# tj12323/GeoPurify

Hardware: AMD Instinct MI355X
Metric: scenes/sec (ScanNet-val shape) + pooled-feature GB/s vs HBM peak (higher is better)
Workload: dtype f32 (student convolutions and pooling: f16 hi/lo split operands, 3 MFMAs per product, fp32 accumulate)

## Files before the change

geopurify_amd/_lib.py:

```python
import ctypes
import os
from ctypes import POINTER, c_char_p, c_double, c_float, c_int32, c_int64, c_size_t, c_uint32, c_void_p

_HERE = os.path.dirname(os.path.abspath(__file__))
LIB_PATH = os.environ.get("GP_LIB") or os.path.join(_HERE, "libgeopurify_hip.so")

_P = c_void_p
GP_KNN_MAX_K = 127

SIGNATURES = {
    "gp_version": (c_int32, []),
    "gp_last_error": (c_char_p, []),
    "gp_debug_set": (c_int32, [c_int32, c_int32]),
    "gp_debug_ptr": (c_int32, [c_int32, _P, c_size_t]),
    "gp_voxelize_workspace_bytes": (c_size_t, [c_int64]),
    "gp_voxelize_f64": (c_int32, [_P, c_int64, POINTER(c_double), _P, _P, _P, _P, _P, _P, _P, c_size_t, _P]),
    "gp_fnv_hash_f64": (c_int32, [_P, c_int64, _P, _P]),
    "gp_project_points_f64": (c_int32, [_P, c_int64, POINTER(c_double), c_double, c_double, c_double,
                                        c_double, _P, c_int32, c_int32, c_int32, c_double, _P, _P, _P]),
    "gp_render_depth_f64": (c_int32, [_P, c_int64, POINTER(c_double), c_double, c_double, c_double, c_double,
                                      c_int32, c_int32, c_int32, _P, _P]),
    "gp_minmax_i32": (c_int32, [_P, c_int64, _P, _P]),
    "gp_morton_order_workspace_bytes": (c_size_t, [c_int64]),
    "gp_morton_order": (c_int32, [_P, c_int64, _P, _P, _P, c_size_t, _P]),
    "gp_grid_bytes": (c_size_t, [c_int64, POINTER(c_int32)]),
    "gp_grid_build": (c_int32, [_P, c_int64, POINTER(c_int32), POINTER(c_int32), _P, c_size_t, _P]),
    "gp_scatter_mean_csr": (c_int32, [_P, c_int64, c_int32, _P, _P, c_int64, _P, _P, c_int64, c_int32, _P]),
    "gp_gather_rows": (c_int32, [_P, c_int64, c_int32, _P, c_int64, _P, _P, c_int64, _P]),
    "gp_kernel_map_build": (c_int32, [_P, _P, c_int64, _P, _P]),
    "gp_coords_order_batched_workspace_bytes": (c_size_t, [c_int64]),
    "gp_coords_order_batched": (c_int32, [_P, c_int64, _P, _P, _P, _P, _P, c_size_t, _P]),
    "gp_kernel_map_sorted": (c_int32, [_P, c_int64, _P, _P]),
    "gp_quantize_batched_workspace_bytes": (c_size_t, [c_int64]),
    "gp_quantize_batched": (c_int32, [_P, c_int64, _P, _P, _P, _P, _P, _P, _P, c_size_t, _P]),
    "gp_segment_labels": (c_int32, [_P, c_int64, _P, _P, _P, c_int64, c_int64, c_int32, _P, _P]),
    "gp_sparse_conv": (c_int32, [_P, c_int64, _P, c_int64, _P, c_int32, c_int32, c_int32, _P, _P, _P,
                                 c_int64, c_int32, _P, c_int64, _P]),
    "gp_conv_pairs_workspace_bytes": (c_size_t, [c_int64, c_int32]),
    "gp_conv_pairs_build": (c_int32, [_P, c_int64, c_int32, c_int32, _P, _P, _P, _P, _P, _P, _P, c_size_t, _P]),
    "gp_conv_chunk_plan_workspace_bytes": (c_size_t, [c_int64, c_int32]),
    "gp_conv_chunk_plan": (c_int32, [_P, c_int64, c_int32, c_int32, c_int32, c_int32, c_int32, _P, _P, _P, c_size_t, _P]),
    "gp_conv_weights_split": (c_int32, [_P, c_int32, c_int32, c_int32, c_float, _P, _P, _P]),
    "gp_split_f16": (c_int32, [_P, c_int64, c_int32, c_int64, _P, _P, c_int64, _P]),
    "gp_sparse_conv_f16x3": (c_int32, [_P, c_int64, _P, _P, c_int64, _P, _P, _P, _P, _P, c_int32, c_int64, c_int64, c_int32, _P, _P,
                                       c_int32, c_int32, _P, _P, _P, _P, c_int64, c_int32, _P, c_int64, _P, _P,
                                       c_int64, c_int32, POINTER(c_int32), POINTER(c_int32), POINTER(c_int32), _P, _P,
                                       _P, _P, c_int64, _P, c_int32, c_int32, _P]),
    "gp_conv_weights_split_blocked": (c_int32, [_P, c_int32, c_int32, c_int32, c_float, _P, _P, c_int32, _P]),
    "gp_pow2_scale": (c_int32, [_P, c_int64, c_int32, c_int64, _P, _P, c_size_t, _P]),
    "gp_voxel_rows_operands": (c_int32, [_P, c_int64, c_int32, _P, c_int64, c_int32, _P, _P, c_int64, _P, _P, c_int64, c_int32, _P, c_int64,
                                         _P, _P, _P, c_size_t, _P]),
    "gp_split_f16_scaled": (c_int32, [_P, c_int64, c_int32, c_int64, _P, _P, c_int64, _P, _P, _P, _P]),
    "gp_rcb_order": (c_int32, [_P, c_int64, c_int32, c_int32, _P, _P, _P]),
    "gp_rows_renumber_i32": (c_int32, [_P, c_int64, c_int32, _P, _P, _P, _P]),
    "gp_l2norm_rows": (c_int32, [_P, c_int64, c_int32, c_int64, _P]),
    "gp_embed_head_f16x3": (c_int32, [_P, _P, c_int64, _P, _P, _P, c_int64, c_int32, c_int32, c_float, c_int32, _P, c_int64, _P, _P, c_float, _P, _P]),
    "gp_knn_workspace_bytes": (c_size_t, [c_int64]),
    "gp_knn_lattice": (c_int32, [_P, _P, _P, c_int64, c_int32, _P, _P, c_size_t, _P]),
    "gp_knn_lattice_two_pass": (c_int32, [_P, _P, _P, c_int64, c_int32, _P, _P, c_size_t, _P]),
    "gp_knn_batched_workspace_bytes": (c_size_t, [c_int64]),
    "gp_knn_batched": (c_int32, [_P, _P, c_int64, c_int32, _P, _P, _P, c_size_t, _P]),
    "gp_affinity_softmax": (c_int32, [_P, c_int64, c_int32, _P, c_int32, c_int64, c_float, _P, _P]),
    "gp_affinity_softmax_scatter": (c_int32, [_P, c_int64, c_int32, _P, c_int32, c_int64, c_float, _P, _P, _P, _P, _P]),
    "gp_pool_ell": (c_int32, [_P, c_int64, _P, _P, c_int32, c_int64, c_int32, _P, c_int64, _P]),
    "gp_pool_transpose_workspace_bytes": (c_size_t, [c_int64, c_int32]),
    "gp_pool_transpose_build": (c_int32, [_P, c_int64, c_int32, _P, _P, _P, c_size_t, _P]),
    "gp_pool_ell_transpose": (c_int32, [_P, c_int64, _P, _P, _P, c_int32, c_int64, c_int32, _P, c_int64, _P]),
    "gp_pool_ell_wgrad": (c_int32, [_P, c_int64, _P, c_int64, _P, c_int32, c_int64, c_int32, _P, c_int32, _P]),
    "gp_affinity_softmax_backward_workspace_bytes": (c_size_t, [c_int64, c_int32]),
    "gp_affinity_softmax_backward": (c_int32, [_P, c_int64, c_int32, _P, _P, _P, c_int32, c_int64, c_float, _P, _P, _P, c_int64, _P,
                                               c_size_t, _P]),
    "gp_l2norm_rows_backward": (c_int32, [_P, c_int64, _P, c_int64, c_int32, c_int64, _P, c_int64, _P]),
    "gp_pool_tiles_workspace_bytes": (c_size_t, [c_int64, c_int32]),
    "gp_pool_tiles_count": (c_int32, [_P, c_int64, c_int32, c_int32, _P, _P, c_size_t, _P]),
    "gp_pool_tiles_fill": (c_int32, [_P, _P, c_int64, c_int32, c_int32, _P, _P, _P, _P]),
    "gp_pool_tiles_apply": (c_int32, [_P, c_int64, _P, _P, _P, c_int32, c_int64, c_int32, _P, c_int64, _P]),
    "gp_pool_mfma_workspace_bytes": (c_size_t, [c_int64, c_int32]),
    "gp_pool_mfma_count": (c_int32, [_P, c_int64, c_int32, c_int32, c_int32, _P, _P, _P, c_size_t, _P]),
    "gp_pool_mfma_fill": (c_int32, [_P, _P, c_int64, c_int32, c_int32, _P, _P, c_int64, _P, _P, _P, _P]),
    "gp_pool_mfma_apply": (c_int32, [_P, _P, c_int64, _P, _P, _P, _P, c_int64, c_int32, c_int32, _P, _P, c_int64, _P, c_int64, _P, _P]),
    "gp_pool_mfma_apply_persistent": (c_int32, [_P, _P, c_int64, _P, _P, _P, _P, c_int64, c_int32, c_int32, c_int32, _P, _P, c_int64,
                                                _P, c_int64, c_int64, _P, _P, _P]),
    "gp_pool_cs_workspace_bytes": (c_size_t, [c_int64, c_int32]),
    "gp_pool_cs_count": (c_int32, [_P, c_int64, c_int32, c_int32, _P, _P, _P, _P, c_size_t, _P]),
    "gp_pool_cs_fill": (c_int32, [_P, _P, c_int64, c_int32, c_int32, _P, c_int64, c_int32, _P, _P, _P, _P, _P]),
    "gp_pool_cs_structure": (c_int32, [_P, c_int64, c_int32, c_int32, _P, c_int64, c_int32, _P, _P, _P, _P, _P, _P]),
    "gp_pool_cs_structure_valid": (c_int32, [_P, c_int64, c_int32, c_int32, _P, c_int64, c_int32, _P, _P, _P, _P]),
    "gp_affinity_cs_fragments": (c_int32, [_P, _P, c_int64, c_int32, c_int32, c_float, _P, _P, _P, _P, c_int32, _P, _P, _P]),
    "gp_pool_cs_apply": (c_int32, [_P, _P, c_int64, _P, _P, _P, _P, _P, c_int64, c_int32, c_int32, _P, _P, c_int64, _P, c_int64, _P, _P]),
    "gp_pool_cs_deps": (c_int32, [_P, _P, c_int64, c_int32, _P, _P, _P]),
    "gp_pool_cs_chain_flag_words": (c_size_t, [c_int64, c_int32]),
    "gp_pool_cs_chain_flag_words_d": (c_size_t, [c_int64, c_int32, c_int32]),
    "gp_pool_cs_apply_chain": (c_int32, [_P, _P, _P, _P, c_int64, _P, _P, _P, _P, _P, c_int64, c_int32, c_int32, c_int32, _P, c_int64, _P, _P, _P,
                                         c_uint32, _P]),
    "gp_lift_dense_accum": (c_int32, [_P, c_int32, c_int32, c_int32, _P, _P, _P, c_int64, _P, c_int64, _P, _P]),
    "gp_lift_dense_bilinear_accum": (c_int32, [_P, c_int32, c_int32, c_int32, c_int32, c_int32, _P, _P, _P, c_int64, _P,
                                               c_int64, _P, _P]),
    "gp_lift_dense_finish": (c_int32, [_P, c_int64, c_int32, _P, c_int64, _P, _P]),
    "gp_lift_masks_workspace_bytes": (c_size_t, [c_int32, c_int32, c_int32]),
    "gp_lift_masks_view": (c_int32, [_P, c_int32, c_int32, c_int32, _P, _P, _P, _P, _P, c_int32, c_int32,
                                     _P, _P, c_int64, _P, _P, _P, c_size_t, _P]),
    "gp_pv_count": (c_int32, [_P, c_int64, _P, _P]),
    "gp_scan_workspace_bytes": (c_size_t, [c_int64]),
    "gp_exclusive_scan_i64": (c_int32, [_P, c_int64, _P, _P, c_size_t, _P]),
    "gp_pv_fill": (c_int32, [_P, _P, c_int64, c_int32, _P, _P, _P, _P, _P]),
    "gp_segment_tables": (c_int32, [_P, c_int32, c_int32, _P, c_int32, c_float, _P, _P, _P]),
    "gp_fuse_views_top3": (c_int32, [_P, _P, _P, c_int64, _P, _P, c_int32, c_int32, c_int32, _P, c_int64, _P, _P]),
    "gp_seen_masks": (c_int32, [_P, c_int64, _P, _P, _P]),
    "gp_fuse_views_top3_fill": (c_int32, [_P, _P, _P, c_int64, _P, _P, c_int32, c_int32, c_int32, _P, _P, c_int64, _P]),
    "gp_nn1_workspace_bytes": (c_size_t, [c_int64, c_int64]),
    "gp_nn1_f64": (c_int32, [_P, c_int64, _P, c_int64, _P, _P, c_size_t, _P]),
    "gp_nn1_masked_workspace_bytes": (c_size_t, [c_int64]),
    "gp_nn1_masked_f64": (c_int32, [_P, c_int64, _P, _P, _P, _P, c_size_t, _P]),
    "gp_visible_lists_workspace_bytes": (c_size_t, [c_int64]),
    "gp_visible_lists": (c_int32, [_P, c_int64, _P, _P, _P, _P, _P, c_size_t, _P]),
    "gp_views_visible_lists_workspace_bytes": (c_size_t, [c_int64, c_int32]),
    "gp_views_visible_lists": (c_int32, [_P, c_int64, _P, _P, c_int32, c_int32, c_int32, c_int32, c_double, c_int64, c_int64,
                                         _P, _P, _P, _P, _P, _P, _P, c_size_t, _P]),
    "gp_lift_masks_views_workspace_bytes": (c_size_t, [c_int32, c_int32, c_int32, c_int32, c_int64, c_int64, c_int64]),
    "gp_lift_masks_views": (c_int32, [_P, c_int32, c_int32, c_int32, c_int32, _P, _P, _P, _P, _P, c_int32, c_int32, _P, c_int64,
                                      _P, _P, _P, _P, _P, _P, c_int32, c_int64, c_int64, _P, _P, _P, _P, _P, c_size_t, _P]),
    "gp_classify_argmax": (c_int32, [_P, c_int64, c_int32, c_int64, _P, c_int32, c_float, _P, _P, _P]),
    "gp_gather_rows_classify": (c_int32, [_P, c_int64, c_int32, _P, c_int64, _P, _P, c_int64, _P, c_int32, c_float, _P, _P, _P]),
    "gp_rows_argmax": (c_int32, [_P, c_int64, c_int32, c_int64, _P, c_int64, c_int32, _P, _P, _P]),
    "gp_col_stats_workspace_bytes": (c_size_t, [c_int64, c_int32]),
    "gp_col_stats": (c_int32, [_P, c_int64, c_int64, c_int32, _P, _P, _P, c_size_t, _P]),
    "gp_bn_train_apply": (c_int32, [_P, c_int64, c_int64, c_int32, _P, _P, _P, _P, c_float, _P, c_int64, c_int32, _P, c_int64,
                                    _P, _P, c_int64, c_float, _P, _P, _P]),
    "gp_bn_train_backward_workspace_bytes": (c_size_t, [c_int64, c_int32]),
    "gp_bn_train_backward": (c_int32, [_P, c_int64, _P, c_int64, _P, c_int64, _P, _P, c_float, _P, _P, c_int64, c_int32, _P, c_int64,
                                       _P, c_int64, _P, _P, _P, _P, _P, c_int64, _P, c_size_t, _P]),
    "gp_col_sums_f64": (c_int32, [_P, c_int64, c_int64, c_int32, _P, _P, _P, c_size_t, _P]),
    "gp_bn_bwd_sums_f64": (c_int32, [_P, c_int64, _P, c_int64, _P, c_int64, _P, _P, c_float, _P, _P, c_int64, c_int32, _P, _P, c_size_t, _P]),
    "gp_bn_bwd_apply": (c_int32, [_P, c_int64, _P, c_int64, _P, c_int64, _P, _P, c_float, _P, _P, _P, c_int64, c_int64, c_int32, _P, c_int64,
                                  _P, c_int64, _P, _P]),
    "gp_infonce_workspace_bytes": (c_size_t, [c_int64, c_int32]),
    "gp_infonce_fwd_bwd": (c_int32, [_P, c_int64, c_int64, c_int32, _P, c_int64, _P, c_int64, c_int32, c_float, _P, _P, c_int64,
                                     _P, c_size_t, _P]),
    "gp_infonce_weighted_fwd_bwd": (c_int32, [_P, c_int64, c_int64, c_int32, _P, c_int64, _P, c_int64, c_int32, c_float, _P, _P, _P, _P, c_int64,
                                              _P, c_size_t, _P]),
    "gp_conv_wgrad_workspace_bytes": (c_size_t, [c_int64, c_int32, c_int32]),
    "gp_conv_wgrad_f16x3": (c_int32, [_P, _P, c_int64, _P, _P, c_int64, _P, _P, _P, c_int64, _P, c_int32, c_int32, c_int32, c_int32,
                                      _P, _P, _P, c_size_t, _P]),
    "gp_adamw_step": (c_int32, [_P, _P, _P, _P, c_int64, c_float, c_float, c_float, c_float, c_float, c_int64, _P]),
    "gp_knn_points_f32": (c_int32, [_P, c_int64, _P, c_int64, c_int32, _P, _P, _P]),
    "gp_sampler_select": (c_int32, [_P, c_int64, c_int64, c_int64, _P, c_int32, _P, _P, _P]),
    "gp_sim_segments_f16x3": (c_int32, [_P, _P, c_int64, c_int32, _P, _P, _P, _P, c_int64, c_int64, _P, _P]),
    "gp_sampler_select_segments": (c_int32, [_P, _P, _P, _P, c_int64, c_int64, _P, c_int32, _P, _P, _P]),
    "gp_sampler_micro_segments": (c_int32, [_P, _P, _P, _P, _P, c_int64, c_int32, _P, c_int64, c_int32, _P, _P]),
    "gp_normalize_split_f16": (c_int32, [_P, c_int64, c_int32, c_int64, c_int64, c_float, _P, _P, c_int64, _P]),
    "gp_iou_hist_i64": (c_int32, [_P, _P, c_int64, c_int32, POINTER(c_int64), c_int32, _P, _P]),
    "gp_nn1_batched_workspace_bytes": (c_size_t, [c_int64]),
    "gp_nn1_batched": (c_int32, [_P, _P, _P, _P, c_int64, c_int32, _P, _P, _P, c_size_t, _P]),
    "gp_iou_hist_batched_i64": (c_int32, [_P, _P, c_int64, _P, _P, c_int64, c_int32, c_int32, POINTER(c_int64), c_int32, _P, _P]),
    "gp_sparse_conv_tiles": (c_int32, [POINTER(c_int32)]),
    "gp_segment_loss_col_step": (c_int32, []),
    "gp_segment_loss_unit_rows": (c_int32, [_P, c_int64, c_int32, c_int64, _P, c_int64, c_int32, _P, _P]),
    "gp_segment_loss_items_workspace_bytes": (c_size_t, [c_int64, c_int64]),
    "gp_segment_loss_items": (c_int32, [_P, _P, c_int64, _P, _P, c_int64, c_int32, POINTER(c_int64), c_int32, c_int32, _P, _P, _P, _P, _P, _P,
                                        _P, c_size_t, _P]),
    "gp_segment_loss_rows": (c_int32, [_P, c_int64, c_int64, c_int32, c_int32, _P, _P, _P, _P, _P, _P, _P, c_int64, _P, _P, _P]),
    "gp_segment_loss_reduce_workspace_bytes": (c_size_t, [c_int64, c_int32]),
    "gp_segment_loss_reduce": (c_int32, [_P, _P, c_int64, _P, c_int32, c_int32, _P, _P, _P, c_size_t, _P]),
    "gp_fused_decode_workspace_bytes": (c_size_t, [c_int64, c_int64]),
    "gp_fused_decode": (c_int32, [_P, c_int64, _P, _P, c_int64, c_int64, _P, c_int64, c_int32, _P, _P, _P, _P, c_size_t, _P]),
    "gp_lift_batched_col_chunk": (c_int32, []),
    "gp_lift_batched_transpose": (c_int32, [_P, c_int32, c_int32, c_int64, _P, _P]),
    "gp_lift_batched_workspace_bytes": (c_size_t, [c_int64, c_int32]),
    "gp_lift_batched": (c_int32, [_P, c_int64, _P, c_int32, c_int32, c_int32, _P, _P, _P, _P, c_int32, c_int32, c_int32, c_int32, c_int32,
                                  c_double, c_int64, c_int64, c_int32, _P, c_int64, _P, _P, _P, _P, _P, _P, _P, c_size_t, _P]),
    "gp_lift_stream_state_bytes": (c_size_t, [c_int64]),
    "gp_lift_stream_begin_workspace_bytes": (c_size_t, [c_int64]),
    "gp_lift_stream_begin": (c_int32, [_P, c_int64, c_int32, _P, c_size_t, _P, c_int64, _P, _P, _P, c_size_t, _P]),
    "gp_lift_stream_add_workspace_bytes": (c_size_t, [c_int32]),
    "gp_lift_stream_add": (c_int32, [_P, c_int64, _P, c_size_t, _P, c_int32, c_int32, c_int32, _P, _P, _P, _P, c_int32, c_int32, c_int32,
                                     c_int32, c_int32, c_double, c_int64, c_int64, _P, c_int64, _P, _P, _P, _P, _P, c_size_t, _P]),
    "gp_lift_stream_finish_workspace_bytes": (c_size_t, [c_int64]),
    "gp_lift_stream_finish": (c_int32, [_P, c_int64, _P, c_size_t, _P, c_int32, c_int64, _P, _P, c_int32, _P, c_int64, _P, _P, _P, _P,
                                        c_size_t, _P]),
    "gp_lift_masks_batched_lists_workspace_bytes": (c_size_t, [c_int64, c_int32]),
    "gp_lift_masks_batched_lists": (c_int32, [_P, c_int64, _P, _P, _P, _P, c_int32, c_int32, c_int32, c_int32, c_double, c_int64, c_int64,
                                              c_int64, _P, _P, _P, _P, _P, _P, _P, _P, _P, c_size_t, _P]),
    "gp_lift_masks_batched_workspace_bytes": (c_size_t, [c_int64, c_int32, c_int32, c_int32, c_int32, c_int32, c_int32, c_int64, c_int32,
                                                         c_int64]),
    "gp_lift_masks_batched": (c_int32, [_P, c_int64, _P, c_int32, _P, c_int32, c_int32, c_int32, _P, _P, _P, _P, _P, c_int32, c_int32,
                                        _P, _P, _P, _P, _P, _P, c_int64, c_int32, c_int64, _P, _P, c_int32, c_int32, c_int32,
                                        _P, c_int64, _P, _P, _P, _P, _P, _P, c_size_t, _P]),
}

_lib = None


# ... 39 lines not shown
```

geopurify_amd/csrc/order_grid.hip:

```cpp
#include <cstring>
#include <rocprim/device/device_radix_sort.hpp>

#include "gp_grid.h"

namespace {

__global__ void minmax_kernel(const int32_t *__restrict__ c, int64_t nv, int32_t *__restrict__ mm) {
    int lo[3] = {INT32_MAX, INT32_MAX, INT32_MAX}, hi[3] = {INT32_MIN, INT32_MIN, INT32_MIN};
    for (int64_t i = blockIdx.x * (int64_t)blockDim.x + threadIdx.x; i < nv; i += (int64_t)gridDim.x * blockDim.x) {
#pragma unroll
        for (int a = 0; a < 3; ++a) {
            int v = c[i * 3 + a];
            lo[a] = min(lo[a], v);
            hi[a] = max(hi[a], v);
        }
    }
    __shared__ int s_lo[4][3], s_hi[4][3];
#pragma unroll
    for (int a = 0; a < 3; ++a) {
        for (int o = 32; o > 0; o >>= 1) {
            lo[a] = min(lo[a], __shfl_xor(lo[a], o, 64));
            hi[a] = max(hi[a], __shfl_xor(hi[a], o, 64));
        }
        if (gp_lane() == 0) { s_lo[threadIdx.x >> 6][a] = lo[a]; s_hi[threadIdx.x >> 6][a] = hi[a]; }
    }
    __syncthreads();
    if (threadIdx.x < 3) {
        const int a = threadIdx.x;
        atomicMin(&mm[a], min(min(s_lo[0][a], s_lo[1][a]), min(s_lo[2][a], s_lo[3][a])));
        atomicMax(&mm[3 + a], max(max(s_hi[0][a], s_hi[1][a]), max(s_hi[2][a], s_hi[3][a])));
    }
}

__global__ void init_minmax_kernel(int32_t *mm) {
    if (threadIdx.x < 3) mm[threadIdx.x] = INT32_MAX;
    else if (threadIdx.x < 6) mm[threadIdx.x] = INT32_MIN;
}

__global__ void morton_keys_kernel(const int32_t *__restrict__ c, int64_t nv, const int32_t *__restrict__ mm,
                                   uint64_t *__restrict__ keys, int32_t *__restrict__ vals) {
    int64_t i = blockIdx.x * (int64_t)blockDim.x + threadIdx.x;
    if (i >= nv) return;
    uint32_t x = (uint32_t)(c[i * 3 + 0] - mm[0]);
    uint32_t y = (uint32_t)(c[i * 3 + 1] - mm[1]);
    uint32_t z = (uint32_t)(c[i * 3 + 2] - mm[2]);
    keys[i] = gp_morton3(x, y, z);
    vals[i] = (int32_t)i;
}

__global__ void invert_perm_kernel(const int32_t *__restrict__ perm, int64_t nv, int32_t *__restrict__ rank) {
    int64_t i = blockIdx.x * (int64_t)blockDim.x + threadIdx.x;
    if (i < nv) rank[perm[i]] = (int32_t)i;
}

__global__ void grid_init_kernel(void *grid, int3 origin, int3 extent, int3 cdim, int64_t nv, int32_t max_cells,
                                 int64_t cell_index_off, int64_t records_off) {
    GpGridHeader *h = reinterpret_cast<GpGridHeader *>(grid);
    if (blockIdx.x == 0 && threadIdx.x == 0) {
        h->origin[0] = origin.x; h->origin[1] = origin.y; h->origin[2] = origin.z;
        h->extent[0] = extent.x; h->extent[1] = extent.y; h->extent[2] = extent.z;
        h->cdim[0] = cdim.x; h->cdim[1] = cdim.y; h->cdim[2] = cdim.z;
        h->status = 0; h->ncells = 0; h->max_cells = max_cells; h->nv = nv;
        h->cell_index_off = cell_index_off; h->records_off = records_off;
    }
    int32_t *ci = reinterpret_cast<int32_t *>(reinterpret_cast<char *>(grid) + cell_index_off);
    int64_t ncell = (int64_t)cdim.x * cdim.y * cdim.z;
    for (int64_t i = blockIdx.x * (int64_t)blockDim.x + threadIdx.x; i < ncell; i += (int64_t)gridDim.x * blockDim.x)
        ci[i] = -1;
}

__device__ __forceinline__ int64_t cell_raster(const GpGridHeader *h, int rx, int ry, int rz) {
    return ((int64_t)(rz >> 3) * h->cdim[1] + (ry >> 3)) * h->cdim[0] + (rx >> 3);
}

__global__ void grid_heads_kernel(void *grid, const int32_t *__restrict__ c, int64_t nv) {
    GpGridHeader *h = reinterpret_cast<GpGridHeader *>(grid);
    int32_t *ci = reinterpret_cast<int32_t *>(reinterpret_cast<char *>(grid) + h->cell_index_off);
    GpCellRec *recs = reinterpret_cast<GpCellRec *>(reinterpret_cast<char *>(grid) + h->records_off);
    int64_t i = blockIdx.x * (int64_t)blockDim.x + threadIdx.x;
    if (i >= nv) return;
    int rx = c[i * 3] - h->origin[0], ry = c[i * 3 + 1] - h->origin[1], rz = c[i * 3 + 2] - h->origin[2];
    bool bad = (unsigned)rx >= (unsigned)h->extent[0] || (unsigned)ry >= (unsigned)h->extent[1] ||
               (unsigned)rz >= (unsigned)h->extent[2];
    uint64_t key = gp_morton3(rx, ry, rz);
    bool head = true;
    if (i > 0) {
        int px = c[i * 3 - 3] - h->origin[0], py = c[i * 3 - 2] - h->origin[1], pz = c[i * 3 - 1] - h->origin[2];
        uint64_t pk = gp_morton3(px, py, pz);
        if (pk >= key) bad = true;
        head = (pk >> 9) != (key >> 9);
    }
    if (bad) { atomicOr(&h->status, 1); return; }
    if (head) {
        int slot = atomicAdd(&h->ncells, 1);
        GpCellRec &r = recs[slot];
        r.start = (int32_t)i;
        r.count = 0;
#pragma unroll
        for (int j = 0; j < 16; ++j) r.bits[j] = 0u;
        ci[cell_raster(h, rx, ry, rz)] = slot;
    }
}

__global__ void grid_fill_kernel(void *grid, const int32_t *__restrict__ c, int64_t nv) {
    GpGridHeader *h = reinterpret_cast<GpGridHeader *>(grid);
    if (h->status) return;
    int32_t *ci = reinterpret_cast<int32_t *>(reinterpret_cast<char *>(grid) + h->cell_index_off);
    GpCellRec *recs = reinterpret_cast<GpCellRec *>(reinterpret_cast<char *>(grid) + h->records_off);
    int64_t i = blockIdx.x * (int64_t)blockDim.x + threadIdx.x;
    if (i >= nv) return;
    int rx = c[i * 3] - h->origin[0], ry = c[i * 3 + 1] - h->origin[1], rz = c[i * 3 + 2] - h->origin[2];
    int slot = ci[cell_raster(h, rx, ry, rz)];
    uint32_t l = gp_local9(rx, ry, rz);
    atomicOr(&recs[slot].bits[l >> 5], 1u << (l & 31));
    atomicAdd(&recs[slot].count, 1);
}

__global__ void kernel_map_kernel(const void *grid, const int32_t *__restrict__ c, int64_t nv,
                                  int32_t *__restrict__ nbr_map) {
    GpGridView g(grid);
    int64_t i = blockIdx.x * (int64_t)blockDim.x + threadIdx.x;
    if (i >= nv) return;
    int rx = c[i * 3] - g.h->origin[0], ry = c[i * 3 + 1] - g.h->origin[1], rz = c[i * 3 + 2] - g.h->origin[2];
    int k = 0;
    for (int dz = -1; dz <= 1; ++dz)
        for (int dy = -1; dy <= 1; ++dy)
            for (int dx = -1; dx <= 1; ++dx, ++k)
                nbr_map[(int64_t)k * nv + i] = (k == 13) ? (int32_t)i : g.lookup_rel(rx + dx, ry + dy, rz + dz);
}

}

extern "C" int gp_minmax_i32(const int32_t *coords, int64_t nv, int32_t *mm, void *stream_) {
    GP_CHECK_ARG(coords && mm && nv > 0, "gp_minmax_i32: null/empty argument");
    hipStream_t s = gp_stream(stream_);
    int blocks = (int)((nv + 255) / 256);
    init_minmax_kernel<<<1, 64, 0, s>>>(mm);
    minmax_kernel<<<min(blocks, 64), 256, 0, s>>>(coords, nv, mm);
    GP_CHECK_LAUNCH();
    return GP_OK;
}

extern "C" size_t gp_morton_order_workspace_bytes(int64_t nv) {
    size_t tmp = 0;
    (void)rocprim::radix_sort_pairs(nullptr, tmp, (uint64_t *)nullptr, (uint64_t *)nullptr, (int32_t *)nullptr,
                              (int32_t *)nullptr, (size_t)nv, 0, 64, 0);
    GpCarver cv(nullptr, 0);
    cv.take<int32_t>(8);
    cv.take<uint64_t>(nv);
    cv.take<uint64_t>(nv);
    cv.take<int32_t>(nv);
    cv.take<char>(tmp);
    return cv.off;
}

extern "C" int gp_morton_order(const int32_t *coords, int64_t nv, int32_t *perm, int32_t *rank, void *workspace,
                               size_t workspace_bytes, void *stream_) {
    GP_CHECK_ARG(nv > 0 && nv < (1ll << 31), "gp_morton_order: nv=%lld out of range", (long long)nv);
    hipStream_t s = gp_stream(stream_);
    size_t tmp = 0;
    (void)rocprim::radix_sort_pairs(nullptr, tmp, (uint64_t *)nullptr, (uint64_t *)nullptr, (int32_t *)nullptr,
                              (int32_t *)nullptr, (size_t)nv, 0, 64, 0);
    GpCarver cv(workspace, workspace_bytes);
    int32_t *mm = cv.take<int32_t>(8);
    uint64_t *k0 = cv.take<uint64_t>(nv);
    uint64_t *k1 = cv.take<uint64_t>(nv);
    int32_t *v0 = cv.take<int32_t>(nv);
    char *t = cv.take<char>(tmp);
    if (!cv.ok()) { gp_set_error("gp_morton_order: workspace too small (%zu < %zu)", workspace_bytes, cv.off); return GP_ENOMEM; }
    int blocks = (int)((nv + 255) / 256);
    init_minmax_kernel<<<1, 64, 0, s>>>(mm);
    minmax_kernel<<<min(blocks, 64), 256, 0, s>>>(coords, nv, mm);
    morton_keys_kernel<<<blocks, 256, 0, s>>>(coords, nv, mm, k0, v0);
    GP_CHECK_LAUNCH();
    GP_CHECK_HIP(rocprim::radix_sort_pairs(t, tmp, k0, k1, v0, perm, (size_t)nv, 0, 64, s));
    invert_perm_kernel<<<blocks, 256, 0, s>>>(perm, nv, rank);
    GP_CHECK_LAUNCH();
    return GP_OK;
}

static void grid_layout(int64_t nv, const int32_t *extent, int3 &cdim, int32_t &max_cells, int64_t &ci_off,
                        int64_t &rec_off, size_t &total) {
    cdim = make_int3(((extent[0] - 1) >> 3) + 1, ((extent[1] - 1) >> 3) + 1, ((extent[2] - 1) >> 3) + 1);
    int64_t ncell = (int64_t)cdim.x * cdim.y * cdim.z;
    max_cells = (int32_t)(nv < ncell ? nv : ncell);
    ci_off = 256;
    rec_off = ci_off + (int64_t)gp_align_up((size_t)ncell * 4, 256);
    total = (size_t)rec_off + gp_align_up((size_t)max_cells * sizeof(GpCellRec), 256);
}

extern "C" size_t gp_grid_bytes(int64_t nv, const int32_t *extent_host) {
    if (!extent_host || nv <= 0 || extent_host[0] <= 0 || extent_host[1] <= 0 || extent_host[2] <= 0) return 0;
    int3 cdim; int32_t mc; int64_t a, b; size_t total;
    grid_layout(nv, extent_host, cdim, mc, a, b, total);
    return total;
}

extern "C" int gp_grid_build(const int32_t *coords, int64_t nv, const int32_t *origin_host, const int32_t *extent_host,
                             void *grid, size_t grid_bytes, void *stream_) {
    GP_CHECK_ARG(coords && grid && origin_host && extent_host && nv > 0, "gp_grid_build: null/empty argument");
    for (int a = 0; a < 3; ++a)
        if (extent_host[a] <= 0 || extent_host[a] > (1 << 15)) { gp_set_error("gp_grid_build: extent[%d]=%d not in 1..32768", a, extent_host[a]); return GP_ERANGE; }
    int3 cdim; int32_t mc; int64_t ci_off, rec_off; size_t total;
    grid_layout(nv, extent_host, cdim, mc, ci_off, rec_off, total);
    if (grid_bytes < total) { gp_set_error("gp_grid_build: grid buffer too small (%zu < %zu)", grid_bytes, total); return GP_ENOMEM; }
    hipStream_t s = gp_stream(stream_);
    int blocks = (int)((nv + 255) / 256);
    grid_init_kernel<<<1024, 256, 0, s>>>(grid, make_int3(origin_host[0], origin_host[1], origin_host[2]),
                                         make_int3(extent_host[0], extent_host[1], extent_host[2]), cdim, nv, mc, ci_off, rec_off);
    grid_heads_kernel<<<blocks, 256, 0, s>>>(grid, coords, nv);
    grid_fill_kernel<<<blocks, 256, 0, s>>>(grid, coords, nv);
    GP_CHECK_LAUNCH();
    return GP_OK;
}

extern "C" int gp_kernel_map_build(const void *grid, const int32_t *coords, int64_t nv, int32_t *nbr_map, void *stream_) {
    GP_CHECK_ARG(grid && coords && nbr_map && nv > 0, "gp_kernel_map_build: null/empty argument");
    kernel_map_kernel<<<(int)((nv + 255) / 256), 256, 0, gp_stream(stream_)>>>(grid, coords, nv, nbr_map);
    GP_CHECK_LAUNCH();
    return GP_OK;
}
```

geopurify_amd/csrc/rcb.hip:

```cpp
#include "gp_common.h"

namespace {

constexpr int RCB_MAX_SEG = 32;

template <int CH, int NT>
__global__ void __launch_bounds__(NT)
rcb_chunk_kernel(const int32_t *__restrict__ coords , int64_t nv, int leaf, int32_t *__restrict__ sigma, int32_t *__restrict__ rho) {
    __shared__ int s_c[3][CH];
    __shared__ unsigned s_key[CH];
    __shared__ unsigned short s_perm[2][CH];
    __shared__ unsigned char s_seg[CH];
    __shared__ int s_start[RCB_MAX_SEG + 1], s_len[RCB_MAX_SEG], s_axis[RCB_MAX_SEG], s_lo[RCB_MAX_SEG][3], s_hi[RCB_MAX_SEG][3];
    __shared__ int s_nseg, s_more;
    const int tid = threadIdx.x;
    const int64_t base = (int64_t)blockIdx.x * CH;
    const int n = (int)((nv - base) < CH ? (nv - base) : CH);
    for (int i = tid; i < CH; i += NT) {
        const int64_t r = base + (i < n ? i : n - 1);
        s_c[0][i] = coords[r * 3];
        s_c[1][i] = coords[r * 3 + 1];
        s_c[2][i] = coords[r * 3 + 2];
        s_perm[0][i] = (unsigned short)i;
    }
    if (tid == 0) { s_nseg = 1; s_start[0] = 0; s_len[0] = n; s_more = n > leaf; }
    __syncthreads();
    int cur = 0, level = 0;
    while (s_more) {
        const int nseg = s_nseg;
        for (int i = tid; i < nseg * 3; i += NT) { s_lo[i / 3][i % 3] = 0x7fffffff; s_hi[i / 3][i % 3] = -0x7fffffff; }
        for (int i = tid; i < CH; i += NT) {
            int sg = 0;
            if (i < n) {
                int lo = 0, hi = nseg - 1;
                while (lo < hi) { const int mid = (lo + hi + 1) >> 1; if (s_start[mid] <= i) lo = mid; else hi = mid - 1; }
                sg = lo;
            }
            s_seg[i] = (unsigned char)sg;
        }
        __syncthreads();
        for (int i = tid; i < n; i += NT) {
            const int sg = s_seg[i];
            if (s_len[sg] > leaf) {
                const int r = s_perm[cur][i];
#pragma unroll
                for (int a = 0; a < 3; ++a) { atomicMin(&s_lo[sg][a], s_c[a][r]); atomicMax(&s_hi[sg][a], s_c[a][r]); }
            }
        }
        __syncthreads();
        if (tid < nseg) {
            int ax = 0, best = -1;
            if (s_len[tid] > leaf) {
#pragma unroll
                for (int a = 0; a < 3; ++a) { const int e = s_hi[tid][a] - s_lo[tid][a]; if (e > best) { best = e; ax = a; } }
            } else {
                ax = -1;
            }
            s_axis[tid] = ax;
        }
        __syncthreads();
        for (int i = tid; i < CH; i += NT) {
            unsigned k = 0xffffffffu;
            if (i < n) {
                const int sg = s_seg[i], ax = s_axis[sg];
                unsigned c = 0;
                if (ax >= 0) c = (unsigned)(s_c[ax][s_perm[cur][i]] - s_lo[sg][ax]) & 0x7fffu;
                k = ((unsigned)sg << 27) | (c << 12) | (unsigned)i;
            }
            s_key[i] = k;
        }
        __syncthreads();
        const int limit = (n == CH) ? (CH >> level) : CH;
        for (int kk = 2; kk <= limit; kk <<= 1)
            for (int j = kk >> 1; j > 0; j >>= 1) {
                for (int i = tid; i < CH; i += NT) {
                    const int ixj = i ^ j;
                    if (ixj > i) {
                        const unsigned x = s_key[i], y = s_key[ixj];
                        const bool up = (kk == limit) || ((i & kk) == 0);
                        if ((x > y) == up) { s_key[i] = y; s_key[ixj] = x; }
                    }
                }
                __syncthreads();
            }
        ++level;
        for (int i = tid; i < n; i += NT) s_perm[cur ^ 1][i] = s_perm[cur][s_key[i] & 0xfffu];
        cur ^= 1;
        if (tid == 0) {
            int ns = 0, more = 0;
            int st[RCB_MAX_SEG], ln[RCB_MAX_SEG];
            for (int sg = 0; sg < nseg; ++sg) {
                const int len = s_len[sg], start = s_start[sg];
                if (len > leaf && ns + 2 <= RCB_MAX_SEG) {
                    int half = ((len / 2 + leaf - 1) / leaf) * leaf;
                    if (half >= len) half = len / 2;
                    st[ns] = start; ln[ns] = half; ++ns;
                    st[ns] = start + half; ln[ns] = len - half; ++ns;
                    more |= (half > leaf) | (len - half > leaf);
                } else {
                    st[ns] = start; ln[ns] = len; ++ns;
                }
            }
            for (int sg = 0; sg < ns; ++sg) { s_start[sg] = st[sg]; s_len[sg] = ln[sg]; }
            s_nseg = ns;
            s_more = more && ns < RCB_MAX_SEG;
        }
        __syncthreads();
    }
    for (int i = tid; i < n; i += NT) {
        const int r = s_perm[cur][i];
        sigma[base + i] = (int32_t)(base + r);
        rho[base + r] = (int32_t)(base + i);
    }
}

__global__ void rows_renumber_kernel(const int32_t *__restrict__ nbr, int64_t nv, int k, const int32_t *__restrict__ sigma,
                                     const int32_t *__restrict__ rho, int32_t *__restrict__ out) {
    const int64_t total = nv * k;
    for (int64_t i = blockIdx.x * (int64_t)blockDim.x + threadIdx.x; i < total; i += (int64_t)gridDim.x * blockDim.x) {
        const int64_t p = i / k;
        const int j = (int)(i - p * k);
        out[i] = rho[nbr[(int64_t)sigma[p] * k + j]];
    }
}

}

extern "C" int gp_rcb_order(const int32_t *coords, int64_t nv, int32_t chunk_rows, int32_t leaf_rows, int32_t *sigma, int32_t *rho,
                            void *stream_) {
    GP_CHECK_ARG(coords && sigma && rho && nv > 0, "gp_rcb_order: null/empty argument");
    GP_CHECK_ARG(chunk_rows == 1024 || chunk_rows == 2048, "gp_rcb_order: chunk_rows=%d (1024 or 2048: a chunk lives in one workgroup's LDS)", chunk_rows);
    GP_CHECK_ARG(leaf_rows >= 16 && chunk_rows % leaf_rows == 0 && chunk_rows / leaf_rows <= RCB_MAX_SEG,
                 "gp_rcb_order: leaf_rows=%d must divide the chunk into at most %d leaves", leaf_rows, RCB_MAX_SEG);
    GP_CHECK_ARG(nv < ((int64_t)1 << 31), "gp_rcb_order: row ids are 32-bit");
    hipStream_t s = gp_stream(stream_);
    const unsigned blocks = (unsigned)((nv + chunk_rows - 1) / chunk_rows);
    if (chunk_rows == 1024) rcb_chunk_kernel<1024, 256><<<blocks, 256, 0, s>>>(coords, nv, leaf_rows, sigma, rho);
    else rcb_chunk_kernel<2048, 512><<<blocks, 512, 0, s>>>(coords, nv, leaf_rows, sigma, rho);
    GP_CHECK_LAUNCH();
    return GP_OK;
}

extern "C" int gp_rows_renumber_i32(const int32_t *nbr, int64_t nv, int32_t k, const int32_t *sigma, const int32_t *rho, int32_t *out,
                                    void *stream_) {
    GP_CHECK_ARG(nbr && sigma && rho && out && nv > 0 && k > 0 && out != nbr, "gp_rows_renumber_i32: null/empty argument (out must not alias nbr)");
    rows_renumber_kernel<<<2048, 256, 0, gp_stream(stream_)>>>(nbr, nv, k, sigma, rho, out);
    GP_CHECK_LAUNCH();
    return GP_OK;
}
```

geopurify_amd/csrc/sparse_conv_v2.hip:

```cpp
#include <cstring>
#include <type_traits>
#include <rocprim/device/device_scan.hpp>

#include <hip/hip_fp16.h>

#include <stdlib.h>

#include "gp_common.h"
#include "gp_gfx950.h"

namespace {

constexpr int TM = 256, TN = 256, TK = 32;
constexpr int NT2 = 512;
constexpr int APITCH = 32;
__device__ __forceinline__ int sw_slot(int row, int slot) {
    const int h = (0x78 >> (((row >> 2) & 3) * 2)) & 3;
    return slot ^ h;
}

__device__ __forceinline__ void pair_decode(int64_t i, int kv, const int32_t *__restrict__ R, int nchunks, int &c, int &k, int64_t &u) {
    const int row_q = (int)(i / kv);
    int lo = 0, hi = nchunks - 1;
    while (lo < hi) {
        const int mid = (lo + hi + 1) >> 1;
        if (R[mid] <= row_q) lo = mid; else hi = mid - 1;
    }
    c = lo;
    const int64_t r0 = R[c], rows_raw = R[c + 1] - r0, rows_c = rows_raw > 0 ? rows_raw : 1;
    const int64_t rem = i - (int64_t)kv * r0;
    int64_t kk = rem / rows_c;
    kk = kk < 0 ? 0 : (kk >= kv ? kv - 1 : kk);
    k = (int)kk;
    u = r0 + (rem - kk * rows_c);
}
__global__ void pair_flags_kernel(const int32_t *__restrict__ nm, int64_t nv, int kv, const int32_t *__restrict__ R, int nchunks,
                                  int32_t *__restrict__ f) {
    int64_t total = (int64_t)kv * nv;
    int64_t i = blockIdx.x * (int64_t)blockDim.x + threadIdx.x;
    if (i >= total) return;
    int c, k; int64_t u;
    pair_decode(i, kv, R, nchunks, c, k, u);
    u = u < 0 ? 0 : (u >= nv ? nv - 1 : u);
    f[i] = nm[(int64_t)k * nv + u] >= 0 ? 1 : 0;
}
__global__ void pair_emit_kernel(const int32_t *__restrict__ nm, const int32_t *__restrict__ sc, int64_t nv, int kv,
                                 const int32_t *__restrict__ R, int nchunks, int32_t *__restrict__ pair_in, int32_t *__restrict__ pair_pos,
                                 int32_t *__restrict__ seg_off ) {
    int64_t total = (int64_t)kv * nv;
    int64_t i = blockIdx.x * (int64_t)blockDim.x + threadIdx.x;
    if (i >= total) return;
    int c, k; int64_t u;
    pair_decode(i, kv, R, nchunks, c, k, u);
    u = u < 0 ? 0 : (u >= nv ? nv - 1 : u);
    int in = nm[(int64_t)k * nv + u];
    int s = sc[i];
    pair_pos[(int64_t)k * nv + u] = in >= 0 ? s : -1;
    if (in >= 0) pair_in[s] = in;
    if (u == (int64_t)R[c]) seg_off[c * kv + k] = s;
    if (i == total - 1) seg_off[(c + 1) * kv] = s + (in >= 0 ? 1 : 0);
}
__global__ void chunk_count_kernel(const int32_t *__restrict__ nm, int64_t nv, int kv, int granule, int32_t *__restrict__ cnt ) {
    const int g = blockIdx.x, k = blockIdx.y;
    const int64_t r0 = (int64_t)g * granule, r1 = r0 + granule < nv ? r0 + granule : nv;
    int c = 0;
    for (int64_t u = r0 + threadIdx.x; u < r1; u += blockDim.x) c += nm[(int64_t)k * nv + u] >= 0;
    c = gp_wave_sum(c);
    __shared__ int s_c[4];
    if (gp_lane() == 0) s_c[threadIdx.x >> 6] = c;
    __syncthreads();
    if (threadIdx.x == 0) cnt[g * 32 + k] = s_c[0] + s_c[1] + s_c[2] + s_c[3];
}
constexpr int CP_WIN = 512;
__device__ __forceinline__ int cp_sum32(int v) {
    v += __builtin_amdgcn_update_dpp(0, v, 0xB1, 0xF, 0xF, true);
    v += __builtin_amdgcn_update_dpp(0, v, 0x4E, 0xF, 0xF, true);
    v += __builtin_amdgcn_update_dpp(0, v, 0x141, 0xF, 0xF, true);
    v += __builtin_amdgcn_update_dpp(0, v, 0x140, 0xF, 0xF, true);
    return __builtin_amdgcn_readlane(v, 0) + __builtin_amdgcn_readlane(v, 16);
}
__global__ void __launch_bounds__(256)
chunk_plan_kernel(const int32_t *__restrict__ cnt, int ngran, int kv, int granule, int64_t nv, int col_tiles, int target,
                  int max_chunks, int32_t *__restrict__ R, int32_t *__restrict__ n_chunks) {
    __shared__ unsigned short s_cnt[CP_WIN * 32];
    const int tid = threadIdx.x, lane = tid & 63;
    int sum = 0, nc = 0, start_g = 0;
    if (tid == 0) R[0] = 0;
    for (int g0 = 0; g0 < ngran; g0 += CP_WIN) {
        const int n = ngran - g0 < CP_WIN ? ngran - g0 : CP_WIN;
        __syncthreads();
        {
            const int4 *c4 = reinterpret_cast<const int4 *>(cnt + (int64_t)g0 * 32);
            const int n4 = n * 8;
            for (int i0 = tid; i0 < n4; i0 += 1024) {
                int4 v[4];
#pragma unroll
                for (int q = 0; q < 4; ++q) v[q] = (i0 + q * 256 < n4) ? c4[i0 + q * 256] : make_int4(0, 0, 0, 0);
#pragma unroll
                for (int q = 0; q < 4; ++q) {
                    const int i = i0 + q * 256;
                    if (i < n4) {
                        const int k0 = (i * 4) & 31;
                        s_cnt[i * 4 + 0] = (unsigned short)(k0 + 0 < kv ? v[q].x : 0);
                        s_cnt[i * 4 + 1] = (unsigned short)(k0 + 1 < kv ? v[q].y : 0);
                        s_cnt[i * 4 + 2] = (unsigned short)(k0 + 2 < kv ? v[q].z : 0);
                        s_cnt[i * 4 + 3] = (unsigned short)(k0 + 3 < kv ? v[q].w : 0);
                    }
                }
            }
        }
        __syncthreads();
        if (tid < 64) {
            auto step = [&](int g, int add, int tiles_with) {
                if (tiles_with > target && g != start_g && nc + 1 < max_chunks) {
                    ++nc;
                    if (lane == 0) R[nc] = g * granule;
                    sum = add;
                    start_g = g;
                    return true;
                }
                sum += add;
                return false;
            };
            for (int gl = 0; gl < n; gl += 4) {
                int a[4], run[4], t[4];
#pragma unroll
                for (int j = 0; j < 4; ++j) a[j] = (lane < 32 && gl + j < n) ? s_cnt[(gl + j) * 32 + lane] : 0;
                run[0] = sum + a[0];
#pragma unroll
                for (int j = 1; j < 4; ++j) run[j] = run[j - 1] + a[j];
#pragma unroll
                for (int j = 0; j < 4; ++j) t[j] = cp_sum32(lane < 32 ? (run[j] + TM - 1) / TM : 0) * col_tiles;
                bool redo = false;
#pragma unroll
                for (int j = 0; j < 4; ++j) {
                    if (gl + j >= n) break;
                    const int tiles_with = redo ? cp_sum32(lane < 32 ? (sum + a[j] + TM - 1) / TM : 0) * col_tiles : t[j];
                    redo = step(g0 + gl + j, a[j], tiles_with) || redo;
                }
            }
        }
    }
    if (tid == 0) { R[nc + 1] = (int32_t)nv; n_chunks[0] = nc + 1; }
}
__global__ void tile_desc_kernel(const int32_t *__restrict__ seg_off, const int32_t *__restrict__ tile_start, int nseg, int kv,
                                 int4 *__restrict__ desc) {
    int sgi = blockIdx.x * blockDim.x + threadIdx.x;
    if (sgi >= nseg) return;
    int t0 = tile_start[sgi], t1 = tile_start[sgi + 1];
    int p0 = seg_off[sgi], p1 = seg_off[sgi + 1];
    for (int t = t0; t < t1; ++t) {
        int base = p0 + (t - t0) * TM;
        desc[t] = make_int4(sgi % kv, base, min(TM, p1 - base), 0);
    }
}

__global__ void tile_start_kernel(const int32_t *__restrict__ seg_off, int nseg, int32_t *__restrict__ tile_start) {
    if (blockIdx.x != 0 || threadIdx.x != 0) return;
    int acc = 0;
    for (int s = 0; s < nseg; ++s) {
        tile_start[s] = acc;
        acc += (seg_off[s + 1] - seg_off[s] + TM - 1) / TM;
    }
    tile_start[nseg] = acc;
}

struct V2Smem {
    _Float16 a_hi[2][TM][APITCH];
    _Float16 a_lo[2][TM][APITCH];
    _Float16 b_hi[2][TN][APITCH];
    _Float16 b_lo[2][TN][APITCH];
};

template <int NRT>
__device__ __forceinline__ void mma_step_f16x3(const V2Smem &sm, int buf, int wm, int wn, int fl, int fsw,
                                               f32x4 (&acc)[4][8]) {
    f16x8 ah[NRT > 0 ? NRT : 1], al[NRT > 0 ? NRT : 1];
#pragma unroll
    for (int i = 0; i < NRT; ++i) {
        ah[i] = *reinterpret_cast<const f16x8 *>(&sm.a_hi[buf][wm * 64 + i * 16 + fl][fsw]);
        al[i] = *reinterpret_cast<const f16x8 *>(&sm.a_lo[buf][wm * 64 + i * 16 + fl][fsw]);
    }
#pragma unroll
    for (int j = 0; j < 8; ++j) {
        f16x8 bh = *reinterpret_cast<const f16x8 *>(&sm.b_hi[buf][wn * 128 + j * 16 + fl][fsw]);
        f16x8 bl = *reinterpret_cast<const f16x8 *>(&sm.b_lo[buf][wn * 128 + j * 16 + fl][fsw]);
#pragma unroll
        for (int i = 0; i < NRT; ++i) acc[i][j] = __builtin_amdgcn_mfma_f32_16x16x32_f16(ah[i], bh, acc[i][j], 0, 0, 0);
#pragma unroll
        for (int i = 0; i < NRT; ++i) acc[i][j] = __builtin_amdgcn_mfma_f32_16x16x32_f16(ah[i], bl, acc[i][j], 0, 0, 0);
#pragma unroll
        for (int i = 0; i < NRT; ++i) acc[i][j] = __builtin_amdgcn_mfma_f32_16x16x32_f16(al[i], bh, acc[i][j], 0, 0, 0);
    }
}
template <int NRT>
__device__ __forceinline__ void mma_step_f16x3_off(const unsigned char *smem, const uint32_t (&fa_hi)[4], const uint32_t (&fa_lo)[4],
                                                   uint32_t a_off, const V2Smem &sm, int buf, int wn, int fl, int fsw, f32x4 (&acc)[4][8]) {
    f16x8 ah[NRT > 0 ? NRT : 1], al[NRT > 0 ? NRT : 1];
#pragma unroll
    for (int i = 0; i < NRT; ++i) {
        ah[i] = *reinterpret_cast<const f16x8 *>(smem + fa_hi[i] + a_off);
        al[i] = *reinterpret_cast<const f16x8 *>(smem + fa_lo[i] + a_off);
    }
#pragma unroll
    for (int j = 0; j < 8; ++j) {
        f16x8 bh = *reinterpret_cast<const f16x8 *>(&sm.b_hi[buf][wn * 128 + j * 16 + fl][fsw]);
        f16x8 bl = *reinterpret_cast<const f16x8 *>(&sm.b_lo[buf][wn * 128 + j * 16 + fl][fsw]);
#pragma unroll
        for (int i = 0; i < NRT; ++i) acc[i][j] = __builtin_amdgcn_mfma_f32_16x16x32_f16(ah[i], bh, acc[i][j], 0, 0, 0);
#pragma unroll
        for (int i = 0; i < NRT; ++i) acc[i][j] = __builtin_amdgcn_mfma_f32_16x16x32_f16(ah[i], bl, acc[i][j], 0, 0, 0);
#pragma unroll
        for (int i = 0; i < NRT; ++i) acc[i][j] = __builtin_amdgcn_mfma_f32_16x16x32_f16(al[i], bh, acc[i][j], 0, 0, 0);
    }
}
template <bool TUNE>
__global__ void __launch_bounds__(NT2)
conv_phase1_kernel(const float *__restrict__ x, int64_t ld_x, const int32_t *__restrict__ pair_in,
                   const int32_t *__restrict__ off, const int32_t *__restrict__ tile_start, const int4 *__restrict__ tile_desc,
                   int nseg, int kv, const _Float16 *__restrict__ w_hi, const _Float16 *__restrict__ w_lo, int cin, int cout,
                   float *__restrict__ P, int n_tiles, int ablate_, int tile_begin, int tile_count, int pair_base, int w_blocked) {
    extern __shared__ __align__(16) unsigned char smem_raw[];
    const int ablate = TUNE ? ablate_ : 0;
    V2Smem &sm = *reinterpret_cast<V2Smem *>(smem_raw);
// ... 798 lines not shown
            }
        }
    }
}

__global__ void split_rows_scaled_kernel(const float *__restrict__ x, int64_t ld_x, int d, int64_t n, _Float16 *__restrict__ hi,
                                         _Float16 *__restrict__ lo, int64_t ld_h, const float *__restrict__ scale,
                                         float *__restrict__ row_inv, const int32_t *__restrict__ dst_row) {
    const int lane = gp_lane();
    for (int64_t r = (blockIdx.x * (int64_t)blockDim.x + threadIdx.x) >> 6; r < n; r += ((int64_t)gridDim.x * blockDim.x) >> 6) {
        float s = scale ? scale[0] : 1.f;
        const int64_t ro = dst_row ? (int64_t)dst_row[r] : r;
        if (row_inv) {
            float amax = 0.f;
            for (int c = lane * 4; c < d; c += 256) {
                float4 a = *reinterpret_cast<const float4 *>(x + r * ld_x + c);
                amax = fmaxf(amax, fmaxf(fmaxf(fabsf(a.x), fabsf(a.y)), fmaxf(fabsf(a.z), fabsf(a.w))));
            }
            s = gp_pow2_for(gp_wave_max(amax));
            if (lane == 0) row_inv[ro] = 1.f / s;
        }
        for (int c = lane * 4; c < d; c += 256) {
            float4 a = *reinterpret_cast<const float4 *>(x + r * ld_x + c);
            float v[4] = {a.x * s, a.y * s, a.z * s, a.w * s};
            f16x4 h, l;
            gp_split_f16<4>(v, h, l);
            if (lo) {
                *reinterpret_cast<f16x4 *>(hi + ro * ld_h + c) = h;
                *reinterpret_cast<f16x4 *>(lo + ro * ld_h + c) = l;
            } else {
                _Float16 *ph = hi + ro * ld_h + ((c >> 5) << 6) + (c & 31);
                *reinterpret_cast<f16x4 *>(ph) = h;
                *reinterpret_cast<f16x4 *>(ph + 32) = l;
            }
        }
    }
}

__global__ void amax_kernel(const float *__restrict__ x, int64_t ld_x, int d, int64_t n, unsigned *__restrict__ out) {
    float m = 0.f;
    const int64_t total = n * (d / 4);
    for (int64_t i = blockIdx.x * (int64_t)blockDim.x + threadIdx.x; i < total; i += (int64_t)gridDim.x * blockDim.x) {
        int64_t r = i / (d / 4);
        int c = (int)(i - r * (d / 4)) * 4;
        float4 a = *reinterpret_cast<const float4 *>(x + r * ld_x + c);
        m = fmaxf(m, fmaxf(fmaxf(fabsf(a.x), fabsf(a.y)), fmaxf(fabsf(a.z), fabsf(a.w))));
    }
    __shared__ float s_m[4];
    m = gp_wave_max(m);
    if (gp_lane() == 0) s_m[threadIdx.x >> 6] = m;
    __syncthreads();
    if (threadIdx.x == 0) atomicMax(out, __float_as_uint(fmaxf(fmaxf(s_m[0], s_m[1]), fmaxf(s_m[2], s_m[3]))));
}
__global__ void pow2_scale_kernel(const unsigned *__restrict__ amax_bits, float *__restrict__ out2) {
    const float s = gp_pow2_for(__uint_as_float(amax_bits[0]));
    out2[0] = s;
    out2[1] = 1.f / s;
}

__global__ void split_rows_kernel(const float *__restrict__ x, int64_t ld_x, int d, int64_t n, _Float16 *__restrict__ hi,
                                  _Float16 *__restrict__ lo, int64_t ld_h) {
    int64_t total = n * (d / 4);
    for (int64_t i = blockIdx.x * (int64_t)blockDim.x + threadIdx.x; i < total; i += (int64_t)gridDim.x * blockDim.x) {
        int64_t r = i / (d / 4);
        int c = (int)(i - r * (d / 4)) * 4;
        float4 a = *reinterpret_cast<const float4 *>(x + r * ld_x + c);
        float v[4] = {a.x, a.y, a.z, a.w};
        f16x4 h, l;
        gp_split_f16<4>(v, h, l);
        *reinterpret_cast<f16x4 *>(hi + r * ld_h + c) = h;
        *reinterpret_cast<f16x4 *>(lo + r * ld_h + c) = l;
    }
}

__global__ void weight_split_kernel(const float *__restrict__ w, int kv, int cin, int cout, float s,
                                    _Float16 *__restrict__ hi, _Float16 *__restrict__ lo) {
    int64_t total = (int64_t)kv * cin * cout;
    for (int64_t i = blockIdx.x * (int64_t)blockDim.x + threadIdx.x; i < total; i += (int64_t)gridDim.x * blockDim.x) {
        int64_t k = i / ((int64_t)cin * cout);
        int64_t rem = i - k * (int64_t)cin * cout;
        int n = (int)(rem / cin), c = (int)(rem % cin);
        const float v = w[(k * cin + c) * cout + n] * s;
        gp_split_f16(v, hi[i], lo[i]);
    }
}

__global__ void __launch_bounds__(256)
weight_split_blocked_kernel(const float *__restrict__ w, int kv, int cin, int cout, float s,
                            _Float16 *__restrict__ hi, _Float16 *__restrict__ lo, int transpose_flip) {
    const int steps = cin / TK, nt = cout / TN;
    const int st = blockIdx.x % steps, t = (blockIdx.x / steps) % nt, k = blockIdx.x / (steps * nt);
    const int c = threadIdx.x;
    const int rho = (c & 128) | ((c >> 3) & 15) | ((c & 7) << 4);
    float v[TK];
    if (transpose_flip) {
        const float *src = w + ((int64_t)(kv - 1 - k) * cout + t * TN + c) * cin + st * TK;
#pragma unroll
        for (int q = 0; q < TK / 4; ++q) *reinterpret_cast<float4 *>(v + 4 * q) = *reinterpret_cast<const float4 *>(src + 4 * q);
    } else {
        const float *src = w + ((int64_t)k * cin + st * TK) * cout + t * TN + c;
#pragma unroll
        for (int kk = 0; kk < TK; ++kk) v[kk] = src[(int64_t)kk * cout];
    }
    const int64_t o = ((((int64_t)k * nt + t) * steps + st) * TN + rho) * TK;
#pragma unroll
    for (int q = 0; q < TK / 8; ++q) {
        f16x8 h, l;
#pragma unroll
        for (int j = 0; j < 8; ++j) gp_split_f16(v[q * 8 + j] * s, h, l, j);
        *reinterpret_cast<f16x8 *>(hi + o + q * 8) = h;
        *reinterpret_cast<f16x8 *>(lo + o + q * 8) = l;
    }
}

size_t scan_tmp32(int64_t n) {
    size_t t = 0;
    (void)rocprim::exclusive_scan(nullptr, t, (int32_t *)nullptr, (int32_t *)nullptr, (int32_t)0, (size_t)n, rocprim::plus<int32_t>(), 0);
    return t;
}

}

#define g_conv_ablate g_gp_knobs[3]


extern "C" size_t gp_conv_pairs_workspace_bytes(int64_t nv, int32_t kv) {
    if (nv <= 0 || kv <= 0) return 0;
    GpCarver cv(nullptr, 0);
    cv.take<int32_t>((size_t)kv * nv);
    cv.take<int32_t>((size_t)kv * nv);
    cv.take<char>(scan_tmp32((int64_t)kv * nv));
    return cv.off;
}

extern "C" int gp_conv_pairs_build(const int32_t *nbr_map, int64_t nv, int32_t kv, int32_t num_chunks, const int32_t *chunk_row_off,
                                   int32_t *pair_in, int32_t *pair_pos, int32_t *seg_off, int32_t *tile_start, int32_t *tile_desc,
                                   void *workspace, size_t workspace_bytes, void *stream_) {
    GP_CHECK_ARG(nbr_map && pair_in && pair_pos && seg_off && tile_start && tile_desc && workspace && nv > 0 && kv > 0, "gp_conv_pairs_build: null/empty argument");
    GP_CHECK_ARG((int64_t)kv * nv < (1ll << 31), "gp_conv_pairs_build: kernel map too large");
    GP_CHECK_ARG(num_chunks >= 1 && chunk_row_off, "gp_conv_pairs_build: num_chunks=%d needs the chunk row offsets (device, [num_chunks + 1], 0 .. nv ascending)", num_chunks);
    int64_t total = (int64_t)kv * nv;
    GpCarver cv(workspace, workspace_bytes);
    int32_t *f = cv.take<int32_t>(total), *sc = cv.take<int32_t>(total);
    size_t tb = scan_tmp32(total);
    char *tmp = cv.take<char>(tb);
    if (!cv.ok()) { gp_set_error("gp_conv_pairs_build: workspace too small (%zu < %zu)", workspace_bytes, cv.off); return GP_ENOMEM; }
    hipStream_t s = gp_stream(stream_);
    int blocks = (int)((total + 255) / 256);
    int nseg = num_chunks * kv;
    pair_flags_kernel<<<blocks, 256, 0, s>>>(nbr_map, nv, kv, chunk_row_off, num_chunks, f);
    GP_CHECK_HIP(rocprim::exclusive_scan(tmp, tb, f, sc, (int32_t)0, (size_t)total, rocprim::plus<int32_t>(), s));
    pair_emit_kernel<<<blocks, 256, 0, s>>>(nbr_map, sc, nv, kv, chunk_row_off, num_chunks, pair_in, pair_pos, seg_off);
    tile_start_kernel<<<1, 64, 0, s>>>(seg_off, nseg, tile_start);
    tile_desc_kernel<<<(nseg + 255) / 256, 256, 0, s>>>(seg_off, tile_start, nseg, kv, reinterpret_cast<int4 *>(tile_desc));
    GP_CHECK_LAUNCH();
    return GP_OK;
}

extern "C" size_t gp_conv_chunk_plan_workspace_bytes(int64_t nv, int32_t granule_rows) {
    if (nv <= 0 || granule_rows <= 0) return 0;
    return (size_t)((nv + granule_rows - 1) / granule_rows) * 32 * sizeof(int32_t);
}
extern "C" int gp_conv_chunk_plan(const int32_t *nbr_map, int64_t nv, int32_t kv, int32_t granule_rows, int32_t col_tiles,
                                  int32_t target_tiles, int32_t max_chunks, int32_t *chunk_row_off, int32_t *n_chunks, void *workspace,
                                  size_t workspace_bytes, void *stream_) {
    GP_CHECK_ARG(nbr_map && chunk_row_off && n_chunks && workspace && nv > 0 && kv > 0 && kv <= 32, "gp_conv_chunk_plan: null/empty argument");
    GP_CHECK_ARG(granule_rows >= 64 && granule_rows <= 65535 && col_tiles >= 1 && target_tiles >= col_tiles && max_chunks >= 1, "gp_conv_chunk_plan: bad sizes");
    const int64_t ngran = (nv + granule_rows - 1) / granule_rows;
    GP_CHECK_ARG(workspace_bytes >= gp_conv_chunk_plan_workspace_bytes(nv, granule_rows), "gp_conv_chunk_plan: workspace too small");
    hipStream_t s = gp_stream(stream_);
    int32_t *cnt = static_cast<int32_t *>(workspace);
    chunk_count_kernel<<<dim3((unsigned)ngran, (unsigned)kv), 256, 0, s>>>(nbr_map, nv, kv, granule_rows, cnt);
    chunk_plan_kernel<<<1, 256, 0, s>>>(cnt, (int)ngran, kv, granule_rows, nv, col_tiles, target_tiles, max_chunks, chunk_row_off, n_chunks);
    GP_CHECK_LAUNCH();
    return GP_OK;
}

extern "C" int gp_conv_weights_split(const float *w, int32_t kv, int32_t cin, int32_t cout, float scale_pow2,
                                     void *w_hi, void *w_lo, void *stream_) {
    GP_CHECK_ARG(w && w_hi && w_lo && kv > 0 && cin > 0 && cout > 0, "gp_conv_weights_split: null/empty argument");
    weight_split_kernel<<<2048, 256, 0, gp_stream(stream_)>>>(w, kv, cin, cout, scale_pow2, static_cast<_Float16 *>(w_hi),
                                                              static_cast<_Float16 *>(w_lo));
    GP_CHECK_LAUNCH();
    return GP_OK;
}

extern "C" int gp_conv_weights_split_blocked(const float *w, int32_t kv, int32_t cin, int32_t cout, float scale_pow2, void *w_hi,
                                             void *w_lo, int32_t transpose_flip, void *stream_) {
    GP_CHECK_ARG(w && w_hi && w_lo && kv > 0 && cin > 0 && cout > 0, "gp_conv_weights_split_blocked: null/empty argument");
    GP_CHECK_ARG(cin % TK == 0 && cout % TN == 0, "gp_conv_weights_split_blocked: cin=%d must be a multiple of %d and cout=%d of %d", cin, TK, cout, TN);
    GP_CHECK_ARG(!transpose_flip || ((reinterpret_cast<uintptr_t>(w) & 15) == 0), "gp_conv_weights_split_blocked: w must be 16-byte aligned");
    weight_split_blocked_kernel<<<(unsigned)((int64_t)kv * (cout / TN) * (cin / TK)), 256, 0, gp_stream(stream_)>>>(
        w, kv, cin, cout, scale_pow2, static_cast<_Float16 *>(w_hi), static_cast<_Float16 *>(w_lo), transpose_flip);
    GP_CHECK_LAUNCH();
    return GP_OK;
}

extern "C" int gp_split_f16(const float *x, int64_t ld_x, int32_t d, int64_t n, void *hi, void *lo, int64_t ld_h,
                            void *stream_) {
    GP_CHECK_ARG(x && hi && lo && n > 0 && d > 0 && d % 4 == 0 && ld_x % 4 == 0 && ld_h % 4 == 0, "gp_split_f16: bad argument");
    split_rows_kernel<<<2048, 256, 0, gp_stream(stream_)>>>(x, ld_x, d, n, static_cast<_Float16 *>(hi), static_cast<_Float16 *>(lo), ld_h);
    GP_CHECK_LAUNCH();
    return GP_OK;
}

extern "C" int gp_pow2_scale(const float *x, int64_t ld_x, int32_t d, int64_t n, float *scale2, void *workspace,
                             size_t workspace_bytes, void *stream_) {
    GP_CHECK_ARG(x && scale2 && workspace && workspace_bytes >= 4 && n > 0 && d > 0 && d % 4 == 0 && ld_x % 4 == 0,
                 "gp_pow2_scale: bad argument");
    hipStream_t s = gp_stream(stream_);
    GP_CHECK_HIP(hipMemsetAsync(workspace, 0, 4, s));
    amax_kernel<<<1024, 256, 0, s>>>(x, ld_x, d, n, static_cast<unsigned *>(workspace));
    pow2_scale_kernel<<<1, 1, 0, s>>>(static_cast<const unsigned *>(workspace), scale2);
    GP_CHECK_LAUNCH();
    return GP_OK;
}

extern "C" int gp_split_f16_scaled(const float *x, int64_t ld_x, int32_t d, int64_t n, void *hi, void *lo, int64_t ld_h,
                                   const float *scale, float *row_inv_scale, const int32_t *dst_row, void *stream_) {
    GP_CHECK_ARG(x && hi && n > 0 && d > 0 && d % 4 == 0 && ld_x % 4 == 0 && ld_h % 4 == 0, "gp_split_f16_scaled: bad argument");
    GP_CHECK_ARG(lo || (d % 32 == 0 && ld_h >= 2 * (int64_t)d), "gp_split_f16_scaled: lo = NULL asks for interleaved rows in hi: d %% 32 == 0 and ld_h >= 2 d");
    GP_CHECK_ARG(!(scale && row_inv_scale), "gp_split_f16_scaled: one global scale OR per-row scales");
    int64_t waves = n < 16384 ? n : 16384;
    split_rows_scaled_kernel<<<(unsigned)((waves * 64 + 255) / 256), 256, 0, gp_stream(stream_)>>>(
        x, ld_x, d, n, static_cast<_Float16 *>(hi), static_cast<_Float16 *>(lo), ld_h, scale, row_inv_scale, dst_row);
    GP_CHECK_LAUNCH();
    return GP_OK;
}

extern "C" int gp_sparse_conv_f16x3(const float *x, int64_t ld_x, const void *x_hi, const void *x_lo, int64_t ld_xh,
                                    const int32_t *pair_in, const int32_t *pair_pos,
                                    const int32_t *pair_off, const int32_t *tile_start, const int32_t *tile_desc,
                                    int32_t nseg, int64_t num_pairs, int64_t nv, int32_t kv,
                                    const void *w_hi, const void *w_lo, int32_t cin, int32_t cout, float *partial,
                                    const float *scale, const float *shift, const float *residual, int64_t ld_res,
                                    int32_t relu, float *y, int64_t ld_y, void *y_hi, void *y_lo, int64_t ld_yh,
                                    int32_t num_chunks, const int32_t *chunk_row_off_host, const int32_t *chunk_tile_off_host,
                                    const int32_t *chunk_pair_off_host, const float *x_row_inv_scale, float *y_row_inv_scale,
                                    const void *res_hi, const void *res_lo, int64_t ld_rh, const float *res_row_inv_scale, int32_t w_blocked,
                                    int32_t plane_flags, void *stream_) {
    GP_CHECK_ARG(plane_flags >= 0 && plane_flags < 64, "gp_sparse_conv_f16x3: plane_flags is a mask of 1 (x interleaved), 2 (y interleaved), 4 (residual interleaved), 8 (fp32 partial rows), 16 (one dense offset: phase 1 writes y), 32 (phase 2 walks one row at a time)");
    const bool direct = (plane_flags & 16) != 0;
    GP_CHECK_ARG(!direct || (kv == 1 && num_pairs == nv && x_hi && y && ld_y == cout && !scale && !shift && !residual && !res_hi && !relu && !y_hi &&
                             !y_row_inv_scale && !(g_gp_knobs[3] & 16)),
                 "gp_sparse_conv_f16x3: plane_flags bit 4 is for kv = 1 with a pair for every row, pre-split x, contiguous fp32 y and no epilogue");
    GP_CHECK_ARG(!(plane_flags & 1) || (x_hi && ld_xh % 64 == 0 && cin % 32 == 0), "gp_sparse_conv_f16x3: interleaved x rows come as ONE tensor (x_hi) of 2 x cin halfs per row");
    GP_CHECK_ARG(!(plane_flags & 2) || (y_hi && ld_yh % 64 == 0 && (uintptr_t)y_hi % 16 == 0), "gp_sparse_conv_f16x3: interleaved y rows go to ONE tensor (y_hi) of 2 x cout halfs per row");
    GP_CHECK_ARG(!(plane_flags & 4) || (res_hi && ld_rh % 64 == 0), "gp_sparse_conv_f16x3: interleaved residual rows come as ONE tensor (res_hi)");
    GP_CHECK_ARG(w_blocked == 0 || w_blocked == 1, "gp_sparse_conv_f16x3: w_blocked is 0 (row-major weights) or 1 (gp_conv_weights_split_blocked)");
    GP_CHECK_ARG(!res_hi || ((res_lo || (plane_flags & 4)) && !residual && ld_rh % 8 == 0 && (uintptr_t)res_hi % 16 == 0 && (uintptr_t)res_lo % 16 == 0),
                 "gp_sparse_conv_f16x3: the residual comes as fp32 rows OR as 16-byte aligned split planes (res_hi + res_lo), not both");
    GP_CHECK_ARG(res_hi || (!res_lo && !res_row_inv_scale), "gp_sparse_conv_f16x3: res_lo / res_row_inv_scale belong to res_hi");
    GP_CHECK_ARG((x || (x_hi && (x_lo || (plane_flags & 1)))) && pair_in && pair_pos && pair_off && tile_start && tile_desc && nseg > 0 && w_hi && w_lo && partial && (y || y_hi), "gp_sparse_conv_f16x3: null argument");
    GP_CHECK_ARG(!x_hi || (ld_xh % 8 == 0 && (uintptr_t)x_hi % 16 == 0 && (uintptr_t)x_lo % 16 == 0), "gp_sparse_conv_f16x3: pre-split rows must be 16-byte aligned");
    GP_CHECK_ARG(!(plane_flags & 1) || !(g_gp_knobs[3] & 16), "gp_sparse_conv_f16x3: interleaved x rows need the LDS-DMA path");
    GP_CHECK_ARG(!y_hi || ((y_lo || (plane_flags & 2)) && ld_yh % 4 == 0), "gp_sparse_conv_f16x3: y_hi/y_lo come as a pair");
    GP_CHECK_ARG(!x_row_inv_scale || x_hi, "gp_sparse_conv_f16x3: x_row_inv_scale belongs to pre-split operands (x_hi/x_lo)");
    GP_CHECK_ARG(!y_row_inv_scale || (y_hi && cout <= 1024), "gp_sparse_conv_f16x3: y_row_inv_scale needs y_hi/y_lo and cout <= 1024");
    GP_CHECK_ARG(nv > 0 && num_pairs > 0 && (kv == 27 || kv == 1), "gp_sparse_conv_f16x3: bad sizes");
    GP_CHECK_ARG(cin % TK == 0, "gp_sparse_conv_f16x3: cin=%d must be a multiple of %d", cin, TK);
    GP_CHECK_ARG(x_hi || (ld_x % 4 == 0 && (uintptr_t)x % 16 == 0), "gp_sparse_conv_f16x3: x rows must be 16-byte aligned");
    GP_SMEM_ATTR(conv_phase1_kernel<false>, sizeof(V2Smem));
    GP_SMEM_ATTR(conv_phase1_kernel<true>, sizeof(V2Smem));
    constexpr size_t P1_DMA_SMEM = sizeof(V2Smem) + TM * sizeof(float);
    GP_SMEM_ATTR(conv_phase1_dma_kernel, P1_DMA_SMEM);
    GP_SMEM_ATTR(conv_phase1_tuning_kernel, P1_DMA_SMEM);
    GP_SMEM_ATTR(conv_phase1_stamp_kernel, P1_DMA_SMEM);

    uint64_t *stamp = static_cast<uint64_t *>(g_gp_debug_ptr[1]);
    GP_CHECK_ARG(cout % TN == 0, "gp_sparse_conv_f16x3: cout=%d must be a multiple of %d on this path", cout, TN);
    hipStream_t s = gp_stream(stream_);
    int n_tiles = cout / TN;
    GP_CHECK_ARG((num_chunks >= 1) == (chunk_tile_off_host != nullptr) && (num_chunks >= 1) == (chunk_pair_off_host != nullptr) &&
                     (num_chunks >= 1) == (chunk_row_off_host != nullptr),
                 "gp_sparse_conv_f16x3: num_chunks=%d needs ALL THREE host chunk tables (row, tile and pair offsets), num_chunks=0 needs none",
                 num_chunks);
    if (num_chunks >= 1) {
        bool rows_ok = chunk_row_off_host[0] == 0 && chunk_row_off_host[num_chunks] == nv;
        for (int c = 0; c < num_chunks && rows_ok; ++c) rows_ok = chunk_row_off_host[c + 1] > chunk_row_off_host[c];
        GP_CHECK_ARG(rows_ok, "gp_sparse_conv_f16x3: the %d chunk row offsets do not cover rows 0 .. %lld in ascending order", num_chunks, (long long)nv);
    }
    const bool chunked = num_chunks >= 1;
    const int nchunk = chunked ? num_chunks : 1;
    constexpr int p2_wg_per_cu = 6;
    bool q24_fits = !(plane_flags & 8);
    for (int c = 0; c < nchunk; ++c) {
        const int64_t cp = chunked ? (int64_t)chunk_pair_off_host[c + 1] - chunk_pair_off_host[c] : num_pairs;
        if (cp * cout * 3 + 32 >= ((int64_t)1 << 32)) q24_fits = false;
    }
    for (int c = 0; c < nchunk; ++c) {
        int tile_begin = chunked ? chunk_tile_off_host[c] : 0;
        int tile_count = chunked ? chunk_tile_off_host[c + 1] - tile_begin : (int)(num_pairs / TM + nseg);
        int pair_base = chunked ? chunk_pair_off_host[c] : 0;
        int64_t row_begin = chunked ? chunk_row_off_host[c] : 0;
        int64_t row_count = chunked ? chunk_row_off_host[c + 1] - row_begin : nv;
        const int64_t chunk_pairs = chunked ? (int64_t)chunk_pair_off_host[c + 1] - pair_base : num_pairs;
        const int64_t q_e_off = (chunk_pairs * cout * 3 + 15) & ~(int64_t)15;
        const bool dma_path = x_hi && !(g_conv_ablate & 16);
        const bool q24 = dma_path && !(g_conv_ablate & 32) && q24_fits;
        if (tile_count > 0) {
            int64_t nblocks = (((int64_t)tile_count * n_tiles + 7) / 8) * 8;
            const int tune = (g_conv_ablate & ~16) | ((dma_path && (!q24_fits || direct)) ? 32 : 0);
#define P1_ARGS static_cast<const _Float16 *>(x_hi), static_cast<const _Float16 *>(x_lo), ld_xh, pair_in, pair_off, tile_start,              \
                reinterpret_cast<const int4 *>(tile_desc), nseg, kv, static_cast<const _Float16 *>(w_hi), static_cast<const _Float16 *>(w_lo), \
                cin, cout, direct ? y + (int64_t)pair_base * cout : partial, n_tiles, tune, tile_begin, tile_count, pair_base, x_row_inv_scale, stamp, \
                q_e_off, w_blocked, plane_flags & 1
// ... 44 lines not shown
```

geopurify_amd/csrc/voxelize.hip:

```cpp
#include <cstring>
#include <rocprim/device/device_radix_sort.hpp>
#include <rocprim/device/device_scan.hpp>

#include "gp_common.h"
#include "gp_project.h"

namespace {

struct Mat34 { double m[3][4]; };
struct Mat44 { double m[4][4]; };

__global__ void vox_affine_kernel(const double *__restrict__ c, int64_t n, Mat34 R, double *__restrict__ out,
                                  long long *__restrict__ mn) {
    long long lo[3] = {LLONG_MAX, LLONG_MAX, LLONG_MAX};
    for (int64_t i = blockIdx.x * (int64_t)blockDim.x + threadIdx.x; i < n; i += (int64_t)gridDim.x * blockDim.x) {
        double x = c[i * 3], y = c[i * 3 + 1], z = c[i * 3 + 2];
#pragma unroll
        for (int a = 0; a < 3; ++a) {
            double v = floor(dot4_blas(R.m[a], x, y, z));
            out[i * 3 + a] = v;
            long long iv = (long long)v;
            lo[a] = iv < lo[a] ? iv : lo[a];
        }
    }
    __shared__ long long s_lo[4][3];
#pragma unroll
    for (int a = 0; a < 3; ++a) {
        for (int o = 32; o > 0; o >>= 1) {
            long long t = __shfl_xor(lo[a], o, 64);
            lo[a] = t < lo[a] ? t : lo[a];
        }
        if (gp_lane() == 0) s_lo[threadIdx.x >> 6][a] = lo[a];
    }
    __syncthreads();
    if (threadIdx.x < 3) {
        const int a = threadIdx.x;
        long long v = s_lo[0][a];
#pragma unroll
        for (int w = 1; w < 4; ++w) v = s_lo[w][a] < v ? s_lo[w][a] : v;
        atomicMin(&mn[a], v);
    }
}

__global__ void init_min_kernel(long long *mn) {
    if (threadIdx.x < 3) mn[threadIdx.x] = LLONG_MAX;
}

__device__ __forceinline__ uint64_t fnv3(double a, double b, double c) {
    uint64_t h = 14695981039346656037ull;
    h *= 1099511628211ull; h ^= (uint64_t)a;
    h *= 1099511628211ull; h ^= (uint64_t)b;
    h *= 1099511628211ull; h ^= (uint64_t)c;
    return h;
}

__global__ void vox_hash_kernel(double *__restrict__ c, int64_t n, const long long *__restrict__ mn,
                                uint64_t *__restrict__ keys, int64_t *__restrict__ vals) {
    int64_t i = blockIdx.x * (int64_t)blockDim.x + threadIdx.x;
    if (i >= n) return;
    double v[3];
#pragma unroll
    for (int a = 0; a < 3; ++a) {
        v[a] = floor(c[i * 3 + a] - (double)mn[a]);
        c[i * 3 + a] = v[a];
    }
    keys[i] = fnv3(v[0], v[1], v[2]);
    vals[i] = i;
}

__global__ void fnv_kernel(const double *__restrict__ c, int64_t n, uint64_t *__restrict__ h) {
    int64_t i = blockIdx.x * (int64_t)blockDim.x + threadIdx.x;
    if (i < n) h[i] = fnv3(c[i * 3], c[i * 3 + 1], c[i * 3 + 2]);
}

__global__ void head_flags_kernel(const uint64_t *__restrict__ ks, int64_t n, int32_t *__restrict__ flag) {
    int64_t i = blockIdx.x * (int64_t)blockDim.x + threadIdx.x;
    if (i < n) flag[i] = (i == 0 || ks[i] != ks[i - 1]) ? 1 : 0;
}

__global__ void vox_emit_kernel(const double *__restrict__ c, const int64_t *__restrict__ order,
                                const int32_t *__restrict__ flag, const int32_t *__restrict__ scan, int64_t n,
                                double *__restrict__ coords_aug, int64_t *__restrict__ inds,
                                int64_t *__restrict__ inv, int64_t *__restrict__ nv_dev,
                                int64_t *__restrict__ order_out, int64_t *__restrict__ seg_start) {
    int64_t i = blockIdx.x * (int64_t)blockDim.x + threadIdx.x;
    if (i >= n) return;
    int64_t p = order[i];
    int64_t v = (int64_t)scan[i] - 1;
    inv[p] = v;
    if (order_out) order_out[i] = p;
    if (flag[i]) {
        inds[v] = p;
        coords_aug[v * 3] = c[p * 3];
        coords_aug[v * 3 + 1] = c[p * 3 + 1];
        coords_aug[v * 3 + 2] = c[p * 3 + 2];
        if (seg_start) seg_start[v] = i;
    }
    if (i == n - 1) {
        *nv_dev = v + 1;
        if (seg_start) seg_start[v + 1] = n;
    }
}

__global__ void views_flags_kernel(const double *__restrict__ c, int64_t n, const double *__restrict__ params,
                                   const double *__restrict__ depth, int W, int H, int cut, double tau, int32_t *__restrict__ flags) {
    const int64_t i = blockIdx.x * (int64_t)blockDim.x + threadIdx.x;
    const int v = blockIdx.y;
    if (i >= n) return;
    const double *P = params + v * 20;
    long long ui, vi;
    flags[(int64_t)v * n + i] = project_point(c[i * 3], c[i * 3 + 1], c[i * 3 + 2], P, P + 4, P + 8, P[16], P[17], P[18], P[19],
                                              depth ? depth + (int64_t)v * W * H : nullptr, W, H, cut, tau, ui, vi) ? 1 : 0;
}
__global__ void views_compact_kernel(const double *__restrict__ c, int64_t n, int nviews, const double *__restrict__ params,
                                     const double *__restrict__ depth, int W, int H, int cut, double tau,
                                     const int32_t *__restrict__ sc , int64_t *__restrict__ ent_pt,
                                     int64_t *__restrict__ ent_x, int64_t *__restrict__ ent_y, int32_t *__restrict__ ent_view,
                                     int64_t *__restrict__ view_off) {
    const int64_t i = blockIdx.x * (int64_t)blockDim.x + threadIdx.x;
    const int v = blockIdx.y;
    if (i >= n) return;
    const double *P = params + v * 20;
    long long ui, vi;
    const bool inside = project_point(c[i * 3], c[i * 3 + 1], c[i * 3 + 2], P, P + 4, P + 8, P[16], P[17], P[18], P[19],
                                      depth ? depth + (int64_t)v * W * H : nullptr, W, H, cut, tau, ui, vi);
    const int32_t pos = sc[(int64_t)v * n + i];
    if (inside) { ent_pt[pos] = i; ent_x[pos] = vi; ent_y[pos] = ui; ent_view[pos] = v; }
    if (i == 0) view_off[v] = pos;
    if (v == nviews - 1 && i == n - 1) view_off[nviews] = pos + (inside ? 1 : 0);
}
__global__ void views_keep_kernel(const int64_t *__restrict__ view_off, int nviews, int64_t min_visible, int64_t val_keep,
                                  uint8_t *__restrict__ keep) {
    const int v = blockIdx.x * blockDim.x + threadIdx.x;
    if (v >= nviews) return;
    const int64_t nv = view_off[v + 1] - view_off[v];
    keep[v] = (nv != 0 && nv >= min_visible && nv <= val_keep) ? 1 : 0;
}

__global__ void project_kernel(const double *__restrict__ c, int64_t n, Mat44 M, double fx, double fy, double cx,
                               double cy, const double *__restrict__ depth, int W, int H, int cut, double tau,
                               int64_t *__restrict__ mapping, double *__restrict__ weight) {
    int64_t i = blockIdx.x * (int64_t)blockDim.x + threadIdx.x;
    if (i >= n) return;
    long long ui, vi;
    const bool inside = project_point(c[i * 3], c[i * 3 + 1], c[i * 3 + 2], M.m[0], M.m[1], M.m[2], fx, fy, cx, cy, depth, W, H,
                                      cut, tau, ui, vi);
    mapping[i * 3] = inside ? vi : 0;
    mapping[i * 3 + 1] = inside ? ui : 0;
    mapping[i * 3 + 2] = inside ? 1 : 0;
    if (weight) {
        double a = (double)ui - (double)W / 2, b = (double)vi - (double)H / 2;
        weight[i] = exp(-sqrt(a * a + b * b) / 10.0);
    }
}

__global__ void depth_fill_kernel(double *__restrict__ depth, int64_t n) {
    int64_t i = blockIdx.x * (int64_t)blockDim.x + threadIdx.x;
    if (i < n) depth[i] = 999999.0;
}
__global__ void render_depth_kernel(const double *__restrict__ c, int64_t n, Mat44 M, double fx, double fy, double cx,
                                    double cy, int W, int H, int cut, double *__restrict__ depth) {
    int64_t i = blockIdx.x * (int64_t)blockDim.x + threadIdx.x;
    if (i >= n) return;
    double x = c[i * 3], y = c[i * 3 + 1], z = c[i * 3 + 2];
    double p0 = dot4_blas(M.m[0], x, y, z), p1 = dot4_blas(M.m[1], x, y, z), p2 = dot4_blas(M.m[2], x, y, z);
    double u = (p0 * fx) / p2 + cx;
    double v = (p1 * fy) / p2 + cy;
    double ur = rint(u), vr = rint(v);
    bool finite = (fabs(ur) < 9.0e15) && (fabs(vr) < 9.0e15);
    long long ui = finite ? (long long)ur : -1, vi = finite ? (long long)vr : -1;
    bool inside = finite && ui >= cut && vi >= cut && ui < (long long)W - cut && vi < (long long)H - cut;
    if (inside && p2 > 0.2)
        atomicMin(reinterpret_cast<unsigned long long *>(depth + vi * W + ui), (unsigned long long)__double_as_longlong(p2));
}

size_t sort_tmp_bytes(int64_t n) {
    size_t t = 0;
    (void)rocprim::radix_sort_pairs(nullptr, t, (uint64_t *)nullptr, (uint64_t *)nullptr, (int64_t *)nullptr,
                                    (int64_t *)nullptr, (size_t)n, 0, 64, 0);
    size_t t2 = 0;
    (void)rocprim::inclusive_scan(nullptr, t2, (int32_t *)nullptr, (int32_t *)nullptr, (size_t)n, rocprim::plus<int32_t>(), 0);
    return t > t2 ? t : t2;
}

struct VoxWs {
    long long *mn; double *ctmp; uint64_t *k0, *k1; int64_t *v0, *v1; int32_t *flag, *scan; char *tmp; size_t tmp_bytes;
};
VoxWs carve_vox(GpCarver &cv, int64_t n) {
    VoxWs w;
    w.tmp_bytes = sort_tmp_bytes(n);
    w.mn = cv.take<long long>(4);
    w.ctmp = cv.take<double>(3 * n);
    w.k0 = cv.take<uint64_t>(n);
    w.k1 = cv.take<uint64_t>(n);
    w.v0 = cv.take<int64_t>(n);
    w.v1 = cv.take<int64_t>(n);
    w.flag = cv.take<int32_t>(n);
    w.scan = cv.take<int32_t>(n);
    w.tmp = cv.take<char>(w.tmp_bytes);
    return w;
}

}

extern "C" size_t gp_voxelize_workspace_bytes(int64_t n) {
    if (n <= 0) return 0;
    GpCarver cv(nullptr, 0);
    carve_vox(cv, n);
    return cv.off;
}

extern "C" int gp_voxelize_f64(const double *coords, int64_t n, const double *rigid_host, double *coords_aug,
                               int64_t *inds, int64_t *inds_reconstruct, int64_t *nv_dev, int64_t *order,
                               int64_t *seg_start, void *workspace, size_t workspace_bytes, void *stream_) {
    GP_CHECK_ARG(coords && rigid_host && coords_aug && inds && inds_reconstruct && nv_dev && workspace,
                 "gp_voxelize_f64: null argument");
    GP_CHECK_ARG(n > 0 && n < (1ll << 31), "gp_voxelize_f64: n=%lld out of range (empty clouds are rejected like the reference's assert)", (long long)n);
    GpCarver cv(workspace, workspace_bytes);
    VoxWs w = carve_vox(cv, n);
    if (!cv.ok()) { gp_set_error("gp_voxelize_f64: workspace too small (%zu < %zu)", workspace_bytes, cv.off); return GP_ENOMEM; }
    hipStream_t s = gp_stream(stream_);
    Mat34 R;
    for (int a = 0; a < 3; ++a)
        for (int k = 0; k < 4; ++k) R.m[a][k] = rigid_host[a * 4 + k];
    int blocks = (int)((n + 255) / 256);
    init_min_kernel<<<1, 64, 0, s>>>(w.mn);
    vox_affine_kernel<<<blocks < 256 ? blocks : 256, 256, 0, s>>>(coords, n, R, w.ctmp, w.mn);
    vox_hash_kernel<<<blocks, 256, 0, s>>>(w.ctmp, n, w.mn, w.k0, w.v0);
    GP_CHECK_LAUNCH();
    size_t tb = w.tmp_bytes;
    GP_CHECK_HIP(rocprim::radix_sort_pairs(w.tmp, tb, w.k0, w.k1, w.v0, w.v1, (size_t)n, 0, 64, s));
    head_flags_kernel<<<blocks, 256, 0, s>>>(w.k1, n, w.flag);
    tb = w.tmp_bytes;
    GP_CHECK_HIP(rocprim::inclusive_scan(w.tmp, tb, w.flag, w.scan, (size_t)n, rocprim::plus<int32_t>(), s));
    vox_emit_kernel<<<blocks, 256, 0, s>>>(w.ctmp, w.v1, w.flag, w.scan, n, coords_aug, inds, inds_reconstruct, nv_dev,
                                           order, seg_start);
    GP_CHECK_LAUNCH();
    return GP_OK;
}

extern "C" int gp_fnv_hash_f64(const double *coords, int64_t n, uint64_t *hash, void *stream_) {
    GP_CHECK_ARG(coords && hash && n > 0, "gp_fnv_hash_f64: null/empty argument");
    fnv_kernel<<<(int)((n + 255) / 256), 256, 0, gp_stream(stream_)>>>(coords, n, hash);
    GP_CHECK_LAUNCH();
    return GP_OK;
}

extern "C" int gp_project_points_f64(const double *coords, int64_t n, const double *w2c_host, double fx, double fy,
                                     double cx, double cy, const double *depth, int32_t width, int32_t height,
                                     int32_t cut_bound, double vis_thres, int64_t *mapping, double *weight,
                                     void *stream_) {
    GP_CHECK_ARG(coords && w2c_host && mapping && n > 0, "gp_project_points_f64: null/empty argument");
    GP_CHECK_ARG(width > 0 && height > 0, "gp_project_points_f64: bad image size %dx%d", width, height);
    Mat44 M;
    for (int a = 0; a < 4; ++a)
        for (int k = 0; k < 4; ++k) M.m[a][k] = w2c_host[a * 4 + k];
    project_kernel<<<(int)((n + 255) / 256), 256, 0, gp_stream(stream_)>>>(coords, n, M, fx, fy, cx, cy, depth, width,
                                                                          height, cut_bound, vis_thres, mapping, weight);
    GP_CHECK_LAUNCH();
    return GP_OK;
}

static size_t views_scan_tmp(int64_t n) {
    size_t t = 0;
    (void)rocprim::exclusive_scan(nullptr, t, (int32_t *)nullptr, (int32_t *)nullptr, (int32_t)0, (size_t)n, rocprim::plus<int32_t>(), 0);
    return t;
}
extern "C" size_t gp_views_visible_lists_workspace_bytes(int64_t n, int32_t nviews) {
    if (n <= 0 || nviews <= 0) return 0;
    GpCarver cv(nullptr, 0);
    cv.take<int32_t>(n * nviews); cv.take<int32_t>(n * nviews); cv.take<char>(views_scan_tmp(n * nviews));
    return cv.off;
}
extern "C" int gp_views_visible_lists(const double *coords, int64_t n, const double *params, const double *depth, int32_t nviews,
                                      int32_t width, int32_t height, int32_t cut_bound, double vis_thres, int64_t min_visible,
                                      int64_t val_keep, int64_t *ent_pt, int64_t *ent_x, int64_t *ent_y, int32_t *ent_view,
                                      int64_t *view_off, uint8_t *keep, void *workspace, size_t workspace_bytes, void *stream_) {
    GP_CHECK_ARG(coords && params && ent_pt && ent_x && ent_y && ent_view && view_off && keep && workspace && n > 0,
                 "gp_views_visible_lists: null/empty argument");
    GP_CHECK_ARG(nviews > 0 && nviews <= 65535 && width > 0 && height > 0, "gp_views_visible_lists: bad view count / image size");
    GP_CHECK_ARG(n * (int64_t)nviews < (int64_t)INT32_MAX, "gp_views_visible_lists: n * views must stay below 2^31");
    GpCarver cv(workspace, workspace_bytes);
    int32_t *flags = cv.take<int32_t>(n * nviews), *sc = cv.take<int32_t>(n * nviews);
    size_t tb = views_scan_tmp(n * nviews);
    char *tmp = cv.take<char>(tb);
    if (!cv.ok()) { gp_set_error("gp_views_visible_lists: workspace too small"); return GP_ENOMEM; }
    hipStream_t s = gp_stream(stream_);
    dim3 grid((unsigned)((n + 255) / 256), (unsigned)nviews);
    views_flags_kernel<<<grid, 256, 0, s>>>(coords, n, params, depth, width, height, cut_bound, vis_thres, flags);
    GP_CHECK_HIP(rocprim::exclusive_scan(tmp, tb, flags, sc, (int32_t)0, (size_t)(n * nviews), rocprim::plus<int32_t>(), s));
    views_compact_kernel<<<grid, 256, 0, s>>>(coords, n, nviews, params, depth, width, height, cut_bound, vis_thres, sc, ent_pt, ent_x,
                                              ent_y, ent_view, view_off);
    views_keep_kernel<<<(nviews + 255) / 256, 256, 0, s>>>(view_off, nviews, min_visible, val_keep, keep);
    GP_CHECK_LAUNCH();
    return GP_OK;
}

extern "C" int gp_render_depth_f64(const double *coords, int64_t n, const double *w2c_host, double fx, double fy, double cx,
                                   double cy, int32_t width, int32_t height, int32_t cut_bound, double *depth,
                                   void *stream_) {
    GP_CHECK_ARG(coords && w2c_host && depth && n > 0, "gp_render_depth_f64: null/empty argument");
    GP_CHECK_ARG(width > 0 && height > 0, "gp_render_depth_f64: bad image size %dx%d", width, height);
    Mat44 M;
    for (int a = 0; a < 4; ++a)
        for (int k = 0; k < 4; ++k) M.m[a][k] = w2c_host[a * 4 + k];
    hipStream_t s = gp_stream(stream_);
    int64_t px = (int64_t)width * height;
    depth_fill_kernel<<<(int)((px + 255) / 256), 256, 0, s>>>(depth, px);
    render_depth_kernel<<<(int)((n + 255) / 256), 256, 0, s>>>(coords, n, M, fx, fy, cx, cy, width, height, cut_bound, depth);
    GP_CHECK_LAUNCH();
    return GP_OK;
}
```

geopurify_amd/ops.py:

```python
import ctypes

import numpy as np
import torch

from . import _lib
from ._lib import check


def _ptr(t):
    return ctypes.c_void_p(t.data_ptr()) if t is not None else None


def _stream():
    return ctypes.c_void_p(torch.cuda.current_stream().cuda_stream)


def _ws(nbytes, device):
    return torch.empty(max(int(nbytes), 256), dtype=torch.uint8, device=device)


def _chk(t, dtype, name):
    if t.dtype != dtype or not t.is_cuda or not t.is_contiguous():
        raise ValueError(f"{name}: expected contiguous CUDA {dtype}, got {t.dtype} cuda={t.is_cuda} contig={t.is_contiguous()}")
    return t


READBACK = {"seconds": 0.0, "calls": 0}


def readback(t):
    import time
    t0 = time.perf_counter()
    v = t.tolist()
    READBACK["seconds"] += time.perf_counter() - t0
    READBACK["calls"] += 1
    return v


def _dbl16(m):
    a = np.ascontiguousarray(np.asarray(m, dtype=np.float64).reshape(16))
    return (ctypes.c_double * 16)(*a.tolist())


def voxelize(coords, rigid):
    lib = _lib.load()
    _chk(coords, torch.float64, "coords")
    n = coords.shape[0]
    dev = coords.device
    ws = _ws(lib.gp_voxelize_workspace_bytes(n), dev)
    ca = torch.empty((n, 3), dtype=torch.float64, device=dev)
    inds = torch.empty(n, dtype=torch.int64, device=dev)
    inv = torch.empty(n, dtype=torch.int64, device=dev)
    order = torch.empty(n, dtype=torch.int64, device=dev)
    seg = torch.empty(n + 1, dtype=torch.int64, device=dev)
    nvd = torch.zeros(1, dtype=torch.int64, device=dev)
    check(lib.gp_voxelize_f64(_ptr(coords), n, _dbl16(rigid), _ptr(ca), _ptr(inds), _ptr(inv), _ptr(nvd),
                              _ptr(order), _ptr(seg), _ptr(ws), ws.numel(), _stream()), "gp_voxelize_f64")
    nv = int(readback(nvd)[0])
    return {"coords_aug": ca[:nv], "inds": inds[:nv], "inds_reconstruct": inv, "order": order,
            "seg_start": seg[:nv + 1], "nv": nv}


def fnv_hash(coords):
    lib = _lib.load()
    _chk(coords, torch.float64, "coords")
    out = torch.empty(coords.shape[0], dtype=torch.int64, device=coords.device)
    check(lib.gp_fnv_hash_f64(_ptr(coords), coords.shape[0], _ptr(out), _stream()), "gp_fnv_hash_f64")
    return out


def project_points(coords, w2c, fx, fy, cx, cy, depth, width, height, cut_bound, vis_thres, want_weight=False):
    lib = _lib.load()
    _chk(coords, torch.float64, "coords")
    n = coords.shape[0]
    if depth is not None:
        _chk(depth, torch.float64, "depth")
        assert depth.shape == (height, width)
    mapping = torch.empty((n, 3), dtype=torch.int64, device=coords.device)
    weight = torch.empty(n, dtype=torch.float64, device=coords.device) if want_weight else None
    check(lib.gp_project_points_f64(_ptr(coords), n, _dbl16(w2c), float(fx), float(fy), float(cx), float(cy),
                                    _ptr(depth), int(width), int(height), int(cut_bound), float(vis_thres),
                                    _ptr(mapping), _ptr(weight), _stream()), "gp_project_points_f64")
    return (mapping, weight) if want_weight else mapping


def render_depth(coords, w2c, fx, fy, cx, cy, width, height, cut_bound):
    lib = _lib.load()
    _chk(coords, torch.float64, "coords")
    depth = torch.empty((height, width), dtype=torch.float64, device=coords.device)
    check(lib.gp_render_depth_f64(_ptr(coords), coords.shape[0], _dbl16(w2c), float(fx), float(fy), float(cx), float(cy),
                                  int(width), int(height), int(cut_bound), _ptr(depth), _stream()), "gp_render_depth_f64")
    return depth


def minmax_i32(coords):
    lib = _lib.load()
    _chk(coords, torch.int32, "coords")
    mm = torch.empty(6, dtype=torch.int32, device=coords.device)
    check(lib.gp_minmax_i32(_ptr(coords), coords.shape[0], _ptr(mm), _stream()), "gp_minmax_i32")
    return mm


def morton_order(coords_i32):
    lib = _lib.load()
    _chk(coords_i32, torch.int32, "coords")
    nv = coords_i32.shape[0]
    dev = coords_i32.device
    ws = _ws(lib.gp_morton_order_workspace_bytes(nv), dev)
    perm = torch.empty(nv, dtype=torch.int32, device=dev)
    rank = torch.empty(nv, dtype=torch.int32, device=dev)
    check(lib.gp_morton_order(_ptr(coords_i32), nv, _ptr(perm), _ptr(rank), _ptr(ws), ws.numel(), _stream()),
          "gp_morton_order")
    return perm, rank


class Grid:

    def __init__(self, buf, origin, extent, nv):
        self.buf, self.origin, self.extent, self.nv = buf, origin, extent, nv

    def status(self):
        return int(self.buf[36:40].view(torch.int32).item())


def grid_build(coords_sorted, origin=None, extent=None):
    lib = _lib.load()
    _chk(coords_sorted, torch.int32, "coords")
    nv = coords_sorted.shape[0]
    if origin is None or extent is None:
        lo = coords_sorted.amin(0)
        hi = coords_sorted.amax(0)
        lohi = torch.stack([lo, hi]).cpu().tolist()
        origin = lohi[0]
        extent = [lohi[1][a] - lohi[0][a] + 1 for a in range(3)]
    o = (ctypes.c_int32 * 3)(*[int(v) for v in origin])
    e = (ctypes.c_int32 * 3)(*[int(v) for v in extent])
    nbytes = lib.gp_grid_bytes(nv, e)
    if nbytes == 0:
        raise _lib.GeoPurifyHipError("gp_grid_bytes: invalid extent")
    buf = _ws(nbytes, coords_sorted.device)
    check(lib.gp_grid_build(_ptr(coords_sorted), nv, o, e, _ptr(buf), buf.numel(), _stream()), "gp_grid_build")
    return Grid(buf, list(origin), list(extent), nv)


def kernel_map_build(grid, coords_sorted):
    lib = _lib.load()
    nv = coords_sorted.shape[0]
    nm = torch.empty((27, nv), dtype=torch.int32, device=coords_sorted.device)
    check(lib.gp_kernel_map_build(_ptr(grid.buf), _ptr(coords_sorted), nv, _ptr(nm), _stream()), "gp_kernel_map_build")
    return nm


def coords_order_batched(coords_b):
    lib = _lib.load()
    _chk(coords_b, torch.int32, "coords")
    if coords_b.dim() != 2 or coords_b.shape[1] != 4:
        raise ValueError(f"coords_order_batched: expected [nv, 4], got {list(coords_b.shape)}")
    nv = coords_b.shape[0]
    dev = coords_b.device
    ws = _ws(lib.gp_coords_order_batched_workspace_bytes(nv), dev)
    perm = torch.empty(nv, dtype=torch.int32, device=dev)
    rank = torch.empty(nv, dtype=torch.int32, device=dev)
    keys = torch.empty(nv, dtype=torch.int64, device=dev)
    status = torch.empty(3, dtype=torch.int32, device=dev)
    check(lib.gp_coords_order_batched(_ptr(coords_b), nv, _ptr(perm), _ptr(rank), _ptr(keys), _ptr(status), _ptr(ws), ws.numel(),
                                      _stream()), "gp_coords_order_batched")
    return perm, rank, keys, status


def kernel_map_sorted(keys_sorted):
    lib = _lib.load()
    _chk(keys_sorted, torch.int64, "keys")
    nv = keys_sorted.shape[0]
    nm = torch.empty((27, nv), dtype=torch.int32, device=keys_sorted.device)
    check(lib.gp_kernel_map_sorted(_ptr(keys_sorted), nv, _ptr(nm), _stream()), "gp_kernel_map_sorted")
    return nm


class QuantizedIndex:

    def __init__(self, n, nv, coordinates, unique_index, inverse, order, seg_start, bad_batch, bad_axes):
        self.n, self.nv, self.coordinates, self.unique_index, self.inverse = n, nv, coordinates, unique_index, inverse
        self.order, self.seg_start, self.bad_batch, self.bad_axes = order, seg_start, bad_batch, bad_axes
        self.counts = seg_start[1:] - seg_start[:-1]


QUANTIZE_OUTPUTS = {"vox_coords": (torch.int32, lambda n: (n, 4)), "unique_index": (torch.int64, lambda n: (n,)),
                    "inverse": (torch.int64, lambda n: (n,)), "order": (torch.int64, lambda n: (n,)),
                    "seg_start": (torch.int64, lambda n: (n + 1,)), "status": (torch.int32, lambda n: (3,))}


def quantize_batched(coords_b, buffers=None):
    lib = _lib.load()
    _chk(coords_b, torch.int32, "coords")
    if coords_b.dim() != 2 or coords_b.shape[1] != 4:
        raise ValueError(f"quantize_batched: expected [n, 4], got {list(coords_b.shape)}")
    n = coords_b.shape[0]
    if not 0 < n < 2 ** 31:
        raise ValueError(f"quantize_batched: n={n} out of range (1 .. 2^31 - 1)")
    dev = coords_b.device
    b = {}
    for name, (dtype, shape) in QUANTIZE_OUTPUTS.items():
        t = (buffers or {}).get(name)
        if t is None:
            t = torch.empty(shape(n), dtype=dtype, device=dev)
        elif _chk(t, dtype, name).shape != shape(n) or t.device != dev:
            raise ValueError(f"quantize_batched: buffer {name} must be {list(shape(n))} on {dev}, got {list(t.shape)} on {t.device}")
        b[name] = t
    ws = _ws(lib.gp_quantize_batched_workspace_bytes(n), dev)
    check(lib.gp_quantize_batched(_ptr(coords_b), n, _ptr(b["vox_coords"]), _ptr(b["unique_index"]), _ptr(b["inverse"]),
                                  _ptr(b["order"]), _ptr(b["seg_start"]), _ptr(b["status"]), _ptr(ws), ws.numel(), _stream()),
          "gp_quantize_batched")
    nv, bad_batch, bad_axes = readback(b["status"])
    return QuantizedIndex(n, nv, b["vox_coords"][:nv], b["unique_index"][:nv], b["inverse"], b["order"], b["seg_start"][:nv + 1],
                     bad_batch, bad_axes)


SEGMENT_LABEL_RULES = {"first": 0, "differ": 1, "count": 2}


def segment_labels(labels, q, ignore_label, rule, out=None):
    lib = _lib.load()
    if rule not in SEGMENT_LABEL_RULES:
        raise ValueError(f"segment_labels: rule={rule!r}, expected one of {sorted(SEGMENT_LABEL_RULES)}")
    _chk(labels, torch.int64, "labels")
    if labels.dim() != 1 or labels.shape[0] != q.n:
        raise ValueError(f"segment_labels: expected labels [{q.n}], got {list(labels.shape)}")
    if labels.device != q.order.device:
        raise ValueError(f"segment_labels: labels on {labels.device}, the quantisation on {q.order.device}")
    if out is None:
        out = torch.empty(q.nv, dtype=torch.int64, device=labels.device)
    elif _chk(out, torch.int64, "out").shape != (q.nv,) or out.device != labels.device:
        raise ValueError(f"segment_labels: expected out [{q.nv}], got {list(out.shape)}")
    check(lib.gp_segment_labels(_ptr(labels), q.n, _ptr(q.order), _ptr(q.seg_start), _ptr(q.unique_index), q.nv, int(ignore_label),
                                SEGMENT_LABEL_RULES[rule], _ptr(out), _stream()), "gp_segment_labels")
    return out


def scatter_mean_csr(src, d, order, seg_start, nv, out, col0=0, row_map=None):
    lib = _lib.load()
    _chk(src, torch.float32, "src")
    check(lib.gp_scatter_mean_csr(_ptr(src), src.stride(0), int(d), _ptr(order), _ptr(seg_start), int(nv),
                                  _ptr(row_map), _ptr(out), out.stride(0), int(col0), _stream()),
          "gp_scatter_mean_csr")
    return out


def voxel_rows_operands(f, d, geo, dg, order, seg_start, nv, cin_pad, row_map=None, want_scale=True):
    lib = _lib.load()
    _chk(f, torch.float32, "f")
    _chk(geo, torch.float32, "geo")
    dev = f.device
    X = torch.empty((nv, cin_pad), dtype=torch.float32, device=dev)
    rows = torch.empty((nv, 2 * cin_pad), dtype=torch.float16, device=dev)
    rinv = torch.empty(nv, dtype=torch.float32, device=dev)
    sc = torch.empty(2, dtype=torch.float32, device=dev) if want_scale else None
    ws = _ws(256, dev) if want_scale else None
    check(lib.gp_voxel_rows_operands(_ptr(f), f.stride(0), int(d), _ptr(geo), geo.stride(0), int(dg), _ptr(order), _ptr(seg_start), int(nv),
                                     _ptr(row_map), _ptr(X), X.stride(0), int(cin_pad), _ptr(rows), rows.stride(0), _ptr(rinv), _ptr(sc),
                                     _ptr(ws), ws.numel() if ws is not None else 0, _stream()), "gp_voxel_rows_operands")
    return X, (rows, None, rinv), sc


def gather_rows(src, d, index, out=None, row_map=None):
    lib = _lib.load()
    n = index.shape[0]
    if out is None:
        out = torch.empty((n, d), dtype=torch.float32, device=src.device)
    check(lib.gp_gather_rows(_ptr(src), src.stride(0), int(d), _ptr(index), n, _ptr(row_map), _ptr(out),
                             out.stride(0), _stream()), "gp_gather_rows")
    return out


def gather_rows_classify(src, d, index, text_norm, logit_scale, row_map=None):
    lib = _lib.load()
    n = index.shape[0]
    out = torch.empty((n, d), dtype=torch.float32, device=src.device)
    pred = torch.empty(n, dtype=torch.int64, device=src.device)
    zero = torch.empty(n, dtype=torch.uint8, device=src.device)
    check(lib.gp_gather_rows_classify(_ptr(src), src.stride(0), int(d), _ptr(index), n, _ptr(row_map), _ptr(out), out.stride(0),
                                      _ptr(text_norm), int(text_norm.shape[0]), float(logit_scale), _ptr(pred), _ptr(zero), _stream()),
          "gp_gather_rows_classify")
    return out, pred, zero


def can_gather_rows_classify(d, num_classes):
    return d % 64 == 0 and d <= 1024 and num_classes * d * 4 <= 64 * 1024


def pool_cs_width_ok(d):
    return d % 256 == 0 and 256 <= d <= 1024


def sparse_conv(x, nbr_map, w, scale=None, shift=None, residual=None, relu=False, out=None):
    lib = _lib.load()
    nv = x.shape[0]
    if w.dim() == 3:
        kv, cin, cout = w.shape
    else:
        kv, (cin, cout) = 1, w.shape
    _chk(w, torch.float32, "w")
    if out is None:
        out = torch.empty((nv, cout), dtype=torch.float32, device=x.device)
    check(lib.gp_sparse_conv(_ptr(x), x.stride(0), _ptr(nbr_map) if kv > 1 else None, nv, _ptr(w), int(kv),
                             int(cin), int(cout), _ptr(scale), _ptr(shift), _ptr(residual),
                             residual.stride(0) if residual is not None else 0, int(bool(relu)), _ptr(out),
                             out.stride(0), _stream()), "gp_sparse_conv")
    return out


class ConvPairs:

    def __init__(self, pair_in, pair_pos, seg_off, tile_start, nseg, num_pairs, nv):
        self.pair_in, self.pair_pos, self.pair_off, self.tile_start = pair_in, pair_pos, seg_off, tile_start
        self.nseg, self.num_pairs, self.nv = nseg, num_pairs, nv
        self.partial = None
        self.num_chunks, self.chunk_row_off, self.chunk_tile_off, self.chunk_pair_off = 0, None, None, None

    def _set_chunks(self, rows, tiles, pairs):
        n = len(rows) - 1
        self.num_chunks = n
        self.chunk_row_off = (ctypes.c_int32 * (n + 1))(*rows)
        self.chunk_tile_off = (ctypes.c_int32 * (n + 1))(*tiles)
        self.chunk_pair_off = (ctypes.c_int32 * (n + 1))(*pairs)
        self.max_chunk_pairs = max(pairs[i + 1] - pairs[i] for i in range(n))

    def regroup(self, g):
        g = max(1, min(int(g), max(self.num_chunks, 1)))
        cp = ConvPairs(self.pair_in, self.pair_pos, self.pair_off, self.tile_start, self.nseg, self.num_pairs, self.nv)
        cp.tile_desc = self.tile_desc
        n = self.num_chunks
        idx = list(range(0, n, g)) + [n]
        ro, po, to = list(self.chunk_row_off), list(self.chunk_pair_off), list(self.chunk_tile_off)
        cp._set_chunks([ro[i] for i in idx], [to[i] for i in idx], [po[i] for i in idx])
        return cp


CONV_TARGET_TILES = None


def conv_pairs_build(nbr_map, chunk_rows="balanced", col_tiles=2):
    lib = _lib.load()
    kv, nv = nbr_map.shape
    dev = nbr_map.device
    if isinstance(chunk_rows, str):
        if chunk_rows != "balanced":
            raise ValueError(f"conv_pairs_build: chunk_rows={chunk_rows!r}")
    if isinstance(chunk_rows, str):
        granule = 256
        max_chunks = (nv + granule - 1) // granule
        plan = torch.empty(max_chunks + 2, dtype=torch.int32, device=dev)
        ws = _ws(lib.gp_conv_chunk_plan_workspace_bytes(nv, granule), dev)
        target = CONV_TARGET_TILES or 3 * torch.cuda.get_device_properties(dev).multi_processor_count - 16
        check(lib.gp_conv_chunk_plan(_ptr(nbr_map), nv, kv, granule, int(col_tiles), int(target), max_chunks, _ptr(plan),
                                     _ptr(plan[max_chunks + 1:]), _ptr(ws), ws.numel(), _stream()), "gp_conv_chunk_plan")
        host = readback(plan)
        nchunks = host[max_chunks + 1]
        rows = host[:nchunks + 1]
        row_off = plan[:nchunks + 1]
    else:
        ch = nv if chunk_rows is None else max(int(chunk_rows), 256)
        rows = list(range(0, nv, ch)) + [nv]
        nchunks = len(rows) - 1
        row_off = torch.tensor(rows, dtype=torch.int32, device=dev)
    nseg = nchunks * kv
    ws = _ws(lib.gp_conv_pairs_workspace_bytes(nv, kv), dev)
    pair_in = torch.empty(kv * nv, dtype=torch.int32, device=dev)
    pair_pos = torch.empty((kv, nv), dtype=torch.int32, device=dev)
    seg_off = torch.empty(nseg + 1, dtype=torch.int32, device=dev)
    tile_start = torch.empty(nseg + 1, dtype=torch.int32, device=dev)
    tile_desc = torch.empty(((kv * nv) // 256 + nseg + 1, 4), dtype=torch.int32, device=dev)
    check(lib.gp_conv_pairs_build(_ptr(nbr_map), nv, kv, nchunks, _ptr(row_off), _ptr(pair_in), _ptr(pair_pos), _ptr(seg_off),
                                  _ptr(tile_start), _ptr(tile_desc), _ptr(ws), ws.numel(), _stream()), "gp_conv_pairs_build")
    bounds = readback(torch.stack([seg_off[::kv], tile_start[::kv]]))
    num_pairs = bounds[0][-1]
    cp = ConvPairs(pair_in, pair_pos, seg_off, tile_start, nseg, num_pairs, nv)
    cp.tile_desc = tile_desc
    cp._set_chunks(rows, bounds[1], bounds[0])
    return cp


def conv_weights_split(w, scale_pow2, blocked=None, transpose_flip=False):
    lib = _lib.load()
    kv, cin, cout = w.shape
    if transpose_flip:
        if cout % 32 == 0 and cin % 256 == 0 and blocked is not False:
            hi = torch.empty((kv, cin // 256, cout // 32, 256, 32), dtype=torch.float16, device=w.device)
            lo = torch.empty_like(hi)
            check(lib.gp_conv_weights_split_blocked(_ptr(w), kv, cout, cin, float(scale_pow2), _ptr(hi), _ptr(lo), 1, _stream()),
                  "gp_conv_weights_split_blocked")
            return hi, lo
        return conv_weights_split(w.flip(0).transpose(1, 2).contiguous(), scale_pow2, blocked)
    if blocked is None:
        blocked = cin % 32 == 0 and cout % 256 == 0
    if blocked:
        hi = torch.empty((kv, cout // 256, cin // 32, 256, 32), dtype=torch.float16, device=w.device)
        lo = torch.empty_like(hi)
        check(lib.gp_conv_weights_split_blocked(_ptr(w), kv, cin, cout, float(scale_pow2), _ptr(hi), _ptr(lo), 0, _stream()),
              "gp_conv_weights_split_blocked")
        return hi, lo
    hi = torch.empty((kv, cout, cin), dtype=torch.float16, device=w.device)
    lo = torch.empty((kv, cout, cin), dtype=torch.float16, device=w.device)
    check(lib.gp_conv_weights_split(_ptr(w), kv, cin, cout, float(scale_pow2), _ptr(hi), _ptr(lo), _stream()),
          "gp_conv_weights_split")
    return hi, lo


def conv_weights_shape(w_hi):
    if w_hi.dim() == 5:
        return int(w_hi.shape[0]), int(w_hi.shape[1]) * 256, int(w_hi.shape[2]) * 32
    return tuple(int(v) for v in w_hi.shape)


def split_f16(x, d=None, scale=None, per_row=False, interleaved=False, dst_row=None, extra_zero_rows=0):
    lib = _lib.load()
    d = x.shape[1] if d is None else d
    if interleaved:
        assert per_row and d % 32 == 0, "interleaved rows are the row-scaled operand of the convolution"
        rows = torch.empty((x.shape[0], 2 * d), dtype=torch.float16, device=x.device)
        rinv = torch.empty(x.shape[0], dtype=torch.float32, device=x.device)
        check(lib.gp_split_f16_scaled(_ptr(x), x.stride(0), int(d), x.shape[0], _ptr(rows), None, rows.stride(0), None, _ptr(rinv),
                                      _ptr(dst_row), _stream()), "gp_split_f16_scaled")
        return rows, None, rinv
    hi = torch.empty((x.shape[0] + extra_zero_rows, d), dtype=torch.float16, device=x.device)
    lo = torch.empty((x.shape[0] + extra_zero_rows, d), dtype=torch.float16, device=x.device)
    if extra_zero_rows:
        hi[x.shape[0]:].zero_()
        lo[x.shape[0]:].zero_()
    if scale is None and not per_row:
        if dst_row is not None:
            raise ValueError("split_f16: dst_row needs a scaled form (scale= or per_row=True)")
        check(lib.gp_split_f16(_ptr(x), x.stride(0), int(d), x.shape[0], _ptr(hi), _ptr(lo), hi.stride(0), _stream()),
              "gp_split_f16")
        return hi, lo
    rinv = torch.empty(x.shape[0], dtype=torch.float32, device=x.device) if per_row else None
    check(lib.gp_split_f16_scaled(_ptr(x), x.stride(0), int(d), x.shape[0], _ptr(hi), _ptr(lo), hi.stride(0), _ptr(scale),
                                  _ptr(rinv), _ptr(dst_row), _stream()), "gp_split_f16_scaled")
    return (hi, lo, rinv) if per_row else (hi, lo)


def rcb_order(coords_sorted, chunk_rows=1024, leaf_rows=128):
    lib = _lib.load()
    _chk(coords_sorted, torch.int32, "coords")
    nv = coords_sorted.shape[0]
    sigma = torch.empty(nv, dtype=torch.int32, device=coords_sorted.device)
    rho = torch.empty(nv, dtype=torch.int32, device=coords_sorted.device)
    check(lib.gp_rcb_order(_ptr(coords_sorted), nv, int(chunk_rows), int(leaf_rows), _ptr(sigma), _ptr(rho), _stream()), "gp_rcb_order")
    return sigma, rho


def rows_renumber(nbr, sigma, rho):
    lib = _lib.load()
    nv, k = nbr.shape
    out = torch.empty_like(nbr)
    check(lib.gp_rows_renumber_i32(_ptr(nbr), nv, int(k), _ptr(sigma), _ptr(rho), _ptr(out), _stream()), "gp_rows_renumber_i32")
    return out


def pow2_scale(x, d=None):
    lib = _lib.load()
    d = x.shape[1] if d is None else d
    out = torch.empty(2, dtype=torch.float32, device=x.device)
    ws = _ws(256, x.device)
    check(lib.gp_pow2_scale(_ptr(x), x.stride(0), int(d), x.shape[0], _ptr(out), _ptr(ws), ws.numel(), _stream()), "gp_pow2_scale")
    return out


def sparse_conv_f16x3(x, pairs, w_hi, w_lo, scale=None, shift=None, residual=None, relu=False, out=None,
                      x_split=None, out_split=None, x_row_inv=None, out_row_inv=None, want_f32=True, fp32_partials=False, dense_single_offset=False,
                      reference_walk=False):
    lib = _lib.load()
    res_planes = residual if isinstance(residual, (tuple, list)) else None
    if res_planes is not None:
        residual = None
    rh, rl, ri = (tuple(res_planes) + (None,))[:3] if res_planes is not None else (None, None, None)
    kv, cout, cin = conv_weights_shape(w_hi)
    w_blocked = int(w_hi.dim() == 5)
    nv = pairs.nv
    dev = w_hi.device
    if dense_single_offset:
        partial = torch.empty(64, dtype=torch.float32, device=dev)
    else:
        if pairs.partial is None or pairs.partial.shape[1] < cout or pairs.partial.shape[0] < max(pairs.max_chunk_pairs, 1):
            pairs.partial = torch.empty((max(pairs.max_chunk_pairs, 1), cout), dtype=torch.float32, device=dev)
        partial = pairs.partial
    if out is None and (want_f32 or out_split is None):
        out = torch.empty((nv, cout), dtype=torch.float32, device=dev)
    xh, xl = x_split if x_split is not None else (None, None)
    yh, yl = out_split if out_split is not None else (None, None)
    plane_flags = (1 if (xh is not None and xl is None) else 0) | (2 if (yh is not None and yl is None) else 0) | \
                  (4 if (rh is not None and rl is None) else 0) | (8 if fp32_partials else 0) | (16 if dense_single_offset else 0) | (32 if reference_walk else 0)
    check(lib.gp_sparse_conv_f16x3(_ptr(x), x.stride(0) if x is not None else 0, _ptr(xh), _ptr(xl),
                                   xh.stride(0) if xh is not None else 0, _ptr(pairs.pair_in), _ptr(pairs.pair_pos),
                                   _ptr(pairs.pair_off), _ptr(pairs.tile_start), _ptr(pairs.tile_desc), pairs.nseg, pairs.num_pairs, nv, kv, _ptr(w_hi), _ptr(w_lo), cin, cout,
                                   _ptr(partial), _ptr(scale), _ptr(shift), _ptr(residual),
                                   residual.stride(0) if residual is not None else 0, int(bool(relu)), _ptr(out),
                                   out.stride(0) if out is not None else 0, _ptr(yh), _ptr(yl), yh.stride(0) if yh is not None else 0,
                                   int(pairs.num_chunks), pairs.chunk_row_off, pairs.chunk_tile_off, pairs.chunk_pair_off,
                                   _ptr(x_row_inv), _ptr(out_row_inv), _ptr(rh), _ptr(rl), rh.stride(0) if rh is not None else 0, _ptr(ri),
                                   w_blocked, plane_flags, _stream()),
          "gp_sparse_conv_f16x3")
    return out


def interleave_planes(hi, lo):
    n, c = hi.shape
    return torch.stack([hi.reshape(n, c // 32, 32), lo.reshape(n, c // 32, 32)], dim=2).reshape(n, 2 * c).contiguous()


def deinterleave_planes(t):
    n, c2 = t.shape
    v = t.reshape(n, c2 // 64, 2, 32)
    return v[:, :, 0].reshape(n, c2 // 2).contiguous(), v[:, :, 1].reshape(n, c2 // 2).contiguous()


def l2norm_rows_(x, d=None):
    lib = _lib.load()
    d = x.shape[1] if d is None else d
    check(lib.gp_l2norm_rows(_ptr(x), x.stride(0), int(d), x.shape[0], _stream()), "gp_l2norm_rows")
    return x


def embed_head_f16x3(x_split, w_hi, w_lo, out_scale, x_row_inv=None, normalize=True, out=None, planes=False, want_f32=True, plane_rows=None):
    lib = _lib.load()
    hi, lo = x_split
    cout, cin = w_hi.shape[-2:]
    nv = hi.shape[0]
    _chk(hi, torch.float16, "x_hi"), _chk(lo, torch.float16, "x_lo")
    if hi.stride(0) != lo.stride(0) or hi.shape[1] < cin:
        raise ValueError("embed_head_f16x3: the hi / lo planes must share a row stride and hold cin channels")
# ... 1331 lines not shown
```

geopurify_amd/pipeline.py:

```python
from dataclasses import dataclass, field
from typing import List, Optional

import numpy as np
import torch

from . import ops
from .bicubic import aa_bicubic_taps

GEO_DIM = 6
CONV_PAD = 32


def _pad_to(v, m):
    return (v + m - 1) // m * m


class StudentWeights:

    def __init__(self, state_dict, device, eps=1e-5, mode="f16x3", residual_from_planes=True, interleaved_rows=True, blocked_weights=True,
                 head="f16x3"):
        sd = {k: v.detach() for k, v in state_dict.items()}
        self.mode = mode
        self.residual_from_planes = bool(residual_from_planes)
        self.interleaved_rows = bool(interleaved_rows)
# ... 305 lines not shown
    if family is None:
        if (cs_ok or mfma_ok) and num_iters >= 3 and D in (256, 512, 768):
            return "cs" if cs_ok else "mfma"
        return "tiles" if tiles_ok else "ell"
    if family in ("cs", "chain"):
        if not cs_ok:
            raise ValueError(f"pool_mode='{mode}' needs D in (256, 512, 768, 1024) and K <= 96 (D={D}, K={K})")
        return "chain" if family == "chain" and num_iters >= 2 else "cs"
    if family in ("mfma", "mfma_persist") and not mfma_ok:
        raise ValueError(f"pool_mode='mfma' needs D == 512 and block_rows*K <= 16384 (D={D}, K={K})")
    if family == "tiles" and not tiles_ok:
        return "ell"
    return family


class HotPath:

    def __init__(self, student: StudentWeights, mask_shape, K=96, sharpen=20.0, num_iters=19, device="cuda",
                 pool_mode="auto", pool_tile_rows=8, pool_block_rows=64, batch_views=True, pool_structure_ahead=True, affinity_mfma=True,
                 all_views_max_pairs=2e11, pool_row_order="rcb"):
        self.student = student
        self.batch_views = batch_views
        self.all_views_max_pairs = float(all_views_max_pairs)
        self.pool_mode, self.pool_tile_rows, self.pool_block_rows = _known_pool_mode(pool_mode), pool_tile_rows, pool_block_rows
        self.pool_structure_ahead = bool(pool_structure_ahead)
        self.affinity_mfma = bool(affinity_mfma)
        self.pool_row_order = pool_row_order
        self.mask_shape = tuple(mask_shape)
        self.K, self.sharpen, self.num_iters = K, sharpen, num_iters
        self.device = torch.device(device)
        self._taps = {}
        self.stats = {}
        self.stage_mark = None
        self._chain_ops = []
        self.keep_lifted, self.last_lifted = False, None

    def _tap_tables(self, h, w):
        key = (h, w)
        if key not in self._taps:
            H, W = self.mask_shape
            tx0, twx = aa_bicubic_taps(w, W)
            ty0, twy = aa_bicubic_taps(h, H)
            d = self.device
            self._taps[key] = tuple(torch.from_numpy(a).to(d) for a in (tx0, twx, ty0, twy))
        return self._taps[key]

    def lift_masks(self, batch: SceneBatch, vlm):
        dev = self.device
        N = batch.scene_coords.shape[0]
        V = len(batch.views)
        has_img = batch.imgs is not None and batch.imgs.numel() > 0
        batched = ((not has_img or getattr(vlm, "ignores_image", False)) and torch.is_tensor(getattr(vlm, "mask_embed", None))
                   and vlm.mask_embed.dim() == 3 and vlm.mask_embed.is_contiguous())
        outs = None
        if batched:
            text_embed, logit_scale = vlm.text_embed, float(vlm.logit_scale)
            Q, D = vlm.mask_embed.shape[1:]
        else:
            outs = [vlm(v.src_view, image=batch.imgs[v.src_view]) if has_img else vlm(v.src_view) for v in batch.views]
            if V:
                text_embed, logit_scale = outs[0]["text_embed"].to(dev), float(outs[0]["logit_scale"])
                Q, D = outs[0]["mask_embed"].shape
            else:
                text_embed, logit_scale = vlm.text_embed, float(vlm.logit_scale)
                Q, D = 1, text_embed.shape[1]
        text_norm = torch.nn.functional.normalize(text_embed, dim=-1).contiguous()
        C = text_norm.shape[0]
        n_tab = vlm.mask_embed.shape[0] if batched else max(V, 1)
        f_seg = torch.empty((n_tab, Q, D), dtype=torch.float32, device=dev)
        l_seg = torch.empty((n_tab, Q, C), dtype=torch.float32, device=dev)
        if batched:
            ops.segment_tables(vlm.mask_embed.view(n_tab * Q, D), text_norm, logit_scale,
                               f_seg.view(n_tab * Q, D), l_seg.view(n_tab * Q, C))
        scores_all = None
        if batched and getattr(vlm, "pred_logits", None) is not None and vlm.pred_logits.dim() == 3:
            scores_all = torch.softmax(vlm.pred_logits, dim=-1)[..., :-1].max(-1).values.contiguous()
        ent = batch.ent
        pm_all = getattr(vlm, "pred_masks", None)
        all_views = (self.batch_views and batched and scores_all is not None and ent is not None and ent["total"] > 0
                     and ent["num_views"] <= 128 and ent.get("sum_nv2", float(ent["max_nv"]) ** 2 * ent["num_views"]) / 4 <= self.all_views_max_pairs
                     and torch.is_tensor(pm_all) and pm_all.dim() == 4 and pm_all.is_contiguous()
                     and pm_all.shape[0] >= ent["num_views"] and pm_all.shape[1] <= 1024)
        if all_views:
            _, start, pvv, pvs = ops.lift_masks_views(pm_all, scores_all, self._tap_tables(pm_all.shape[2], pm_all.shape[3]),
                                                      self.mask_shape, batch.scene_coords, ent, ent["total"], ent["num_views"])
            return self._fuse_and_fill(batch, start, pvv, pvs, f_seg, l_seg, D, text_norm, logit_scale)
        cnt = torch.zeros(N + 1, dtype=torch.int64, device=dev)
        segs = []
        ws_m = ws_n = None
        for i, v in enumerate(batch.views):
            out = vlm(v.src_view) if batched else outs[i]
            pm = out["pred_masks"].to(dev).contiguous()
            scores = scores_all[v.src_view] if scores_all is not None else \
                torch.softmax(out["pred_logits"].to(dev), dim=-1)[..., :-1].max(-1).values.contiguous()
            if ws_m is None:
                lib = ops._lib.load()
                ws_m = torch.empty(lib.gp_lift_masks_workspace_bytes(*pm.shape), dtype=torch.uint8, device=dev)
                ws_n = torch.empty(lib.gp_nn1_masked_workspace_bytes(N), dtype=torch.uint8, device=dev)
            seg = ops.lift_masks_view(pm, scores, self._tap_tables(pm.shape[1], pm.shape[2]), self.mask_shape,
                                      v.x, v.y, workspace=ws_m)
            xyz = batch.scene_coords[v.pt].contiguous()
            covered = (seg >= 0).to(torch.uint8)
            nn = ops.nn1_masked(xyz, covered, 1 - covered, workspace=ws_n)
            seg = torch.where(nn >= 0, seg[nn.clamp(min=0)], seg)
            if not batched:
                ops.segment_tables(out["mask_embed"].to(dev).contiguous(), text_norm, logit_scale, f_seg[i], l_seg[i])
            ops.pv_count(v.pt, cnt)
            segs.append(seg)
        start = ops.exclusive_scan_i64(cnt)
        total = sum(len(v.pt) for v in batch.views)
        cursor = torch.zeros(N, dtype=torch.int32, device=dev)
        pvv = torch.empty(max(total, 1), dtype=torch.int32, device=dev)
        pvs = torch.empty(max(total, 1), dtype=torch.int32, device=dev)
        for i, v in enumerate(batch.views):
            ops.pv_fill(v.pt, segs[i], v.src_view if batched else i, start, cursor, pvv, pvs)
        return self._fuse_and_fill(batch, start, pvv, pvs, f_seg, l_seg, D, text_norm if V else text_embed, logit_scale)

    def _fuse_and_fill(self, batch, start, pvv, pvs, f_seg, l_seg, D, text, logit_scale):
        dev = self.device
        N = batch.scene_coords.shape[0]
        F = torch.empty((N, D), dtype=torch.float32, device=dev)
        seen, unseen = ops.seen_masks(start, N)
        nn = ops.nn1_masked(batch.scene_coords, seen, unseen)
        ops.fuse_views_top3_fill(start, pvv, pvs, N, f_seg, l_seg, nn, F)
        return F, text, logit_scale

    def lift_dense(self, batch: SceneBatch, vlm: DenseFeatureVLM):
        dev = self.device
        N = batch.scene_coords.shape[0]
        D = vlm.feat.shape[1]
        s = torch.zeros((N, D), dtype=torch.float32, device=dev)
        cnt = torch.zeros(N, dtype=torch.float32, device=dev)
        for v in batch.views:
            ops.lift_dense_accum(vlm.feat[v.src_view], v.pt, v.x, v.y, s, cnt)
        seen = ops.lift_dense_finish(s, D, cnt)
        nn = ops.nn1_masked(batch.scene_coords, seen, 1 - seen)
        src = torch.where(nn >= 0, nn, torch.arange(N, device=dev))
        return ops.gather_rows(s, D, src), vlm.text_embed, vlm.logit_scale

    def lift_lseg(self, batch: SceneBatch, vlm: LSegFeatureVLM):
        dev = self.device
        N = batch.scene_coords.shape[0]
        D = vlm.feat_lo.shape[1]
        H, W = vlm.image_shape
        s = torch.zeros((N, D), dtype=torch.float32, device=dev)
        cnt = torch.zeros(N, dtype=torch.float32, device=dev)
        for v in batch.views:
            ops.lift_dense_bilinear_accum(vlm.feat_lo[v.src_view], H, W, v.pt, v.x, v.y, s, cnt)
        seen = ops.lift_dense_finish(s, D, cnt)
        nn = ops.nn1_masked(batch.scene_coords, seen, 1 - seen)
        src = torch.where(nn >= 0, nn, torch.arange(N, device=dev))
        return ops.gather_rows(s, D, src), vlm.text_embed, vlm.logit_scale

    def prepare(self, batch: SceneBatch, F):
        dev = self.device
        N, D = F.shape
        st = self.student
        assert st.cin == D + GEO_DIM, f"student expects {st.cin} input channels, lift gives {D}+{GEO_DIM}"
        coords = batch.scene_coords_3d.floor().to(torch.int32).contiguous()
        Nv = coords.shape[0]
        perm, rank = ops.morton_order(coords)
        cs = coords[perm.long()].contiguous()
        mark = self.stage_mark if self.stage_mark is not None else (lambda name: None)
        mark("morton order")
        if batch.order is None:
            order = torch.sort(batch.scene_inds_reconstruct, stable=True).indices
            segc = torch.zeros(Nv + 1, dtype=torch.int64, device=dev)
            segc[1:] = torch.bincount(batch.scene_inds_reconstruct, minlength=Nv).cumsum(0)
            batch.order, batch.seg_start = order, segc
        family = self._pool_family(D)
        xs = sc = None
        if st.one_pass_input(F, batch.scene_gauss_features):
            X, xs, sc = ops.voxel_rows_operands(F, D, batch.scene_gauss_features, GEO_DIM, batch.order, batch.seg_start, Nv, st.cin_pad,
                                                row_map=rank, want_scale=family in ("cs", "chain"))
        else:
            X = torch.zeros((Nv, st.cin_pad), dtype=torch.float32, device=dev)
            ops.scatter_mean_csr(F, D, batch.order, batch.seg_start, Nv, X, col0=0, row_map=rank)
            ops.scatter_mean_csr(batch.scene_gauss_features, GEO_DIM, batch.order, batch.seg_start, Nv, X, col0=D,
                                 row_map=rank)
        mark("scatter_mean")
        if batch.extent is not None:
            grid = ops.grid_build(cs, [0, 0, 0], batch.extent)
        else:
            grid = ops.grid_build(cs)
        nbr_map = ops.kernel_map_build(grid, cs)
        pairs = ops.conv_pairs_build(nbr_map, col_tiles=max(1, st.hidden // 256)) if any(l[0] == "f16x3" for l in st.layers) else None
        mark("grid+kernel_map")
        nbr = ops.knn_lattice(grid, cs, perm, self.K)
        mark("kNN")
        state = {"X": X, "rank": rank, "nbr_map": nbr_map, "pairs": pairs, "nbr": nbr, "Nv": Nv, "D": D, "pool": None,
                 "xs": xs if xs is not None else st.split_input(X)}
        if family in ("cs", "chain"):
            if sc is None:
                sc = ops.pow2_scale(X, D)
            how = self.pool_structure_ahead
            if how and self.affinity_mfma and self.K <= 96 and self.student is not None and self.student.embed == 128:
                how = "valid"
            rho = None
            nbr_op = nbr
            if how == "valid" and self.pool_row_order == "rcb" and Nv > 1024:
                sigma, rho = ops.rcb_order(cs, 1024, 128)
                nbr_op = ops.rows_renumber(nbr, sigma, rho)
                state["rank_pool"] = rho[rank.long()].contiguous()
            state["pool"] = {"op": ops.pool_cs_plan(nbr_op, structure=how), "sc": sc, "rho": rho, "nbr": nbr_op,
                             "x_split": ops.split_f16(X, D, scale=sc[0:1], dst_row=rho),
                             "pong": tuple(torch.empty((Nv, D), dtype=torch.float16, device=dev) for _ in range(2))}
            if family == "chain" and (state["pool"]["op"].dst is not None or state["pool"]["op"].valid is not None):
                ops.pool_cs_deps(state["pool"]["op"], D)
            mark("pool plan+split")
        return state

    def refine(self, batch: SceneBatch, F, after_student=None, prepared=None, classify_text=None):
        p = prepared if prepared is not None else self.prepare(batch, F)
        X, rank, nbr, Nv, D = p["X"], p["rank"], p["nbr"], p["Nv"], p["D"]
        mark = self.stage_mark if self.stage_mark is not None else (lambda name: None)
        op = p["pool"]["op"] if p["pool"] is not None else None
        mfma_aff = op is not None and op.valid is not None
        rho = p["pool"]["rho"] if (p["pool"] is not None and mfma_aff) else None
        E = self.student.forward(X, p["nbr_map"], p["pairs"], x_split=p.get("xs"), mark=self.stage_mark, planes=mfma_aff, plane_rows=rho)
        mark("embed head" if self.stage_mark is not None else "student")
        if after_student is not None:
            after_student()
        if mfma_aff:
            ops.affinity_cs_fragments(None, self.sharpen, op, planes=E)
            w = None
        else:
            w = ops.affinity_softmax(E, nbr, self.sharpen, into=op if op is not None and op.dst is not None else None)
        mark("affinity")
        self._last_E, self._last_E_rho = E, rho
        self._last_pool_inputs = (X, nbr, w, Nv, D)
        self._last_pool_plan = p["pool"]
        out = self._pool(X, nbr, w, Nv, D, plan=p["pool"])
        mark("pooling")
        self._fused_pred = None
        if classify_text is not None and ops.can_gather_rows_classify(D, classify_text[0].shape[0]) and classify_text[0].shape[0] <= 32:
            text_norm = torch.nn.functional.normalize(classify_text[0], dim=-1).contiguous()
            out, pred, zero = ops.gather_rows_classify(out, D, batch.scene_inds_reconstruct, text_norm, classify_text[1],
                                                       row_map=p.get("rank_pool", rank))
            self._fused_pred = (out, classify_text[0], pred, zero)
        else:
            out = ops.gather_rows(out, D, batch.scene_inds_reconstruct, row_map=p.get("rank_pool", rank))
        mark("gather")
        self.stats = {"Nv": Nv, "nbr_map": p["nbr_map"], "pool_bytes_per_iter": Nv * (2 * D * 4 + self.K * 8),
                      "pool_kernel": self._pool_kernel}
        return out

    def _pool_family(self, D):
        return resolve_pool_mode(self.pool_mode, D, self.K, self.num_iters, self.pool_tile_rows, self.pool_block_rows)

    def _pool(self, X, nbr, w, Nv, D, plan=None):
        dev = X.device
        family = self._pool_family(D)
        if w is None and (plan is None or not plan["op"].filled):
            E = self._last_E
            if isinstance(E, tuple):
                E = (E[0].float() + E[1].float()) / ops.AFFINITY_PLANE_SCALE
                if getattr(self, "_last_E_rho", None) is not None:
                    E = E[self._last_E_rho.long()]
            w = ops.affinity_softmax(E.contiguous(), nbr, self.sharpen)
        if self.num_iters == 0:
            out = torch.empty((Nv, D), dtype=torch.float32, device=dev)
            out.copy_(X[:, :D])
            self._pool_kernel = "none"
            return out
        if family in ("cs", "chain"):
            if plan is None:
                sc = ops.pow2_scale(X, D)
                plan = {"op": ops.pool_cs_plan(nbr), "sc": sc, "x_split": ops.split_f16(X, D, scale=sc[0:1]),
                        "pong": tuple(torch.empty((Nv, D), dtype=torch.float16, device=dev) for _ in range(2))}
            op = plan["op"] if plan["op"].filled else ops.pool_cs_fill(plan["op"], nbr, w)
            out = torch.empty((Nv, D), dtype=torch.float32, device=dev)
            sc = plan["sc"]
            sp = [plan["x_split"], plan["pong"]]
            if self.stage_mark is not None:
                self.stage_mark("pool operator fill")
            if family == "chain":
                if op.dep is None:
                    ops.pool_cs_deps(op, D)
                ops.pool_cs_apply_chain(sp[0], sp[1], op, D, self.num_iters, out, out_scale=sc[1:2])
                if op not in self._chain_ops:
                    self._chain_ops.append(op)
                self._pool_kernel = "cs_chain_kernel" if D == 512 else "cs_chain_ns_kernel"
                return out
            src = sp[0]
            for t in range(self.num_iters):
                last = t == self.num_iters - 1
                dst = None if last else sp[(t + 1) % 2]
                ops.pool_cs_apply(src, op, D, out_split=dst, out_f32=out if last else None, out_scale=sc[1:2] if last else None)
                src = dst
            self._pool_kernel = "cs_pool_kernel" if D == 512 else "cs_pool_ns_kernel"
            return out
        if family in ("mfma", "mfma_persist"):
            op = ops.pool_mfma_build(nbr, w, self.pool_block_rows, min_steps=9 if family == "mfma_persist" else 0)
            persistent = family == "mfma_persist" and op.min_steps >= 9 and self.pool_block_rows == 64
            rows = op.rows_padded if persistent else Nv
            out = torch.empty((rows, D), dtype=torch.float32, device=dev)
            sc = ops.pow2_scale(X, D)
            sp = [ops.split_f16(X, D, scale=sc[0:1]), tuple(torch.empty((rows, D), dtype=torch.float16, device=dev) for _ in range(2))]
            if persistent and self.num_iters > 1:
                sp.append(tuple(torch.empty((rows, D), dtype=torch.float16, device=dev) for _ in range(2)))
            apply = ops.pool_mfma_apply_persistent if persistent else ops.pool_mfma_apply
            src = sp[0]
            for t in range(self.num_iters):
                last = t == self.num_iters - 1
                dst = None if last else sp[1 + (t % 2)] if persistent else sp[(t + 1) % 2]
                apply(src, op, D, out_split=dst, out_f32=out if last else None, out_scale=sc[1:2] if last else None)
                src = dst
            self._pool_kernel = "pool_mfma_persist_kernel" if persistent else "pool_mfma_kernel"
            return out[:Nv]
        use_tiles = family == "tiles"
        tiles = ops.pool_tiles_build(nbr, w, self.pool_tile_rows) if use_tiles else None
        bufs = [torch.empty((Nv, D), dtype=torch.float32, device=dev) for _ in range(2)]
        cur = X
        for t in range(self.num_iters):
            if use_tiles:
                ops.pool_tiles_apply(cur, tiles, D, bufs[t % 2])
            else:
                ops.pool_ell(cur, nbr, w, D, bufs[t % 2])
            cur = bufs[t % 2]
        self._pool_kernel = ("pool_tiles64_kernel" if D == 64 else "pool_tiles_kernel") if use_tiles else "pool_ell_kernel"
        return cur

    def evaluate_scene(self, batch: SceneBatch, vlm):
        if isinstance(vlm, LSegFeatureVLM):
            F, text, scale = self.lift_lseg(batch, vlm)
        elif isinstance(vlm, DenseFeatureVLM):
            F, text, scale = self.lift_dense(batch, vlm)
        else:
            F, text, scale = self.lift_masks(batch, vlm)
        if self.keep_lifted:
            self.last_lifted = F
        feats = self.refine(batch, F)
        if self._chain_ops:
            self.pool_chain_check()
        return {"scene_features": feats, "text_features": text, "logit_scale": scale}

    def pool_chain_check(self, block=True):
        keep = []
        while self._chain_ops:
# ... 63 lines not shown
```

include/geopurify_hip.h:

```cpp
#ifndef GEOPURIFY_HIP_H
#define GEOPURIFY_HIP_H

#include <stddef.h>
#include <stdint.h>

#ifdef __cplusplus
extern "C" {
#endif

#define GP_OK 0
#define GP_EINVAL (-22)
#define GP_ENOMEM (-12)
#define GP_EHIP (-5)
#define GP_ERANGE (-34)

#define GP_KNN_MAX_K 127

int gp_version(void);
int gp_debug_set(int32_t key, int32_t value);
int gp_debug_ptr(int32_t key, void *device_buffer, size_t bytes);
const char *gp_last_error(void);

size_t gp_voxelize_workspace_bytes(int64_t n);
int gp_voxelize_f64(const double *coords, int64_t n, const double *rigid_host,
                    double *coords_aug, int64_t *inds, int64_t *inds_reconstruct, int64_t *nv_dev,
                    int64_t *order, int64_t *seg_start,
                    void *workspace, size_t workspace_bytes, void *stream);
int gp_fnv_hash_f64(const double *coords, int64_t n, uint64_t *hash, void *stream);

int gp_project_points_f64(const double *coords, int64_t n, const double *w2c_host,
                          double fx, double fy, double cx, double cy,
                          const double *depth, int32_t width, int32_t height,
                          int32_t cut_bound, double vis_thres,
                          int64_t *mapping, double *weight, void *stream);
int gp_render_depth_f64(const double *coords, int64_t n, const double *w2c_host,
                        double fx, double fy, double cx, double cy, int32_t width, int32_t height,
                        int32_t cut_bound, double *depth, void *stream);

int gp_minmax_i32(const int32_t *coords, int64_t nv, int32_t *mm, void *stream);
size_t gp_morton_order_workspace_bytes(int64_t nv);
int gp_morton_order(const int32_t *coords, int64_t nv, int32_t *perm, int32_t *rank,
                    void *workspace, size_t workspace_bytes, void *stream);
size_t gp_grid_bytes(int64_t nv, const int32_t *extent_host);
int gp_grid_build(const int32_t *coords, int64_t nv, const int32_t *origin_host,
                  const int32_t *extent_host, void *grid, size_t grid_bytes, void *stream);

int gp_scatter_mean_csr(const float *src, int64_t ld_src, int32_t d, const int64_t *order,
                        const int64_t *seg_start, int64_t nv, const int32_t *row_map,
                        float *out, int64_t ld_out, int32_t col0, void *stream);
int gp_gather_rows(const float *src, int64_t ld_src, int32_t d, const int64_t *index, int64_t n,
                   const int32_t *row_map, float *out, int64_t ld_out, void *stream);

int gp_kernel_map_build(const void *grid, const int32_t *coords, int64_t nv, int32_t *nbr_map,
                        void *stream);
size_t gp_coords_order_batched_workspace_bytes(int64_t nv);
int gp_coords_order_batched(const int32_t *coords, int64_t nv, int32_t *perm, int32_t *rank, uint64_t *keys_sorted,
                            int32_t *status, void *workspace, size_t workspace_bytes, void *stream);
size_t gp_quantize_batched_workspace_bytes(int64_t n);
int gp_quantize_batched(const int32_t *coords, int64_t n, int32_t *vox_coords, int64_t *unique_index, int64_t *inverse,
                        int64_t *order, int64_t *seg_start, int32_t *status, void *workspace, size_t workspace_bytes,
                        void *stream);
int gp_segment_labels(const int64_t *labels, int64_t n, const int64_t *order, const int64_t *seg_start,
                      const int64_t *unique_index, int64_t nv, int64_t ignore_label, int32_t rule, int64_t *out, void *stream);
int gp_kernel_map_sorted(const uint64_t *keys_sorted, int64_t nv, int32_t *nbr_map, void *stream);
int gp_sparse_conv(const float *x, int64_t ld_x, const int32_t *nbr_map, int64_t nv,
                   const float *w, int32_t kv, int32_t cin, int32_t cout,
                   const float *scale, const float *shift, const float *residual, int64_t ld_res,
                   int32_t relu, float *y, int64_t ld_y, void *stream);
int gp_sparse_conv_tiles(int32_t *tiles);
size_t gp_conv_pairs_workspace_bytes(int64_t nv, int32_t kv);
int gp_conv_pairs_build(const int32_t *nbr_map, int64_t nv, int32_t kv, int32_t num_chunks, const int32_t *chunk_row_off,
                        int32_t *pair_in, int32_t *pair_pos, int32_t *seg_off, int32_t *tile_start,
                        int32_t *tile_desc ,
                        void *workspace, size_t workspace_bytes, void *stream);
size_t gp_conv_chunk_plan_workspace_bytes(int64_t nv, int32_t granule_rows);
int gp_conv_chunk_plan(const int32_t *nbr_map, int64_t nv, int32_t kv, int32_t granule_rows, int32_t col_tiles,
                       int32_t target_tiles, int32_t max_chunks, int32_t *chunk_row_off, int32_t *n_chunks, void *workspace,
                       size_t workspace_bytes, void *stream);
int gp_conv_weights_split(const float *w, int32_t kv, int32_t cin, int32_t cout, float scale_pow2,
                          void *w_hi, void *w_lo, void *stream);
int gp_split_f16(const float *x, int64_t ld_x, int32_t d, int64_t n, void *hi, void *lo, int64_t ld_h,
                 void *stream);
int gp_pow2_scale(const float *x, int64_t ld_x, int32_t d, int64_t n, float *scale2, void *workspace,
                  size_t workspace_bytes, void *stream);
int gp_split_f16_scaled(const float *x, int64_t ld_x, int32_t d, int64_t n, void *hi, void *lo, int64_t ld_h,
                        const float *scale, float *row_inv_scale, const int32_t *dst_row, void *stream);
int gp_voxel_rows_operands(const float *f, int64_t ld_f, int32_t d, const float *geo, int64_t ld_geo, int32_t dg,
                           const int64_t *order, const int64_t *seg_start, int64_t nv, const int32_t *row_map, float *x,
                           int64_t ld_x, int32_t cin_pad, void *rows, int64_t ld_rows, float *row_inv_scale, float *scale2,
                           void *workspace, size_t workspace_bytes, void *stream);
int gp_sparse_conv_f16x3(const float *x, int64_t ld_x, const void *x_hi, const void *x_lo, int64_t ld_xh,
                         const int32_t *pair_in, const int32_t *pair_pos,
                         const int32_t *seg_off, const int32_t *tile_start, const int32_t *tile_desc,
                         int32_t nseg, int64_t num_pairs, int64_t nv, int32_t kv,
                         const void *w_hi, const void *w_lo, int32_t cin, int32_t cout, float *partial,
                         const float *scale, const float *shift, const float *residual, int64_t ld_res,
                         int32_t relu, float *y, int64_t ld_y, void *y_hi, void *y_lo, int64_t ld_yh,
                         int32_t num_chunks, const int32_t *chunk_row_off_host, const int32_t *chunk_tile_off_host,
                         const int32_t *chunk_pair_off_host, const float *x_row_inv_scale, float *y_row_inv_scale,
                         const void *res_hi, const void *res_lo, int64_t ld_rh, const float *res_row_inv_scale, int32_t w_blocked,
                         int32_t plane_flags, void *stream);
int gp_conv_weights_split_blocked(const float *w, int32_t kv, int32_t cin, int32_t cout, float scale_pow2,
                                  void *w_hi, void *w_lo, int32_t transpose_flip, void *stream);
int gp_l2norm_rows(float *x, int64_t ld, int32_t d, int64_t n, void *stream);
int gp_embed_head_f16x3(const void *x_hi, const void *x_lo, int64_t ld_x, const float *x_row_inv_scale, const void *w_hi,
                        const void *w_lo, int64_t nv, int32_t cin, int32_t cout, float out_scale, int32_t l2_normalize,
                        float *y, int64_t ld_y, void *e_hi, void *e_lo, float plane_scale,
                        const int32_t *e_dst_row ,
                        void *stream);

int gp_rcb_order(const int32_t *coords, int64_t nv, int32_t chunk_rows, int32_t leaf_rows, int32_t *sigma, int32_t *rho, void *stream);
int gp_rows_renumber_i32(const int32_t *nbr, int64_t nv, int32_t k, const int32_t *sigma, const int32_t *rho, int32_t *out,
                         void *stream);

size_t gp_knn_workspace_bytes(int64_t nv);
int gp_knn_lattice(const void *grid, const int32_t *coords, const int32_t *ids, int64_t nv,
                   int32_t k, int32_t *nbr, void *workspace, size_t workspace_bytes, void *stream);
int gp_knn_lattice_two_pass(const void *grid, const int32_t *coords, const int32_t *ids, int64_t nv,
                            int32_t k, int32_t *nbr, void *workspace, size_t workspace_bytes, void *stream);
size_t gp_knn_batched_workspace_bytes(int64_t nv);
int gp_knn_batched(const uint64_t *keys_sorted, const int32_t *ids, int64_t nv, int32_t k, int32_t *nbr, int32_t *status,
                   void *workspace, size_t workspace_bytes, void *stream);

int gp_affinity_softmax(const float *e, int64_t ld_e, int32_t d, const int32_t *nbr, int32_t k,
                        int64_t nv, float sharpen, float *w, void *stream);
int gp_affinity_softmax_scatter(const float *e, int64_t ld_e, int32_t d, const int32_t *nbr, int32_t k, int64_t nv,
                                float sharpen, float *w, const int32_t *dst, void *wa_hi, void *wa_lo, void *stream);

int gp_pool_ell(const float *x, int64_t ld_x, const int32_t *nbr, const float *w, int32_t k,
                int64_t nv, int32_t d, float *y, int64_t ld_y, void *stream);

size_t gp_pool_transpose_workspace_bytes(int64_t nv, int32_t k);
int gp_pool_transpose_build(const int32_t *nbr, int64_t nv, int32_t k, int64_t *tr_off, int32_t *tr_slot, void *workspace,
                            size_t workspace_bytes, void *stream);
int gp_pool_ell_transpose(const float *g, int64_t ld_g, const int64_t *tr_off, const int32_t *tr_slot, const float *w, int32_t k,
                          int64_t nv, int32_t d, float *out, int64_t ld_out, void *stream);
int gp_pool_ell_wgrad(const float *g, int64_t ld_g, const float *x_prev, int64_t ld_x, const int32_t *nbr, int32_t k, int64_t nv,
                      int32_t d, float *dw, int32_t accumulate, void *stream);
size_t gp_affinity_softmax_backward_workspace_bytes(int64_t nv, int32_t k);
int gp_affinity_softmax_backward(const float *e_unit, int64_t ld_e, int32_t d, const int32_t *nbr, const float *w, const float *dw,
                                 int32_t k, int64_t nv, float sharpen, const int64_t *tr_off, const int32_t *tr_slot, float *de_unit,
                                 int64_t ld_de, void *workspace, size_t workspace_bytes, void *stream);
int gp_l2norm_rows_backward(const float *e_raw, int64_t ld_e, const float *de_unit, int64_t ld_du, int32_t d, int64_t n,
                            float *de_raw, int64_t ld_de, void *stream);

size_t gp_pool_tiles_workspace_bytes(int64_t nv, int32_t r);
int gp_pool_tiles_count(const int32_t *nbr, int64_t nv, int32_t k, int32_t r, int64_t *tile_off,
                        void *workspace, size_t workspace_bytes, void *stream);
int gp_pool_tiles_fill(const int32_t *nbr, const float *w, int64_t nv, int32_t k, int32_t r,
                       const int64_t *tile_off, int32_t *u_row, float *u_w, void *stream);
int gp_pool_tiles_apply(const float *x, int64_t ld_x, const int64_t *tile_off, const int32_t *u_row,
                        const float *u_w, int32_t r, int64_t nv, int32_t d, float *y, int64_t ld_y,
                        void *stream);

size_t gp_pool_mfma_workspace_bytes(int64_t nv, int32_t block_rows);
int gp_pool_mfma_count(const int32_t *nbr, int64_t nv, int32_t k, int32_t block_rows, int32_t min_steps,
                       int64_t *bu_off, int32_t *bu_n, void *workspace, size_t workspace_bytes, void *stream);
int gp_pool_mfma_fill(const int32_t *nbr, const float *w, int64_t nv, int32_t k, int32_t block_rows,
                      const int64_t *bu_off, const int32_t *bu_n, int64_t total_rows, int32_t *bu_row,
                      void *wa_hi, void *wa_lo, void *stream);
int gp_pool_mfma_apply(const void *x_hi, const void *x_lo, int64_t ld_x, const int64_t *bu_off,
                       const int32_t *bu_row, const void *wa_hi, const void *wa_lo, int64_t nv, int32_t d,
                       int32_t block_rows, void *y_hi, void *y_lo, int64_t ld_y, float *y_f32,
                       int64_t ld_yf, const float *out_scale, void *stream);
int gp_pool_mfma_apply_persistent(const void *x_hi, const void *x_lo, int64_t ld_x, const int64_t *bu_off,
                                  const int32_t *bu_row, const void *wa_hi, const void *wa_lo, int64_t nv,
                                  int32_t d, int32_t block_rows, int32_t min_steps, void *y_hi, void *y_lo,
                                  int64_t ld_y, float *y_f32, int64_t ld_yf, int64_t y_rows,
                                  const float *out_scale, uint32_t *queue, void *stream);

size_t gp_pool_cs_workspace_bytes(int64_t nv, int32_t rows_per_block);
int gp_pool_cs_count(const int32_t *nbr, int64_t nv, int32_t k, int32_t rows_per_block, int64_t *bu_off, int32_t *bu_n,
                     int64_t *max_union, void *workspace, size_t workspace_bytes, void *stream);
int gp_pool_cs_fill(const int32_t *nbr, const float *w, int64_t nv, int32_t k, int32_t rows_per_block, const int64_t *bu_off,
                    int64_t total_rows, int32_t max_union, int32_t *bu_row, uint32_t *bu_mask, void *wa_hi, void *wa_lo, void *stream);
int gp_pool_cs_structure(const int32_t *nbr, int64_t nv, int32_t k, int32_t rows_per_block, const int64_t *bu_off,
                         int64_t total_rows, int32_t max_union, int32_t *bu_row, uint32_t *bu_mask, void *wa_hi, void *wa_lo,
                         int32_t *dst, void *stream);
int gp_pool_cs_structure_valid(const int32_t *nbr, int64_t nv, int32_t k, int32_t rows_per_block, const int64_t *bu_off,
                               int64_t total_rows, int32_t max_union, int32_t *bu_row, uint32_t *bu_mask, uint32_t *bu_valid,
                               void *stream);
int gp_affinity_cs_fragments(const void *e_hi, const void *e_lo, int64_t nv, int32_t d, int32_t k, float sharpen,
                             const int64_t *bu_off, const int32_t *bu_row, const uint32_t *bu_mask, const uint32_t *bu_valid,
                             int32_t rows_per_block, void *wa_hi, void *wa_lo, void *stream);
int gp_pool_cs_apply(const void *x_hi, const void *x_lo, int64_t ld_x, const int64_t *bu_off, const int32_t *bu_row,
                     const uint32_t *bu_mask, const void *wa_hi, const void *wa_lo, int64_t nv, int32_t d,
                     int32_t rows_per_block, void *y_hi, void *y_lo, int64_t ld_y, float *y_f32, int64_t ld_yf,
                     const float *out_scale, void *stream);
int gp_pool_cs_deps(const int64_t *bu_off, const int32_t *bu_row, int64_t nv, int32_t rows_per_block, int32_t *dep,
                    int32_t *scratch, void *stream);
size_t gp_pool_cs_chain_flag_words(int64_t nv, int32_t rows_per_block);
size_t gp_pool_cs_chain_flag_words_d(int64_t nv, int32_t rows_per_block, int32_t d);
int gp_pool_cs_apply_chain(void *x_hi, void *x_lo, void *p_hi, void *p_lo, int64_t ld, const int64_t *bu_off,
                           const int32_t *bu_row, const uint32_t *bu_mask, const void *wa_hi, const void *wa_lo, int64_t nv,
                           int32_t d, int32_t rows_per_block, int32_t applications, float *y_f32, int64_t ld_yf,
                           const float *out_scale, const int32_t *dep, uint32_t *flags, uint32_t epoch, void *stream);

int gp_lift_dense_accum(const float *feat2d, int32_t d, int32_t height, int32_t width,
                        const int64_t *pt, const int64_t *x, const int64_t *y, int64_t n_v,
                        float *sum, int64_t ld_sum, float *cnt, void *stream);
int gp_lift_dense_bilinear_accum(const float *feat, int32_t d, int32_t h, int32_t w, int32_t out_h, int32_t out_w,
                                 const int64_t *pt, const int64_t *x, const int64_t *y, int64_t n_v,
                                 float *sum, int64_t ld_sum, float *cnt, void *stream);
int gp_lift_dense_finish(float *sum, int64_t ld_sum, int32_t d, const float *cnt, int64_t n,
                         uint8_t *seen, void *stream);
size_t gp_lift_masks_workspace_bytes(int32_t q, int32_t h, int32_t w);
int gp_lift_masks_view(const float *pred_masks, int32_t q, int32_t h, int32_t w,
                       const float *scores, const int32_t *tap_x0, const float *tap_wx,
                       const int32_t *tap_y0, const float *tap_wy, int32_t out_h, int32_t out_w,
                       const int64_t *x, const int64_t *y, int64_t n_v, int32_t *seg,
                       float *seg_logit, void *workspace, size_t workspace_bytes, void *stream);
size_t gp_lift_masks_views_workspace_bytes(int32_t nsrc, int32_t q, int32_t h, int32_t w, int64_t total, int64_t n,
                                           int64_t fill_cap);
int gp_lift_masks_views(const float *pred_masks, int32_t nsrc, int32_t q, int32_t h, int32_t w, const float *scores,
                        const int32_t *tap_x0, const float *tap_wx, const int32_t *tap_y0, const float *tap_wy,
                        int32_t out_h, int32_t out_w, const float *xyz, int64_t n, const int64_t *ent_pt,
                        const int64_t *ent_x, const int64_t *ent_y, const int32_t *ent_view, const int64_t *view_off,
                        const uint8_t *keep, int32_t nviews, int64_t total, int64_t fill_cap, int32_t *seg, int64_t *pv_start,
                        int32_t *pv_view, int32_t *pv_seg, void *workspace, size_t workspace_bytes, void *stream);
int gp_segment_tables(const float *mask_embed, int32_t q, int32_t d, const float *text_norm,
                      int32_t c, float logit_scale, float *f_seg, float *logit_seg, void *stream);
int gp_pv_count(const int64_t *pt, int64_t n_v, int64_t *cnt, void *stream);
size_t gp_scan_workspace_bytes(int64_t n);
int gp_exclusive_scan_i64(const int64_t *in, int64_t n, int64_t *out, void *workspace,
                          size_t workspace_bytes, void *stream);
int gp_pv_fill(const int64_t *pt, const int32_t *seg, int64_t n_v, int32_t view,
               const int64_t *pv_start, int32_t *cursor, int32_t *pv_view, int32_t *pv_seg,
// ... 166 lines not shown
```

Before: 47.73.

## Replace Morton radix sort with counting sort; add counted pair build and RCB binning

Adds a counting-sort Morton ordering that histograms voxels into 8^3 cells, scans the counts and ranks each voxel by popcount over per-cell occupancy bits. This avoids the radix sort and the separate gather of sorted coordinates. Conv pair construction gets a counted path that reuses the chunk-plan counts, and the ordering's status readback is folded into an existing readback, with a fallback to the sorted path when the check fails. The RCB kernel gains wave-level min/max reductions and an in-shared-memory histogram binning partition. In exchange there are more kernels, larger workspaces and a possible re-run of prepare.

Result: no change. 47.71 (-0.0%).

```diff
diff --git a/geopurify_amd/_lib.py b/geopurify_amd/_lib.py
--- a/geopurify_amd/_lib.py
+++ b/geopurify_amd/_lib.py
@@ -23,6 +23,8 @@
     "gp_minmax_i32": (c_int32, [_P, c_int64, _P, _P]),
     "gp_morton_order_workspace_bytes": (c_size_t, [c_int64]),
     "gp_morton_order": (c_int32, [_P, c_int64, _P, _P, _P, c_size_t, _P]),
+    "gp_morton_order_counted_workspace_bytes": (c_size_t, [c_int64, POINTER(c_int32), POINTER(c_int32)]),
+    "gp_morton_order_counted": (c_int32, [_P, c_int64, POINTER(c_int32), POINTER(c_int32), _P, _P, _P, _P, _P, c_size_t, _P]),
     "gp_grid_bytes": (c_size_t, [c_int64, POINTER(c_int32)]),
     "gp_grid_build": (c_int32, [_P, c_int64, POINTER(c_int32), POINTER(c_int32), _P, c_size_t, _P]),
     "gp_scatter_mean_csr": (c_int32, [_P, c_int64, c_int32, _P, _P, c_int64, _P, _P, c_int64, c_int32, _P]),
@@ -38,6 +40,8 @@
                                  c_int64, c_int32, _P, c_int64, _P]),
     "gp_conv_pairs_workspace_bytes": (c_size_t, [c_int64, c_int32]),
     "gp_conv_pairs_build": (c_int32, [_P, c_int64, c_int32, c_int32, _P, _P, _P, _P, _P, _P, _P, c_size_t, _P]),
+    "gp_conv_pairs_build_counted_workspace_bytes": (c_size_t, [c_int64, c_int32, c_int32]),
+    "gp_conv_pairs_build_counted": (c_int32, [_P, c_int64, c_int32, c_int32, _P, _P, _P, _P, _P, _P, _P, _P, c_size_t, _P]),
     "gp_conv_chunk_plan_workspace_bytes": (c_size_t, [c_int64, c_int32]),
     "gp_conv_chunk_plan": (c_int32, [_P, c_int64, c_int32, c_int32, c_int32, c_int32, c_int32, _P, _P, _P, c_size_t, _P]),
     "gp_conv_weights_split": (c_int32, [_P, c_int32, c_int32, c_int32, c_float, _P, _P, _P]),
diff --git a/geopurify_amd/csrc/order_grid.hip b/geopurify_amd/csrc/order_grid.hip
--- a/geopurify_amd/csrc/order_grid.hip
+++ b/geopurify_amd/csrc/order_grid.hip
@@ -93,6 +93,7 @@
     if (bad) { atomicOr(&h->status, 1); return; }
     if (head) {
         int slot = atomicAdd(&h->ncells, 1);
+        if (slot >= h->max_cells) { atomicOr(&h->status, 1); return; }
         GpCellRec &r = recs[slot];
         r.start = (int32_t)i;
         r.count = 0;
@@ -127,6 +128,166 @@
         for (int dy = -1; dy <= 1; ++dy)
             for (int dx = -1; dx <= 1; ++dx, ++k)
                 nbr_map[(int64_t)k * nv + i] = (k == 13) ? (int32_t)i : g.lookup_rel(rx + dx, ry + dy, rz + dz);
+}
+
+
+struct McParams { int32_t origin[3], extent[3], nb[3]; };
+constexpr int MC_MAX_BITS = 21;
+constexpr int MC_SCAN = 2048;
+
+__device__ __forceinline__ uint32_t mc_code(uint32_t cx, uint32_t cy, uint32_t cz, const McParams &p) {
+    uint32_t code = 0, pos = 0;
+    const uint32_t c[3] = {cx, cy, cz};
+#pragma unroll
+    for (int b = 0; b < 12; ++b)
+#pragma unroll
+        for (int a = 0; a < 3; ++a)
+            if (b < p.nb[a]) { code |= ((c[a] >> b) & 1u) << pos; ++pos; }
+    return code;
+}
+__device__ __forceinline__ bool mc_rel(const int32_t *__restrict__ c, int64_t i, const McParams &p, int rel[3]) {
+    bool ok = true;
+#pragma unroll
+    for (int a = 0; a < 3; ++a) {
+        const int64_t r = (int64_t)c[i * 3 + a] - p.origin[a];
+        ok = ok && r >= 0 && r < p.extent[a];
+        rel[a] = (int)r;
+    }
+    return ok;
+}
+__global__ void mc_count_kernel(const int32_t *__restrict__ c, int64_t nv, McParams p, uint32_t *__restrict__ cnt, int32_t *__restrict__ st) {
+    const int64_t i = blockIdx.x * (int64_t)blockDim.x + threadIdx.x;
+    int rel[3] = {1, 1, 1};
+    const bool ok = i < nv ? mc_rel(c, i, p, rel) : true;
+    int zero = 0;
+#pragma unroll
+    for (int a = 0; a < 3; ++a) zero |= (__ballot(i < nv && ok && rel[a] == 0) != 0ull) << a;
+    if (gp_lane() == 0 && zero) atomicOr(&st[1], zero);
+    if (i >= nv) return;
+    if (!ok) { atomicOr(&st[0], 1); return; }
+    atomicAdd(&cnt[mc_code(rel[0] >> 3, rel[1] >> 3, rel[2] >> 3, p)], 1u);
+}
+__device__ __forceinline__ unsigned long long mc_block_scan(unsigned long long v, unsigned long long *s_w , unsigned long long &total) {
+    const int lane = threadIdx.x & 63, wave = threadIdx.x >> 6;
+    unsigned long long inc = v;
+    for (int o = 1; o < 64; o <<= 1) { const unsigned long long t = __shfl_up(inc, o, 64); if (lane >= o) inc += t; }
+    __syncthreads();
+    if (lane == 63) s_w[wave] = inc;
+    __syncthreads();
+    unsigned long long before = inc - v;
+    for (int w = 0; w < wave; ++w) before += s_w[w];
+    total = s_w[0] + s_w[1] + s_w[2] + s_w[3];
+    return before;
+}
+__global__ void __launch_bounds__(256)
+mc_sums_kernel(const uint32_t *__restrict__ cnt, int64_t ncells, unsigned long long *__restrict__ bsum) {
+    __shared__ unsigned long long s_w[4];
+    const int64_t e0 = blockIdx.x * (int64_t)MC_SCAN + threadIdx.x * 8;
+    unsigned long long v = 0;
+#pragma unroll
+    for (int j = 0; j < 8; ++j) { const uint32_t k = e0 + j < ncells ? cnt[e0 + j] : 0u; v += ((unsigned long long)(k != 0) << 32) | k; }
+    unsigned long long total;
+    mc_block_scan(v, s_w, total);
+    if (threadIdx.x == 0) bsum[blockIdx.x] = total;
+}
+__global__ void __launch_bounds__(256)
+mc_sums_scan_kernel(unsigned long long *__restrict__ bsum, int nblk) {
+    __shared__ unsigned long long s_w[4];
+    unsigned long long carry = 0;
+    for (int b0 = 0; b0 < nblk; b0 += 256) {
+        const int b = b0 + threadIdx.x;
+        const unsigned long long v = b < nblk ? bsum[b] : 0ull;
+        unsigned long long total;
+        const unsigned long long before = mc_block_scan(v, s_w, total);
+        if (b < nblk) bsum[b] = carry + before;
+        carry += total;
+    }
+}
+__global__ void __launch_bounds__(256)
+mc_prefix_kernel(const uint32_t *__restrict__ cnt, int64_t ncells, const unsigned long long *__restrict__ bsum, unsigned long long *__restrict__ pre,
+                 uint4 *__restrict__ occ ) {
+    __shared__ unsigned long long s_w[4];
+    const int64_t e0 = blockIdx.x * (int64_t)MC_SCAN + threadIdx.x * 8;
+    uint32_t k[8];
+    unsigned long long v = 0;
+#pragma unroll
+    for (int j = 0; j < 8; ++j) { k[j] = e0 + j < ncells ? cnt[e0 + j] : 0u; v += ((unsigned long long)(k[j] != 0) << 32) | k[j]; }
+    unsigned long long total;
+    unsigned long long run = bsum[blockIdx.x] + mc_block_scan(v, s_w, total);
+#pragma unroll
+    for (int j = 0; j < 8; ++j) {
+        if (k[j]) {
+            pre[e0 + j] = run;
+            uint4 *o = occ + (run >> 32) * 4;
+            o[0] = o[1] = o[2] = o[3] = make_uint4(0u, 0u, 0u, 0u);
+        }
+        run += ((unsigned long long)(k[j] != 0) << 32) | k[j];
+    }
+}
+__global__ void mc_occupy_kernel(const int32_t *__restrict__ c, int64_t nv, McParams p, const unsigned long long *__restrict__ pre,
+                                 uint32_t *__restrict__ occ, int32_t *__restrict__ st) {
+    const int64_t i = blockIdx.x * (int64_t)blockDim.x + threadIdx.x;
+    if (i >= nv || st[0] != 0) return;
+    int rel[3];
+    mc_rel(c, i, p, rel);
+    const uint32_t slot = (uint32_t)(pre[mc_code(rel[0] >> 3, rel[1] >> 3, rel[2] >> 3, p)] >> 32);
+    const uint32_t l = gp_local9(rel[0], rel[1], rel[2]), bit = 1u << (l & 31);
+    if (atomicOr(&occ[(int64_t)slot * 16 + (l >> 5)], bit) & bit) atomicOr(&st[2], 1);
+}
+__global__ void mc_rank_kernel(const int32_t *__restrict__ c, int64_t nv, McParams p, const unsigned long long *__restrict__ pre,
+                               const uint32_t *__restrict__ occ, const int32_t *__restrict__ st, int32_t *__restrict__ perm,
+                               int32_t *__restrict__ rank, int32_t *__restrict__ sorted ,
+                               int32_t *__restrict__ status) {
+    const int64_t i = blockIdx.x * (int64_t)blockDim.x + threadIdx.x;
+    if (i >= nv) return;
+    const bool bad = st[0] != 0 || st[1] != 7 || st[2] != 0;
+    if (i == 0) status[0] = bad ? 1 : 0;
+    int64_t r = i;
+    if (!bad) {
+        int rel[3];
+        mc_rel(c, i, p, rel);
+        const unsigned long long e = pre[mc_code(rel[0] >> 3, rel[1] >> 3, rel[2] >> 3, p)];
+        const uint32_t *bits = occ + (int64_t)(uint32_t)(e >> 32) * 16;
+        const uint32_t l = gp_local9(rel[0], rel[1], rel[2]), wi = l >> 5;
+        r = (int64_t)(uint32_t)e + __popc(bits[wi] & ((1u << (l & 31)) - 1u));
+        for (uint32_t j = 0; j < wi; ++j) r += __popc(bits[j]);
+    }
+    perm[r] = (int32_t)i;
+    rank[i] = (int32_t)r;
+    if (sorted) { sorted[r * 3] = c[i * 3]; sorted[r * 3 + 1] = c[i * 3 + 1]; sorted[r * 3 + 2] = c[i * 3 + 2]; }
+}
+
+struct McLayout { McParams p; int64_t ncells, nblk, nslots; bool ok; };
+McLayout mc_layout(int64_t nv, const int32_t *origin, const int32_t *extent) {
+    McLayout L;
+    L.ok = false;
+    if (!origin || !extent || nv <= 0 || nv >= (1ll << 31)) return L;
+    int bits = 0;
+    for (int a = 0; a < 3; ++a) {
+        if (extent[a] <= 0 || extent[a] > (1 << 15)) return L;
+        L.p.origin[a] = origin[a];
+        L.p.extent[a] = extent[a];
+        int nb = 0;
+        while ((((int64_t)extent[a] - 1) >> 3) >> nb) ++nb;
+        L.p.nb[a] = nb;
+        bits += nb;
+    }
+    if (bits > MC_MAX_BITS) return L;
+    L.ncells = (int64_t)1 << bits;
+    L.nblk = (L.ncells + MC_SCAN - 1) / MC_SCAN;
+    L.nslots = nv < L.ncells ? nv : L.ncells;
+    L.ok = true;
+    return L;
+}
+struct McWs { int32_t *st; uint32_t *cnt; unsigned long long *bsum, *pre; uint32_t *occ; };
+McWs mc_carve(GpCarver &cv, const McLayout &L) {
+    McWs w;
+    w.st = cv.take<int32_t>(64);
+    w.cnt = cv.take<uint32_t>((size_t)L.ncells);
+    w.occ = cv.take<uint32_t>((size_t)L.nslots * 16);
+    w.bsum = cv.take<unsigned long long>((size_t)L.nblk);
+    w.pre = cv.take<unsigned long long>((size_t)L.ncells);
+    return w;
 }
 
 }
@@ -179,6 +340,35 @@
     return GP_OK;
 }
 
+extern "C" size_t gp_morton_order_counted_workspace_bytes(int64_t nv, const int32_t *origin_host, const int32_t *extent_host) {
+    const McLayout L = mc_layout(nv, origin_host, extent_host);
+    if (!L.ok) return 0;
+    GpCarver cv(nullptr, 0);
+    mc_carve(cv, L);
+    return cv.off;
+}
+extern "C" int gp_morton_order_counted(const int32_t *coords, int64_t nv, const int32_t *origin_host, const int32_t *extent_host,
+                                       int32_t *perm, int32_t *rank, int32_t *coords_sorted, int32_t *status, void *workspace,
+                                       size_t workspace_bytes, void *stream_) {
+    GP_CHECK_ARG(coords && perm && rank && status && workspace, "gp_morton_order_counted: null argument");
+    const McLayout L = mc_layout(nv, origin_host, extent_host);
+    GP_CHECK_ARG(L.ok, "gp_morton_order_counted: nv, or an extent outside 1..32768, or a cell table above 2^%d entries: sort (gp_morton_order)", MC_MAX_BITS);
+    GpCarver cv(workspace, workspace_bytes);
+    const McWs w = mc_carve(cv, L);
+    if (!cv.ok()) { gp_set_error("gp_morton_order_counted: workspace too small (%zu < %zu)", workspace_bytes, cv.off); return GP_ENOMEM; }
+    hipStream_t s = gp_stream(stream_);
+    const int blocks = (int)((nv + 255) / 256);
+    GP_CHECK_HIP(hipMemsetAsync(w.st, 0, (size_t)((char *)w.occ - (char *)w.st), s));
+    mc_count_kernel<<<blocks, 256, 0, s>>>(coords, nv, L.p, w.cnt, w.st);
+    mc_sums_kernel<<<(unsigned)L.nblk, 256, 0, s>>>(w.cnt, L.ncells, w.bsum);
+    mc_sums_scan_kernel<<<1, 256, 0, s>>>(w.bsum, (int)L.nblk);
+    mc_prefix_kernel<<<(unsigned)L.nblk, 256, 0, s>>>(w.cnt, L.ncells, w.bsum, w.pre, reinterpret_cast<uint4 *>(w.occ));
+    mc_occupy_kernel<<<blocks, 256, 0, s>>>(coords, nv, L.p, w.pre, w.occ, w.st);
+    mc_rank_kernel<<<blocks, 256, 0, s>>>(coords, nv, L.p, w.pre, w.occ, w.st, perm, rank, coords_sorted, status);
+    GP_CHECK_LAUNCH();
+    return GP_OK;
+}
+
 static void grid_layout(int64_t nv, const int32_t *extent, int3 &cdim, int32_t &max_cells, int64_t &ci_off,
                         int64_t &rec_off, size_t &total) {
     cdim = make_int3(((extent[0] - 1) >> 3) + 1, ((extent[1] - 1) >> 3) + 1, ((extent[2] - 1) >> 3) + 1);
diff --git a/geopurify_amd/csrc/rcb.hip b/geopurify_amd/csrc/rcb.hip
--- a/geopurify_amd/csrc/rcb.hip
+++ b/geopurify_amd/csrc/rcb.hip
@@ -4,9 +4,15 @@
 
 constexpr int RCB_MAX_SEG = 32;
 
-template <int CH, int NT>
+template <int CH, int NT, int MAXB>
 __global__ void __launch_bounds__(NT)
-rcb_chunk_kernel(const int32_t *__restrict__ coords , int64_t nv, int leaf, int32_t *__restrict__ sigma, int32_t *__restrict__ rho) {
+rcb_chunk_kernel(const int32_t *__restrict__ coords , int64_t nv, int leaf, int32_t *__restrict__ sigma, int32_t *__restrict__ rho,
+                 int32_t *__restrict__ level_counts ) {
+    constexpr int NW = NT / 64, PW = CH / NW;
+    constexpr int BITS = 32 - __builtin_clz((unsigned)(MAXB - 1));
+    static_assert(PW % 64 == 0 && (MAXB * NW) % NT == 0, "rcb_chunk_kernel: shapes");
+    __shared__ int s_hist[MAXB * NW];
+    __shared__ int s_bin0[RCB_MAX_SEG], s_wsum[NW], s_nbins;
     __shared__ int s_c[3][CH];
     __shared__ unsigned s_key[CH];
     __shared__ unsigned short s_perm[2][CH];
@@ -39,12 +45,23 @@
             s_seg[i] = (unsigned char)sg;
         }
         __syncthreads();
-        for (int i = tid; i < n; i += NT) {
-            const int sg = s_seg[i];
-            if (s_len[sg] > leaf) {
-                const int r = s_perm[cur][i];
-#pragma unroll
-                for (int a = 0; a < 3; ++a) { atomicMin(&s_lo[sg][a], s_c[a][r]); atomicMax(&s_hi[sg][a], s_c[a][r]); }
+        for (int i0 = 0; i0 < CH; i0 += NT) {
+            const int i = i0 + tid;
+            const int sg = i < n ? s_seg[i] : -1;
+            const bool act = sg >= 0 && s_len[sg] > leaf;
+            int v[3] = {0, 0, 0};
+            if (act) { const int r = s_perm[cur][i]; v[0] = s_c[0][r]; v[1] = s_c[1][r]; v[2] = s_c[2][r]; }
+            const int sg0 = __builtin_amdgcn_readfirstlane(sg);
+            if (__all(sg == sg0 && act)) {
+#pragma unroll
+                for (int a = 0; a < 3; ++a) {
+                    int lo = v[a], hi = v[a];
+                    for (int o = 32; o > 0; o >>= 1) { lo = min(lo, __shfl_xor(lo, o, 64)); hi = max(hi, __shfl_xor(hi, o, 64)); }
+                    if (gp_lane() == 0) { atomicMin(&s_lo[sg0][a], lo); atomicMax(&s_hi[sg0][a], hi); }
+                }
+            } else if (act) {
+#pragma unroll
+                for (int a = 0; a < 3; ++a) { atomicMin(&s_lo[sg][a], v[a]); atomicMax(&s_hi[sg][a], v[a]); }
             }
         }
         __syncthreads();
@@ -59,6 +76,73 @@
             s_axis[tid] = ax;
         }
         __syncthreads();
+        if (tid == 0) {
+            int64_t nb = 0;
+            for (int sg = 0; sg < nseg; ++sg) {
+                s_bin0[sg] = (int)(nb < MAXB ? nb : MAXB);
+                const int ax = s_axis[sg];
+                nb += ax >= 0 ? (int64_t)s_hi[sg][ax] - s_lo[sg][ax] + 1 : 1;
+            }
+            s_nbins = (int)(nb <= MAXB ? nb : MAXB + 1);
+            if (level_counts) atomicAdd(&level_counts[nb <= MAXB ? 0 : 1], 1);
+        }
+        __syncthreads();
+        if (s_nbins <= MAXB) {
+            const int wave = tid >> 6, lane = tid & 63;
+            const int ne = s_nbins * NW;
+            for (int e = tid; e < ne; e += NT) s_hist[e] = 0;
+            __syncthreads();
+            int bin[PW / 64];
+#pragma unroll
+            for (int q = 0; q < PW / 64; ++q) {
+                const int i = wave * PW + q * 64 + lane;
+                bin[q] = -1;
+                if (i < n) {
+                    const int sg = s_seg[i], ax = s_axis[sg];
+                    bin[q] = s_bin0[sg] + (ax >= 0 ? s_c[ax][s_perm[cur][i]] - s_lo[sg][ax] : 0);
+                    atomicAdd(&s_hist[bin[q] * NW + wave], 1);
+                }
+            }
+            __syncthreads();
+            {
+                constexpr int PER = MAXB * NW / NT;
+                int acc = 0;
+#pragma unroll
+                for (int j = 0; j < PER; ++j) { const int e = tid * PER + j; acc += e < ne ? s_hist[e] : 0; }
+                int inc = acc;
+                for (int o = 1; o < 64; o <<= 1) { const int t = __shfl_up(inc, o, 64); if (lane >= o) inc += t; }
+                if (lane == 63) s_wsum[wave] = inc;
+                __syncthreads();
+                int run = inc - acc;
+                for (int w = 0; w < wave; ++w) run += s_wsum[w];
+#pragma unroll
+                for (int j = 0; j < PER; ++j) {
+                    const int e = tid * PER + j;
+                    if (e < ne) { const int c = s_hist[e]; s_hist[e] = run; run += c; }
+                }
+            }
+            __syncthreads();
+#pragma unroll
+            for (int q = 0; q < PW / 64; ++q) {
+                const int i = wave * PW + q * 64 + lane;
+                const bool act = bin[q] >= 0;
+                unsigned long long peers = __ballot(act);
+#pragma unroll
+                for (int b = 0; b < BITS; ++b) {
+                    const bool bit = (bin[q] >> b) & 1;
+                    const unsigned long long m = __ballot(act && bit);
+                    peers &= bit ? m : ~m;
+                }
+                if (act) {
+                    const int e = bin[q] * NW + wave;
+                    const int first = s_hist[e];
+                    const int before = __popcll(peers & ((1ull << lane) - 1ull));
+                    s_perm[cur ^ 1][first + before] = s_perm[cur][i];
+                    if ((peers >> lane) == 1ull) s_hist[e] = first + before + 1;
+                }
+                gp_wave_sync();
+            }
+        } else {
         for (int i = tid; i < CH; i += NT) {
             unsigned k = 0xffffffffu;
             if (i < n) {
@@ -83,8 +167,9 @@
                 }
                 __syncthreads();
             }
+        for (int i = tid; i < n; i += NT) s_perm[cur ^ 1][i] = s_perm[cur][s_key[i] & 0xfffu];
+        }
         ++level;
-        for (int i = tid; i < n; i += NT) s_perm[cur ^ 1][i] = s_perm[cur][s_key[i] & 0xfffu];
         cur ^= 1;
         if (tid == 0) {
             int ns = 0, more = 0;
@@ -135,8 +220,9 @@
     GP_CHECK_ARG(nv < ((int64_t)1 << 31), "gp_rcb_order: row ids are 32-bit");
     hipStream_t s = gp_stream(stream_);
     const unsigned blocks = (unsigned)((nv + chunk_rows - 1) / chunk_rows);
-    if (chunk_rows == 1024) rcb_chunk_kernel<1024, 256><<<blocks, 256, 0, s>>>(coords, nv, leaf_rows, sigma, rho);
-    else rcb_chunk_kernel<2048, 512><<<blocks, 512, 0, s>>>(coords, nv, leaf_rows, sigma, rho);
+    int32_t *lc = g_gp_debug_bytes[1] >= 2 * sizeof(int32_t) ? static_cast<int32_t *>(g_gp_debug_ptr[1]) : nullptr;
+    if (chunk_rows == 1024) rcb_chunk_kernel<1024, 256, 1024><<<blocks, 256, 0, s>>>(coords, nv, leaf_rows, sigma, rho, lc);
+    else rcb_chunk_kernel<2048, 512, 512><<<blocks, 512, 0, s>>>(coords, nv, leaf_rows, sigma, rho, lc);
     GP_CHECK_LAUNCH();
     return GP_OK;
 }
diff --git a/geopurify_amd/csrc/sparse_conv_v2.hip b/geopurify_amd/csrc/sparse_conv_v2.hip
--- a/geopurify_amd/csrc/sparse_conv_v2.hip
+++ b/geopurify_amd/csrc/sparse_conv_v2.hip
@@ -70,6 +70,83 @@
     if (gp_lane() == 0) s_c[threadIdx.x >> 6] = c;
     __syncthreads();
     if (threadIdx.x == 0) cnt[g * 32 + k] = s_c[0] + s_c[1] + s_c[2] + s_c[3];
+}
+constexpr int PG = 256;
+__device__ __forceinline__ bool pc_table_valid(const int32_t *__restrict__ R, int nchunks, int64_t nv) {
+    bool ok = true;
+    for (int c = threadIdx.x; c <= nchunks; c += blockDim.x) {
+        const int r = R[c];
+        if (c == 0) ok = ok && r == 0;
+        if (c == nchunks) ok = ok && r == nv;
+        else ok = ok && (r % PG) == 0 && r <= R[c + 1] && r >= 0;
+    }
+    return __syncthreads_and(ok);
+}
+__device__ __forceinline__ int pc_gran(const int32_t *__restrict__ R, int nchunks, int ngran, bool valid, int c) {
+    return c >= nchunks ? ngran : (valid ? R[c] / PG : 0);
+}
+__global__ void __launch_bounds__(256)
+pc_seg_sum_kernel(const int32_t *__restrict__ cnt, const int32_t *__restrict__ R, int nchunks, int kv, int64_t nv, int ngran,
+                  int32_t *__restrict__ segsum, int32_t *__restrict__ rel , int32_t *__restrict__ cid ) {
+    const bool valid = pc_table_valid(R, nchunks, nv);
+    const int sgi = blockIdx.x * 4 + (threadIdx.x >> 6), lane = gp_lane();
+    if (sgi >= nchunks * kv) return;
+    const int c = sgi / kv, k = sgi - c * kv;
+    const int g0 = pc_gran(R, nchunks, ngran, valid, c), g1 = pc_gran(R, nchunks, ngran, valid, c + 1);
+    int carry = 0;
+    for (int gb = g0; gb < g1; gb += 64) {
+        const int g = gb + lane;
+        const int a = g < g1 ? cnt[(int64_t)g * 32 + k] : 0;
+        int inc = a;
+        for (int o = 1; o < 64; o <<= 1) { const int t = __shfl_up(inc, o, 64); if (lane >= o) inc += t; }
+        if (g < g1) {
+            rel[(int64_t)g * 32 + k] = carry + inc - a;
+            if (k == 0) cid[g] = c;
+        }
+        carry += __shfl(inc, 63, 64);
+    }
+    if (lane == 0) segsum[sgi] = carry;
+}
+__global__ void __launch_bounds__(1024)
+pc_seg_scan_kernel(const int32_t *__restrict__ segsum, int nseg, int32_t *__restrict__ seg_off, int32_t *__restrict__ tile_start) {
+    __shared__ int s_p[16], s_t[16];
+    const int tid = threadIdx.x, lane = tid & 63, wave = tid >> 6;
+    int carry_p = 0, carry_t = 0;
+    for (int s0 = 0; s0 < nseg; s0 += 1024) {
+        const int sgi = s0 + tid;
+        const int p = sgi < nseg ? segsum[sgi] : 0, t = (p + TM - 1) / TM;
+        int ip = p, it = t;
+        for (int o = 1; o < 64; o <<= 1) {
+            const int a = __shfl_up(ip, o, 64), b = __shfl_up(it, o, 64);
+            if (lane >= o) { ip += a; it += b; }
+        }
+        __syncthreads();
+        if (lane == 63) { s_p[wave] = ip; s_t[wave] = it; }
+        __syncthreads();
+        int bp = carry_p, bt = carry_t;
+        for (int w = 0; w < wave; ++w) { bp += s_p[w]; bt += s_t[w]; }
+        if (sgi < nseg) { seg_off[sgi] = bp + ip - p; tile_start[sgi] = bt + it - t; }
+        for (int w = 0; w < 16; ++w) { carry_p += s_p[w]; carry_t += s_t[w]; }
+    }
+    if (tid == 0) { seg_off[nseg] = carry_p; tile_start[nseg] = carry_t; }
+}
+__global__ void __launch_bounds__(PG)
+pc_emit_kernel(const int32_t *__restrict__ nm, const int32_t *__restrict__ rel, const int32_t *__restrict__ cid,
+               const int32_t *__restrict__ seg_off, int64_t nv, int kv, int32_t *__restrict__ pair_in, int32_t *__restrict__ pair_pos) {
+    __shared__ int s_w[4];
+    const int g = blockIdx.x, k = blockIdx.y, tid = threadIdx.x, lane = tid & 63, wave = tid >> 6;
+    const int64_t u = (int64_t)g * PG + tid;
+    const int in = u < nv ? nm[(int64_t)k * nv + u] : -1;
+    const int base = seg_off[cid[g] * kv + k] + rel[(int64_t)g * 32 + k];
+    const unsigned long long m = __ballot(in >= 0);
+    if (lane == 0) s_w[wave] = __popcll(m);
+    __syncthreads();
+    int slot = base + __popcll(m & ((1ull << lane) - 1ull));
+    for (int w = 0; w < wave; ++w) slot += s_w[w];
+    if (u < nv) {
+        pair_pos[(int64_t)k * nv + u] = in >= 0 ? slot : -1;
+        if (in >= 0) pair_in[slot] = in;
+    }
 }
 constexpr int CP_WIN = 512;
 __device__ __forceinline__ int cp_sum32(int v) {
@@ -1174,6 +1251,42 @@
     GP_CHECK_HIP(rocprim::exclusive_scan(tmp, tb, f, sc, (int32_t)0, (size_t)total, rocprim::plus<int32_t>(), s));
     pair_emit_kernel<<<blocks, 256, 0, s>>>(nbr_map, sc, nv, kv, chunk_row_off, num_chunks, pair_in, pair_pos, seg_off);
     tile_start_kernel<<<1, 64, 0, s>>>(seg_off, nseg, tile_start);
+    tile_desc_kernel<<<(nseg + 255) / 256, 256, 0, s>>>(seg_off, tile_start, nseg, kv, reinterpret_cast<int4 *>(tile_desc));
+    GP_CHECK_LAUNCH();
+    return GP_OK;
+}
+
+extern "C" size_t gp_conv_pairs_build_counted_workspace_bytes(int64_t nv, int32_t kv, int32_t num_chunks) {
+    if (nv <= 0 || kv <= 0 || num_chunks <= 0) return 0;
+    GpCarver cv(nullptr, 0);
+    const size_t ngran = (size_t)((nv + PG - 1) / PG);
+    cv.take<int32_t>((size_t)num_chunks * kv);
+    cv.take<int32_t>(ngran * 32);
+    cv.take<int32_t>(ngran * 32);
+    cv.take<int32_t>(ngran);
+    return cv.off;
+}
+extern "C" int gp_conv_pairs_build_counted(const int32_t *nbr_map, int64_t nv, int32_t kv, int32_t num_chunks, const int32_t *chunk_row_off,
+                                           const int32_t *counts, int32_t *pair_in, int32_t *pair_pos, int32_t *seg_off,
+                                           int32_t *tile_start, int32_t *tile_desc, void *workspace, size_t workspace_bytes, void *stream_) {
+    GP_CHECK_ARG(nbr_map && pair_in && pair_pos && seg_off && tile_start && tile_desc && workspace && nv > 0 && kv > 0 && kv <= 32,
+                 "gp_conv_pairs_build_counted: null/empty argument");
+    GP_CHECK_ARG((int64_t)kv * nv < (1ll << 31), "gp_conv_pairs_build_counted: kernel map too large");
+    GP_CHECK_ARG(num_chunks >= 1 && chunk_row_off, "gp_conv_pairs_build_counted: num_chunks=%d needs the chunk row offsets", num_chunks);
+    const int64_t ngran = (nv + PG - 1) / PG;
+    const int nseg = num_chunks * kv;
+    GpCarver cv(workspace, workspace_bytes);
+    int32_t *segsum = cv.take<int32_t>((size_t)nseg), *own = cv.take<int32_t>((size_t)ngran * 32);
+    int32_t *rel = cv.take<int32_t>((size_t)ngran * 32), *cid = cv.take<int32_t>((size_t)ngran);
+    if (!cv.ok()) { gp_set_error("gp_conv_pairs_build_counted: workspace too small (%zu < %zu)", workspace_bytes, cv.off); return GP_ENOMEM; }
+    hipStream_t s = gp_stream(stream_);
+    if (!counts) {
+        chunk_count_kernel<<<dim3((unsigned)ngran, (unsigned)kv), 256, 0, s>>>(nbr_map, nv, kv, PG, own);
+        counts = own;
+    }
+    pc_seg_sum_kernel<<<(nseg + 3) / 4, 256, 0, s>>>(counts, chunk_row_off, num_chunks, kv, nv, (int)ngran, segsum, rel, cid);
+    pc_seg_scan_kernel<<<1, 1024, 0, s>>>(segsum, nseg, seg_off, tile_start);
+    pc_emit_kernel<<<dim3((unsigned)ngran, (unsigned)kv), PG, 0, s>>>(nbr_map, rel, cid, seg_off, nv, kv, pair_in, pair_pos);
     tile_desc_kernel<<<(nseg + 255) / 256, 256, 0, s>>>(seg_off, tile_start, nseg, kv, reinterpret_cast<int4 *>(tile_desc));
     GP_CHECK_LAUNCH();
     return GP_OK;
diff --git a/geopurify_amd/csrc/voxelize.hip b/geopurify_amd/csrc/voxelize.hip
--- a/geopurify_amd/csrc/voxelize.hip
+++ b/geopurify_amd/csrc/voxelize.hip
@@ -102,39 +102,77 @@
     }
 }
 
-__global__ void views_flags_kernel(const double *__restrict__ c, int64_t n, const double *__restrict__ params,
-                                   const double *__restrict__ depth, int W, int H, int cut, double tau, int32_t *__restrict__ flags) {
-    const int64_t i = blockIdx.x * (int64_t)blockDim.x + threadIdx.x;
-    const int v = blockIdx.y;
-    if (i >= n) return;
+constexpr int VB = 256;
+__global__ void __launch_bounds__(VB)
+views_project_kernel(const double *__restrict__ c, int64_t n, const double *__restrict__ params, const double *__restrict__ depth, int W,
+                     int H, int cut, double tau, unsigned long long *__restrict__ mask , int32_t *__restrict__ cnt ,
+                     int2 *__restrict__ pix ) {
+    __shared__ int s_w[4];
+    const int v = blockIdx.y, lane = threadIdx.x & 63, wave = threadIdx.x >> 6;
+    const int64_t nb = gridDim.x, blk = (int64_t)v * nb + blockIdx.x, i = blockIdx.x * (int64_t)VB + threadIdx.x;
     const double *P = params + v * 20;
-    long long ui, vi;
-    flags[(int64_t)v * n + i] = project_point(c[i * 3], c[i * 3 + 1], c[i * 3 + 2], P, P + 4, P + 8, P[16], P[17], P[18], P[19],
-                                              depth ? depth + (int64_t)v * W * H : nullptr, W, H, cut, tau, ui, vi) ? 1 : 0;
-}
-__global__ void views_compact_kernel(const double *__restrict__ c, int64_t n, int nviews, const double *__restrict__ params,
-                                     const double *__restrict__ depth, int W, int H, int cut, double tau,
-                                     const int32_t *__restrict__ sc , int64_t *__restrict__ ent_pt,
-                                     int64_t *__restrict__ ent_x, int64_t *__restrict__ ent_y, int32_t *__restrict__ ent_view,
-                                     int64_t *__restrict__ view_off) {
-    const int64_t i = blockIdx.x * (int64_t)blockDim.x + threadIdx.x;
-    const int v = blockIdx.y;
-    if (i >= n) return;
-    const double *P = params + v * 20;
-    long long ui, vi;
-    const bool inside = project_point(c[i * 3], c[i * 3 + 1], c[i * 3 + 2], P, P + 4, P + 8, P[16], P[17], P[18], P[19],
-                                      depth ? depth + (int64_t)v * W * H : nullptr, W, H, cut, tau, ui, vi);
-    const int32_t pos = sc[(int64_t)v * n + i];
-    if (inside) { ent_pt[pos] = i; ent_x[pos] = vi; ent_y[pos] = ui; ent_view[pos] = v; }
-    if (i == 0) view_off[v] = pos;
-    if (v == nviews - 1 && i == n - 1) view_off[nviews] = pos + (inside ? 1 : 0);
-}
-__global__ void views_keep_kernel(const int64_t *__restrict__ view_off, int nviews, int64_t min_visible, int64_t val_keep,
-                                  uint8_t *__restrict__ keep) {
-    const int v = blockIdx.x * blockDim.x + threadIdx.x;
-    if (v >= nviews) return;
-    const int64_t nv = view_off[v + 1] - view_off[v];
-    keep[v] = (nv != 0 && nv >= min_visible && nv <= val_keep) ? 1 : 0;
+    long long ui = 0, vi = 0;
+    bool inside = false;
+    if (i < n)
+        inside = project_point(c[i * 3], c[i * 3 + 1], c[i * 3 + 2], P, P + 4, P + 8, P[16], P[17], P[18], P[19],
+                               depth ? depth + (int64_t)v * W * H : nullptr, W, H, cut, tau, ui, vi);
+    const unsigned long long m = __ballot(inside);
+    if (lane == 0) { mask[blk * 4 + wave] = m; s_w[wave] = __popcll(m); }
+    __syncthreads();
+    int rank = __popcll(m & ((1ull << lane) - 1ull));
+    for (int w = 0; w < wave; ++w) rank += s_w[w];
+    if (inside) pix[blk * VB + rank] = make_int2((int)ui, (int)vi);
+    if (threadIdx.x == 0) cnt[blk] = s_w[0] + s_w[1] + s_w[2] + s_w[3];
+}
+__global__ void __launch_bounds__(1024)
+views_scan_kernel(const int32_t *__restrict__ cnt, int nviews, int nb, int32_t *__restrict__ first, int64_t *__restrict__ view_off,
+                  int64_t min_visible, int64_t val_keep, uint8_t *__restrict__ keep) {
+    __shared__ int s_p[16];
+    const int tid = threadIdx.x, lane = tid & 63, wave = tid >> 6;
+    const int64_t total = (int64_t)nviews * nb, per = (total + 1023) / 1024;
+    const int64_t e0 = tid * per, e1 = e0 + per < total ? e0 + per : total;
+    int sum = 0;
+    for (int64_t e = e0; e < e1; ++e) sum += cnt[e];
+    int inc = sum;
+    for (int o = 1; o < 64; o <<= 1) { const int a = __shfl_up(inc, o, 64); if (lane >= o) inc += a; }
+    if (lane == 63) s_p[wave] = inc;
+    __syncthreads();
+    int run = inc - sum, all = 0;
+    for (int w = 0; w < 16; ++w) { if (w < wave) run += s_p[w]; all += s_p[w]; }
+    for (int64_t e = e0; e < e1; ++e) {
+        first[e] = run;
+        if (e % nb == 0) view_off[e / nb] = run;
+        run += cnt[e];
+    }
+    if (tid == 0) view_off[nviews] = all;
+    __threadfence_block();
+    __syncthreads();
+    for (int v = tid; v < nviews; v += 1024) {
+        const int64_t nvis = view_off[v + 1] - view_off[v];
+        keep[v] = (nvis != 0 && nvis >= min_visible && nvis <= val_keep) ? 1 : 0;
+    }
+}
+__global__ void __launch_bounds__(VB)
+views_compact_kernel(int64_t n, const unsigned long long *__restrict__ mask, const int32_t *__restrict__ first, const int2 *__restrict__ pix,
+                     int64_t *__restrict__ ent_pt, int64_t *__restrict__ ent_x, int64_t *__restrict__ ent_y, int32_t *__restrict__ ent_view) {
+    const int v = blockIdx.y, lane = threadIdx.x & 63, wave = threadIdx.x >> 6;
+    const int64_t nb = gridDim.x, blk = (int64_t)v * nb + blockIdx.x;
+    int rank = 0;
+    unsigned long long m = 0;
+#pragma unroll
+    for (int w = 0; w < 4; ++w) {
+        const unsigned long long mw = mask[blk * 4 + w];
+        if (w < wave) rank += __popcll(mw);
+        if (w == wave) m = mw;
+    }
+    if (!((m >> lane) & 1ull)) return;
+    rank += __popcll(m & ((1ull << lane) - 1ull));
+    const int2 px = pix[blk * VB + rank];
+    const int64_t pos = (int64_t)first[blk] + rank;
+    ent_pt[pos] = blockIdx.x * (int64_t)VB + threadIdx.x;
+    ent_x[pos] = px.y;
+    ent_y[pos] = px.x;
+    ent_view[pos] = v;
 }
 
 __global__ void project_kernel(const double *__restrict__ c, int64_t n, Mat44 M, double fx, double fy, double cx,
@@ -261,15 +299,18 @@
     return GP_OK;
 }
 
-static size_t views_scan_tmp(int64_t n) {
-    size_t t = 0;
-    (void)rocprim::exclusive_scan(nullptr, t, (int32_t *)nullptr, (int32_t *)nullptr, (int32_t)0, (size_t)n, rocprim::plus<int32_t>(), 0);
-    return t;
+static void carve_views(GpCarver &cv, int64_t n, int32_t nviews, unsigned long long *&mask, int32_t *&cnt, int32_t *&first, int2 *&pix) {
+    const size_t blocks = (size_t)((n + VB - 1) / VB) * (size_t)nviews;
+    mask = cv.take<unsigned long long>(blocks * 4);
+    cnt = cv.take<int32_t>(blocks);
+    first = cv.take<int32_t>(blocks);
+    pix = cv.take<int2>(blocks * VB);
 }
 extern "C" size_t gp_views_visible_lists_workspace_bytes(int64_t n, int32_t nviews) {
     if (n <= 0 || nviews <= 0) return 0;
     GpCarver cv(nullptr, 0);
-    cv.take<int32_t>(n * nviews); cv.take<int32_t>(n * nviews); cv.take<char>(views_scan_tmp(n * nviews));
+    unsigned long long *mask; int32_t *cnt, *first; int2 *pix;
+    carve_views(cv, n, nviews, mask, cnt, first, pix);
     return cv.off;
 }
 extern "C" int gp_views_visible_lists(const double *coords, int64_t n, const double *params, const double *depth, int32_t nviews,
@@ -281,17 +322,15 @@
     GP_CHECK_ARG(nviews > 0 && nviews <= 65535 && width > 0 && height > 0, "gp_views_visible_lists: bad view count / image size");
     GP_CHECK_ARG(n * (int64_t)nviews < (int64_t)INT32_MAX, "gp_views_visible_lists: n * views must stay below 2^31");
     GpCarver cv(workspace, workspace_bytes);
-    int32_t *flags = cv.take<int32_t>(n * nviews), *sc = cv.take<int32_t>(n * nviews);
-    size_t tb = views_scan_tmp(n * nviews);
-    char *tmp = cv.take<char>(tb);
+    unsigned long long *mask; int32_t *cnt, *first; int2 *pix;
+    carve_views(cv, n, nviews, mask, cnt, first, pix);
     if (!cv.ok()) { gp_set_error("gp_views_visible_lists: workspace too small"); return GP_ENOMEM; }
     hipStream_t s = gp_stream(stream_);
-    dim3 grid((unsigned)((n + 255) / 256), (unsigned)nviews);
-    views_flags_kernel<<<grid, 256, 0, s>>>(coords, n, params, depth, width, height, cut_bound, vis_thres, flags);
-    GP_CHECK_HIP(rocprim::exclusive_scan(tmp, tb, flags, sc, (int32_t)0, (size_t)(n * nviews), rocprim::plus<int32_t>(), s));
-    views_compact_kernel<<<grid, 256, 0, s>>>(coords, n, nviews, params, depth, width, height, cut_bound, vis_thres, sc, ent_pt, ent_x,
-                                              ent_y, ent_view, view_off);
-    views_keep_kernel<<<(nviews + 255) / 256, 256, 0, s>>>(view_off, nviews, min_visible, val_keep, keep);
+    const int nb = (int)((n + VB - 1) / VB);
+    dim3 grid((unsigned)nb, (unsigned)nviews);
+    views_project_kernel<<<grid, VB, 0, s>>>(coords, n, params, depth, width, height, cut_bound, vis_thres, mask, cnt, pix);
+    views_scan_kernel<<<1, 1024, 0, s>>>(cnt, nviews, nb, first, view_off, min_visible, val_keep, keep);
+    views_compact_kernel<<<grid, VB, 0, s>>>(n, mask, first, pix, ent_pt, ent_x, ent_y, ent_view);
     GP_CHECK_LAUNCH();
     return GP_OK;
 }
diff --git a/geopurify_amd/ops.py b/geopurify_amd/ops.py
--- a/geopurify_amd/ops.py
+++ b/geopurify_amd/ops.py
@@ -112,6 +112,29 @@
     check(lib.gp_morton_order(_ptr(coords_i32), nv, _ptr(perm), _ptr(rank), _ptr(ws), ws.numel(), _stream()),
           "gp_morton_order")
     return perm, rank
+
+
+ORDER_BUILT = {"counted": 0, "sorted": 0, "sorted_after_status": 0}
+
+
+def morton_order_counted(coords_i32, origin, extent, want_sorted=False):
+    lib = _lib.load()
+    _chk(coords_i32, torch.int32, "coords")
+    nv = coords_i32.shape[0]
+    dev = coords_i32.device
+    o = (ctypes.c_int32 * 3)(*[int(v) for v in origin])
+    e = (ctypes.c_int32 * 3)(*[int(v) for v in extent])
+    nbytes = lib.gp_morton_order_counted_workspace_bytes(nv, o, e)
+    if nbytes == 0:
+        return None
+    ws = _ws(nbytes, dev)
+    perm = torch.empty(nv, dtype=torch.int32, device=dev)
+    rank = torch.empty(nv, dtype=torch.int32, device=dev)
+    status = torch.empty(1, dtype=torch.int32, device=dev)
+    cs = torch.empty_like(coords_i32) if want_sorted else None
+    check(lib.gp_morton_order_counted(_ptr(coords_i32), nv, o, e, _ptr(perm), _ptr(rank), _ptr(cs), _ptr(status), _ptr(ws), ws.numel(),
+                                      _stream()), "gp_morton_order_counted")
+    return (perm, rank, status, cs) if want_sorted else (perm, rank, status)
 
 
 class Grid:
@@ -339,7 +362,10 @@
 CONV_TARGET_TILES = None
 
 
-def conv_pairs_build(nbr_map, chunk_rows="balanced", col_tiles=2):
+PAIRS_BUILT = {"counted": 0, "scan": 0}
+
+
+def conv_pairs_build(nbr_map, chunk_rows="balanced", col_tiles=2, also_read=None):
     lib = _lib.load()
     kv, nv = nbr_map.shape
     dev = nbr_map.device
@@ -354,7 +380,8 @@
         target = CONV_TARGET_TILES or 3 * torch.cuda.get_device_properties(dev).multi_processor_count - 16
         check(lib.gp_conv_chunk_plan(_ptr(nbr_map), nv, kv, granule, int(col_tiles), int(target), max_chunks, _ptr(plan),
                                      _ptr(plan[max_chunks + 1:]), _ptr(ws), ws.numel(), _stream()), "gp_conv_chunk_plan")
-        host = readback(plan)
+        host = readback(plan if also_read is None else torch.cat([plan, also_read.reshape(-1)]))
+        extra = host[max_chunks + 2:]
         nchunks = host[max_chunks + 1]
         rows = host[:nchunks + 1]
         row_off = plan[:nchunks + 1]
@@ -363,19 +390,34 @@
         rows = list(range(0, nv, ch)) + [nv]
         nchunks = len(rows) - 1
         row_off = torch.tensor(rows, dtype=torch.int32, device=dev)
+        extra = None
     nseg = nchunks * kv
-    ws = _ws(lib.gp_conv_pairs_workspace_bytes(nv, kv), dev)
+    counted = kv <= 32 and all(r % 256 == 0 for r in rows[:-1])
+    PAIRS_BUILT["counted" if counted else "scan"] += 1
     pair_in = torch.empty(kv * nv, dtype=torch.int32, device=dev)
     pair_pos = torch.empty((kv, nv), dtype=torch.int32, device=dev)
     seg_off = torch.empty(nseg + 1, dtype=torch.int32, device=dev)
     tile_start = torch.empty(nseg + 1, dtype=torch.int32, device=dev)
     tile_desc = torch.empty(((kv * nv) // 256 + nseg + 1, 4), dtype=torch.int32, device=dev)
-    check(lib.gp_conv_pairs_build(_ptr(nbr_map), nv, kv, nchunks, _ptr(row_off), _ptr(pair_in), _ptr(pair_pos), _ptr(seg_off),
-                                  _ptr(tile_start), _ptr(tile_desc), _ptr(ws), ws.numel(), _stream()), "gp_conv_pairs_build")
-    bounds = readback(torch.stack([seg_off[::kv], tile_start[::kv]]))
+    if counted:
+        counts = ws if isinstance(chunk_rows, str) else None
+        ws2 = _ws(lib.gp_conv_pairs_build_counted_workspace_bytes(nv, kv, nchunks), dev)
+        check(lib.gp_conv_pairs_build_counted(_ptr(nbr_map), nv, kv, nchunks, _ptr(row_off), _ptr(counts), _ptr(pair_in), _ptr(pair_pos),
+                                              _ptr(seg_off), _ptr(tile_start), _ptr(tile_desc), _ptr(ws2), ws2.numel(), _stream()),
+              "gp_conv_pairs_build_counted")
+    else:
+        ws = _ws(lib.gp_conv_pairs_workspace_bytes(nv, kv), dev)
+        check(lib.gp_conv_pairs_build(_ptr(nbr_map), nv, kv, nchunks, _ptr(row_off), _ptr(pair_in), _ptr(pair_pos), _ptr(seg_off),
+                                      _ptr(tile_start), _ptr(tile_desc), _ptr(ws), ws.numel(), _stream()), "gp_conv_pairs_build")
+    if also_read is not None and extra is None:
+        both = readback(torch.cat([seg_off[::kv], tile_start[::kv], also_read.reshape(-1)]))
+        bounds, extra = [both[:nchunks + 1], both[nchunks + 1:2 * nchunks + 2]], both[2 * nchunks + 2:]
+    else:
+        bounds = readback(torch.stack([seg_off[::kv], tile_start[::kv]]))
     num_pairs = bounds[0][-1]
     cp = ConvPairs(pair_in, pair_pos, seg_off, tile_start, nseg, num_pairs, nv)
     cp.tile_desc = tile_desc
+    cp.also_read = extra
     cp._set_chunks(rows, bounds[1], bounds[0])
     return cp
 
diff --git a/geopurify_amd/pipeline.py b/geopurify_amd/pipeline.py
--- a/geopurify_amd/pipeline.py
+++ b/geopurify_amd/pipeline.py
@@ -481,15 +481,22 @@
         src = torch.where(nn >= 0, nn, torch.arange(N, device=dev))
         return ops.gather_rows(s, D, src), vlm.text_embed, vlm.logit_scale
 
-    def prepare(self, batch: SceneBatch, F):
+    def prepare(self, batch: SceneBatch, F, _sort=False):
         dev = self.device
         N, D = F.shape
         st = self.student
         assert st.cin == D + GEO_DIM, f"student expects {st.cin} input channels, lift gives {D}+{GEO_DIM}"
         coords = batch.scene_coords_3d.floor().to(torch.int32).contiguous()
         Nv = coords.shape[0]
-        perm, rank = ops.morton_order(coords)
-        cs = coords[perm.long()].contiguous()
+        conv = any(l[0] == "f16x3" for l in st.layers)
+        counted = ops.morton_order_counted(coords, [0, 0, 0], batch.extent, want_sorted=True) if (batch.extent is not None and conv
+                                                                                                 and not _sort) else None
+        if counted is not None:
+            perm, rank, order_status, cs = counted
+        else:
+            (perm, rank), order_status = ops.morton_order(coords), None
+            cs = coords[perm.long()].contiguous()
+        ops.ORDER_BUILT["sorted_after_status" if _sort else ("counted" if counted is not None else "sorted")] += 1
         mark = self.stage_mark if self.stage_mark is not None else (lambda name: None)
         mark("morton order")
         if batch.order is None:
@@ -513,7 +520,9 @@
         else:
             grid = ops.grid_build(cs)
         nbr_map = ops.kernel_map_build(grid, cs)
-        pairs = ops.conv_pairs_build(nbr_map, col_tiles=max(1, st.hidden // 256)) if any(l[0] == "f16x3" for l in st.layers) else None
+        pairs = ops.conv_pairs_build(nbr_map, col_tiles=max(1, st.hidden // 256), also_read=order_status) if conv else None
+        if order_status is not None and pairs.also_read[0] != 0:
+            return self.prepare(batch, F, _sort=True)
         mark("grid+kernel_map")
         nbr = ops.knn_lattice(grid, cs, perm, self.K)
         mark("kNN")
diff --git a/include/geopurify_hip.h b/include/geopurify_hip.h
--- a/include/geopurify_hip.h
+++ b/include/geopurify_hip.h
@@ -41,6 +41,10 @@
 size_t gp_morton_order_workspace_bytes(int64_t nv);
 int gp_morton_order(const int32_t *coords, int64_t nv, int32_t *perm, int32_t *rank,
                     void *workspace, size_t workspace_bytes, void *stream);
+size_t gp_morton_order_counted_workspace_bytes(int64_t nv, const int32_t *origin_host, const int32_t *extent_host);
+int gp_morton_order_counted(const int32_t *coords, int64_t nv, const int32_t *origin_host, const int32_t *extent_host,
+                            int32_t *perm, int32_t *rank, int32_t *coords_sorted ,
+                            int32_t *status, void *workspace, size_t workspace_bytes, void *stream);
 size_t gp_grid_bytes(int64_t nv, const int32_t *extent_host);
 int gp_grid_build(const int32_t *coords, int64_t nv, const int32_t *origin_host,
                   const int32_t *extent_host, void *grid, size_t grid_bytes, void *stream);
@@ -73,6 +77,10 @@
                         int32_t *pair_in, int32_t *pair_pos, int32_t *seg_off, int32_t *tile_start,
                         int32_t *tile_desc ,
                         void *workspace, size_t workspace_bytes, void *stream);
+size_t gp_conv_pairs_build_counted_workspace_bytes(int64_t nv, int32_t kv, int32_t num_chunks);
+int gp_conv_pairs_build_counted(const int32_t *nbr_map, int64_t nv, int32_t kv, int32_t num_chunks, const int32_t *chunk_row_off,
+                                const int32_t *counts, int32_t *pair_in, int32_t *pair_pos, int32_t *seg_off, int32_t *tile_start,
+                                int32_t *tile_desc, void *workspace, size_t workspace_bytes, void *stream);
 size_t gp_conv_chunk_plan_workspace_bytes(int64_t nv, int32_t granule_rows);
 int gp_conv_chunk_plan(const int32_t *nbr_map, int64_t nv, int32_t kv, int32_t granule_rows, int32_t col_tiles,
                        int32_t target_tiles, int32_t max_chunks, int32_t *chunk_row_off, int32_t *n_chunks, void *workspace,
```
